# datvo06/MSAU

Measured on AMD Instinct MI355X. Metric: chargrid tiles/sec (train fwd+bwd), 336x256x64 3-stage MSAU, higher is better.
Workload: dtype bf16; 1 GPU; configs[1]: one-hot chargrid 336x256x64, 3-stage MSAU (featRoot 8, 4 scales, res_depth 2), batch 16/GPU, fwd+masked-CE+bwd+clip+Adam; global_batch=16, parallelism=dp1, graph=False

## Files before the change

### include/msau_hip.h

```cpp
#ifndef MSAU_HIP_H
#define MSAU_HIP_H

#include <stdint.h>

#ifdef __cplusplus
extern "C" {
#endif

typedef enum { MSAU_F32 = 0, MSAU_BF16 = 1 } msau_dtype;

typedef enum {
    MSAU_OK = 0,
    MSAU_ERR_ARG = -1,
    MSAU_ERR_LDS = -2,
    MSAU_ERR_HIP = -3
} msau_status;

const char* msau_last_error(void);
int msau_version(void);
const char* msau_source_hash(void);
int msau_sizeof(int which);
int msau_lds_pixel_stride(int raw_bytes, int esz, int c8_per_chunk, int read_stride);
int msau_lds_wrow_stride(int nks, int esz);

enum {
    MSAU_CONV_RELU_IN  = 1,
    MSAU_CONV_RELU_OUT = 2,
    MSAU_CONV_ADD      = 4,
    MSAU_CONV_ACCUM    = 8,
    MSAU_CONV_MASK_A   = 16,
    MSAU_CONV_MASK_B   = 32,
    MSAU_CONV_DOUT     = 128,
    MSAU_CONV_LRN      = 256,
    MSAU_CONV_POOL     = 512,
    MSAU_CONV_IDS      = 1024,
    MSAU_CONV_OWNER    = 2048,
    MSAU_CONV_NCHW     = 4096,
    MSAU_CONV_WGRAD    = 8192,
    MSAU_CONV_ELU      = 32768,
    MSAU_CONV_EXTENT   = 65536,
    MSAU_CONV_HEAD     = 64
};

typedef struct {
    int32_t B, Hin, Win, Hout, Wout;
    int32_t C1, C2;
    int32_t Cout;
    int32_t KH, KW, dil;
    int32_t pad_t, pad_l;
    int32_t stride;
    int32_t ups;
    int32_t flags;
    const void* x1;
    const void* x2;
    const void* wpack;
    const float* bias;
    const void* add;
    const void* mask_a;
    const void* mask_b;
    void* y;
    float* head_probs;
    uint8_t* head_argmax;
    int32_t head_classes;
    int32_t flags2;
    void* y2;
    const void* mask_b2;
    float lrn_alpha_over_n, lrn_beta, lrn_k;
    int32_t reserved0;
    void* pool_y;
    uint8_t* pool_idx;
    const void* wg_x1;
    float* wg_slabs;
    int32_t wg_nslabs;
    int32_t reserved1;
    const int32_t* extent;
} msau_conv_desc;
int msau_conv2d_rider_slabs(int dtype, const msau_conv_desc* d);

typedef struct {
    int32_t cch;
    int32_t nchunks;
    int32_t kchunk;
    int32_t rows;
    int64_t bytes;
} msau_conv_pack_geom;

int msau_conv_pack_geometry(int dtype, int C1_stored, int C2_stored, int Cout_stored, int KH, int KW, int dil,
                            int stride, int ups, msau_conv_pack_geom* out);
int msau_conv2d(void* stream, int dtype, const msau_conv_desc* d);
int msau_conv2d_launch_info(int dtype, const msau_conv_desc* d, int32_t* info8);

enum { MSAU_PAIR_RELU_IN = 1, MSAU_PAIR_RELU_MID = 2, MSAU_PAIR_MASK_MID = 4,
       MSAU_PAIR_LRN_BWD = 16,
       MSAU_PAIR_WGRAD1 = 32,
       MSAU_PAIR_COUPLE = 64,
       MSAU_PAIR_DCOUPLE = 128,
       MSAU_PAIR_TILES = 8 };
typedef struct {
    int32_t B, H, W, C;
    int32_t flags1, flags2;
    const void* x;
    const void* w1;
    const float* b1;
    const void* mask_mid;
    void* mid;
    const void* w2;
    const float* b2;
    const void* add;
    const void* mask_a;
    const void* mask_b;
    void* y;
    void* pool_y;
    uint8_t* pool_idx;
    uint8_t* bits_mid;
    uint8_t* bits_a;
    const void* lrn_a;
    void* lrn_da;
    float lrn_alpha_over_n, lrn_beta, lrn_k;
    int32_t reserved0;
    const void* wg1_x;
    float* wg1_slabs;
    int32_t wg1_nslabs;
    int32_t reserved1;
    const void* cpl_prev;
    const void* cpl_w;
    const float* cpl_b;
    void* cpl_y;
    void* cpl_pool_y;
    uint8_t* cpl_pool_idx;
    const void* dcp_dz;
    const void* dcp_w;
    const void* dcp_mask;
    void* dcp_dprev;
} msau_conv_pair_desc;
int msau_conv_pair_applicable(int dtype, const msau_conv_pair_desc* d);
int msau_conv_pair(void* stream, int dtype, const msau_conv_pair_desc* d);
int64_t msau_conv_pair_bits_bytes(int dtype, const msau_conv_pair_desc* d);
int msau_conv_pair_wgrad_slabs(int dtype, const msau_conv_pair_desc* d);
int msau_conv_pair_instance(int dtype, const msau_conv_pair_desc* d);
void msau_reload_env(void);

typedef struct {
    int32_t B, Hin, Win, Hout, Wout;
    int32_t C1, C2, Cout;
    int32_t KH, KW, dil, pad_t, pad_l, stride;
    int32_t flags;
    const void* x1;
    const void* x2;
    const void* g;
    float* slabs;
    int32_t nslabs;
} msau_wgrad_desc;

typedef struct {
    int32_t cch, nchunks;
    int32_t kext;
    int32_t max_slabs;
// ... 239 lines not shown
```

### msau_amd/_lib.py

```python
from __future__ import annotations

import ctypes as C
import os

HERE = os.path.dirname(os.path.abspath(__file__))
LIB_PATH = os.environ.get("MSAU_HIP_LIB", os.path.join(HERE, "libmsau_hip.so"))

F32, BF16 = 0, 1

CONV_RELU_IN, CONV_RELU_OUT, CONV_ADD, CONV_ACCUM, CONV_MASK_A, CONV_MASK_B, CONV_HEAD, CONV_DOUT = 1, 2, 4, 8, 16, 32, 64, 128
CONV_LRN, CONV_POOL, CONV_IDS, CONV_OWNER, CONV_NCHW, CONV_WGRAD, CONV_ELU = 256, 512, 1024, 2048, 4096, 8192, 32768
CONV_EXTENT = 65536

i32, i64, vp, f32 = C.c_int32, C.c_int64, C.c_void_p, C.c_float


class ConvDesc(C.Structure):
    _fields_ = [(n, i32) for n in ("B", "Hin", "Win", "Hout", "Wout", "C1", "C2", "Cout", "KH", "KW", "dil",
                                   "pad_t", "pad_l", "stride", "ups", "flags")] + \
               [(n, vp) for n in ("x1", "x2", "wpack", "bias", "add", "mask_a", "mask_b", "y", "head_probs", "head_argmax")] + \
               [("head_classes", i32), ("flags2", i32), ("y2", vp), ("mask_b2", vp)] + \
               [("lrn_alpha_over_n", f32), ("lrn_beta", f32), ("lrn_k", f32), ("reserved0", i32), ("pool_y", vp), ("pool_idx", vp)] + \
               [("wg_x1", vp), ("wg_slabs", vp), ("wg_nslabs", i32), ("reserved1", i32), ("extent", vp)]


class ConvPairDesc(C.Structure):
    _fields_ = [(n, i32) for n in ("B", "H", "W", "C", "flags1", "flags2")] + \
               [(n, vp) for n in ("x", "w1", "b1", "mask_mid", "mid", "w2", "b2", "add", "mask_a", "mask_b", "y", "pool_y", "pool_idx", "bits_mid", "bits_a",
                                  "lrn_a", "lrn_da")] + \
               [("lrn_alpha_over_n", f32), ("lrn_beta", f32), ("lrn_k", f32), ("reserved0", i32), ("wg1_x", vp), ("wg1_slabs", vp), ("wg1_nslabs", i32), ("reserved1", i32)] + \
               [(n, vp) for n in ("cpl_prev", "cpl_w", "cpl_b", "cpl_y", "cpl_pool_y", "cpl_pool_idx", "dcp_dz", "dcp_w", "dcp_mask", "dcp_dprev")]


PAIR_RELU_IN, PAIR_RELU_MID, PAIR_MASK_MID, PAIR_TILES, PAIR_LRN_BWD, PAIR_WGRAD1, PAIR_COUPLE, PAIR_DCOUPLE = 1, 2, 4, 8, 16, 32, 64, 128


class BoxArgs(C.Structure):
    _fields_ = [(n, vp) for n in ("in_", "ii", "params_fwd", "params_refl", "out", "gout", "gin", "ii_g", "ws", "flat_grads", "ws_ii",
                                  "mask_a", "add", "mask_b")] + \
               [(n, i64) for n in ("off_hmin", "off_hmax", "off_wmin", "off_wmax")] + \
               [(n, i32) for n in ("B", "H", "W", "C", "F", "Cs_in", "Cs_out", "relu_in", "accumulate")] + \
               [("max_h", f32), ("max_w", f32)]


class ConvPackGeom(C.Structure):
    _fields_ = [("cch", i32), ("nchunks", i32), ("kchunk", i32), ("rows", i32), ("bytes", i64)]


class WgradDesc(C.Structure):
    _fields_ = [(n, i32) for n in ("B", "Hin", "Win", "Hout", "Wout", "C1", "C2", "Cout", "KH", "KW", "dil",
                                   "pad_t", "pad_l", "stride", "flags")] + \
               [(n, vp) for n in ("x1", "x2", "g", "slabs")] + [("nslabs", i32)]


class WgradGeom(C.Structure):
    _fields_ = [("cch", i32), ("nchunks", i32), ("kext", i32), ("max_slabs", i32), ("slab_bytes", i64),
                ("lean", i32), ("reserved", i32)]


class PackEntry(C.Structure):
    _fields_ = [("src_off", i64), ("dst_off", i64)] + \
               [(n, i32) for n in ("kind", "dim0", "dim1", "KH", "KW", "row_is_dim0", "flip", "row_off", "rows_real",
                                   "rows_pad", "k1_real", "k1_store", "k2_real", "k2_store", "cch", "nchunks",
                                   "kchunk", "dtype")]


class UnpackEntry(C.Structure):
    _fields_ = [("slab_off", i64), ("w_off", i64), ("b_off", i64), ("b_src_off", i64), ("b_slab_stride", i64)] + \
               [(n, i32) for n in ("b_elem_stride", "b_nslabs", "b_count", "nslabs", "slab_elems", "kext", "dim0", "dim1", "KH",
                                   "KW", "row_is_dim0", "rows_real", "k1_real", "k1_store", "k2_real", "k2_store",
                                   "cch", "nchunks", "accumulate")]


class Op(C.Structure):
    _fields_ = [("kind", i32), ("dtype", i32), ("args", vp)]


class LrnArgs(C.Structure):
    _fields_ = [("a", vp), ("dy", vp), ("out", vp), ("npix", i64), ("C", i32), ("Cs", i32), ("n", i32),
                ("alpha", f32), ("beta", f32), ("k", f32)]


class PoolArgs(C.Structure):
    _fields_ = [("x_or_dy", vp), ("y_or_dx", vp), ("idx", vp), ("mask", vp)] + \
               [(n, i32) for n in ("B", "H", "W", "Cs", "accumulate")] + [("extent", vp)]


class AttnArgs(C.Structure):
    _fields_ = [(n, vp) for n in ("f", "g", "h", "x_or_dy", "y", "stats", "df", "dg", "dh", "ws")] + \
               [(n, i32) for n in ("B", "N", "Ds", "Cs")] + [("extent", vp), ("W", i32), ("reserved0", i32)]


class CsumArgs(C.Structure):
    _fields_ = [("g", vp), ("npix", i64), ("Cs", i32), ("partials", vp), ("nblk", i32)]


class ReduceArgs(C.Structure):
    _fields_ = [("slab_arena", vp), ("flat_grads", vp), ("table_dev", vp), ("n_entries", i32), ("max_elems", i32)]


class AllreduceArgs(C.Structure):
    _fields_ = [("comm", vp), ("buf", vp), ("count", i64)]


class OwnerCtx(C.Structure):
    _fields_ = [(n, vp) for n in ("owner", "boxes", "feats", "w", "wt", "table", "sums", "csum")] + \
# ... 230 lines not shown
```

### msau_amd/csrc/conv.hip

```cpp
#include "msau_common.h"

namespace {

struct ConvGeom {
    int esz, taps, cch, nchunks, kchunk, rows, CT, ngroups;
    int nslices;
};

__host__ __device__ inline int pix_stride_bytes(int cch, int esz) {
    int ps = cch * esz;
    if (((ps >> 4) & 1) == 0) ps += 16;
    return ps;
}

struct TileGeom { int TH, TIH, TIW, PS, WS, in_bytes, w_bytes, tab_bytes, total; };

inline bool conv_compact(int KH, int KW, int dil, int stride, int ups) { return stride == 1 && ups == 1 && dil >= 16 && KH * KW > 1; }

inline TileGeom tile_geom(const ConvGeom& g, int PT, int KH, int KW, int dil, int stride, int ups = 1) {
    TileGeom t;
    t.TH = 4 * PT;
    t.TIH = (t.TH - 1) * stride + (KH - 1) * dil + 1;
    t.TIW = 15 * stride + (KW - 1) * dil + 1;
    if (conv_compact(KH, KW, dil, stride, ups)) { t.TIH = KH * KW * t.TH; t.TIW = 16; }
// ... 228 lines not shown
#pragma unroll
                    for (int j = 0; j < 4; ++j) v[j] = fmaxf(v[j], 0.f);
                }
            }
            if (flags & MSAU_CONV_MASK_B) {
                V4 m = load4<T>(mask_b + pbase + co);
                if (flags & MSAU_CONV_ELU) {
#pragma unroll
                    for (int j = 0; j < 4; ++j) v[j] = ((float)m[j] > 0.f) ? v[j] : v[j] * ((float)m[j] + 1.f);
                } else {
#pragma unroll
                    for (int j = 0; j < 4; ++j) v[j] = ((float)m[j] > 0.f) ? v[j] : 0.f;
                }
            }
            if (outside) v = f32x4{0.f, 0.f, 0.f, 0.f};
            V4 o;
#pragma unroll
            for (int j = 0; j < 4; ++j) o[j] = (T)v[j];
            store4<T>(y + pbase + co, o);
        }
    }
}

template <typename T, int CT, int PT>
int launch_conv(hipStream_t s, const ConvArgs& a, int nblocks, int nsplit, int lds) {
    static bool attr_set = false;
    if (!attr_set) {
        hipError_t e = hipFuncSetAttribute(reinterpret_cast<const void*>(&conv_kernel<T, CT, PT>),
                                           hipFuncAttributeMaxDynamicSharedMemorySize, MSAU_LDS_LIMIT);
        if (e != hipSuccess) return msau_set_error(MSAU_ERR_HIP, "conv: hipFuncSetAttribute: %s", hipGetErrorString(e));
        attr_set = true;
    }
    hipLaunchKernelGGL((conv_kernel<T, CT, PT>), dim3(nblocks, nsplit), dim3(256), lds, s, a);
    MSAU_CHECK_LAUNCH("conv_kernel");
    return 0;
}

template <typename T, int CT>
int launch_conv_pt(hipStream_t s, const ConvArgs& a, int PT, int nblocks, int nsplit, int lds) {
    switch (PT) {
        case 4: return launch_conv<T, CT, 4>(s, a, nblocks, nsplit, lds);
        case 2: return launch_conv<T, CT, 2>(s, a, nblocks, nsplit, lds);
        default: return launch_conv<T, CT, 1>(s, a, nblocks, nsplit, lds);
    }
}

template <typename T>
int launch_conv_ct(hipStream_t s, const ConvArgs& a, int CT, int PT, int nblocks, int nsplit, int lds) {
    switch (CT) {
        case 1: return launch_conv_pt<T, 1>(s, a, PT, nblocks, nsplit, lds);
        case 2: return launch_conv_pt<T, 2>(s, a, PT, nblocks, nsplit, lds);
        case 4: return launch_conv_pt<T, 4>(s, a, PT, nblocks, nsplit, lds);
        default: return launch_conv_pt<T, 8>(s, a, PT, nblocks, nsplit, lds);
    }
}

}

extern "C" int msau_conv_pack_geometry(int dtype, int C1, int C2, int Cout, int KH, int KW, int dil, int stride, int ups,
                                       msau_conv_pack_geom* out) {
    ConvGeom g;
    int rc = conv_geom(dtype, C1, C2, Cout, KH, KW, dil, stride, ups, &g);
    if (rc) return rc;
    out->cch = g.cch; out->nchunks = g.nchunks; out->kchunk = g.kchunk; out->rows = g.rows * g.nslices;
    out->bytes = (int64_t)g.nslices * g.nchunks * g.rows * g.kchunk * g.esz;
    return 0;
}

static int conv_plan(int dtype, const msau_conv_desc* d, ConvGeom* gout, TileGeom* tout, int* PTout, int64_t* nbout);
int msau_conv_lean_applicable(int dtype, const msau_conv_desc* d, int nchunks, int CT);
int msau_conv_lean_try(hipStream_t s, int dtype, const msau_conv_desc* d, int kchunk, int nchunks, int CT);
int msau_conv_lean_head_capable(int dtype, const msau_conv_desc* d, int nchunks, int CT);
int msau_conv_lean_dout_capable(int dtype, const msau_conv_desc* d, int nchunks, int CT);
int msau_conv_lean_lrn_capable(int dtype, const msau_conv_desc* d, int nchunks, int CT);
int msau_conv_lean_pool_capable(int dtype, const msau_conv_desc* d, int nchunks, int CT);
int msau_conv_lean_ids_capable(int dtype, const msau_conv_desc* d, int nchunks, int CT);
int msau_conv_chunked_try(hipStream_t s, int dtype, const msau_conv_desc* d, int cch, int kchunk, int nchunks, int CT);
int msau_conv_chunked_capable(int dtype, const msau_conv_desc* d, int cch, int nchunks, int CT);
int msau_firstconv_takes(int dtype, const msau_conv_desc* d);
int msau_firstconv_launch(hipStream_t s, int dtype, const msau_conv_desc* d, int real_channels);

static int conv_takes_extent(int dtype, const msau_conv_desc* d, const ConvGeom& g) {
    const int only_others = MSAU_CONV_HEAD | MSAU_CONV_DOUT | MSAU_CONV_LRN | MSAU_CONV_POOL | MSAU_CONV_IDS | MSAU_CONV_OWNER |
                            MSAU_CONV_NCHW | MSAU_CONV_WGRAD;
    if (d->flags & only_others) return 0;
    if (g.nslices == 1 && (msau_rowconv_takes(dtype, d) || msau_conv_chunked_capable(dtype, d, g.cch, g.nchunks, g.CT) ||
                           msau_conv_lean_applicable(dtype, d, g.nchunks, g.CT)))
        return 0;
    return 1;
}

extern "C" int msau_conv2d_launch_info(int dtype, const msau_conv_desc* d, int32_t* info) {
    MSAU_CHECK_ARG(d && info, "conv2d_launch_info: null pointer");
    ConvGeom g; TileGeom t; int PT; int64_t nb;
    int rc = conv_plan(dtype, d, &g, &t, &PT, &nb);
    if (rc) return rc;
    info[0] = g.CT; info[1] = PT; info[2] = t.total; info[3] = (int32_t)nb; info[4] = g.cch; info[5] = g.nchunks;
    info[6] = msau_conv_lean_applicable(dtype, d, g.nchunks, g.CT);
    if (g.nslices == 1 && msau_rowconv_takes(dtype, d)) info[6] = 3;
    if (g.nslices == 1 && !(d->flags & (MSAU_CONV_HEAD | MSAU_CONV_DOUT | MSAU_CONV_LRN | MSAU_CONV_POOL | MSAU_CONV_IDS)) &&
        msau_conv_chunked_capable(dtype, d, g.cch, g.nchunks, g.CT)) info[6] = 2;
    info[7] = msau_conv_lean_head_capable(dtype, d, g.nchunks, g.CT) | (msau_conv_lean_dout_capable(dtype, d, g.nchunks, g.CT) << 1) |
              (((d->flags & MSAU_CONV_DOUT) && g.nslices == 1 && msau_rowconv_takes(dtype, d)) << 1) |
              (msau_conv_lean_lrn_capable(dtype, d, g.nchunks, g.CT) << 2) | (msau_conv_lean_pool_capable(dtype, d, g.nchunks, g.CT) << 3) |
              (msau_conv_lean_ids_capable(dtype, d, g.nchunks, g.CT) << 4);
    {
        msau_conv_desc p = *d;
        p.flags |= MSAU_CONV_OWNER;
        if (msau_ownerconv_takes(dtype, &p)) info[7] |= 32;
    }
    {
        msau_conv_desc p = *d;
        p.flags |= MSAU_CONV_NCHW;
        if (msau_firstconv_takes(dtype, &p)) info[7] |= 64;
    }
    {
        msau_conv_desc p = *d;
        p.flags |= MSAU_CONV_EXTENT;
        if (conv_takes_extent(dtype, &p, g)) info[7] |= 128;
    }
    if (g.nslices == 1 && !(info[7] & 4)) {
        msau_conv_desc p = *d;
        p.flags |= MSAU_CONV_LRN;
        if (!p.y2) p.y2 = p.y;
        if (!(p.lrn_k > 0.f)) p.lrn_k = 1.f;
        if (msau_rowconv_takes(dtype, &p)) info[7] |= 4;
    }
    return 0;
}

static int conv_plan(int dtype, const msau_conv_desc* d, ConvGeom* gout, TileGeom* tout, int* PTout, int64_t* nbout) {
    ConvGeom g;
    int rc = conv_geom(dtype, d->C1, d->C2, d->Cout, d->KH, d->KW, d->dil, d->stride, d->ups, &g);
    if (rc) return rc;
    int PT = 4;
    auto ntiles = [&](int pt) { return (int64_t)d->B * cdiv(d->Hout, 4 * pt) * cdiv(d->Wout, 16); };
    if (ntiles(4) < 512) PT = ntiles(2) >= 384 ? 2 : 1;
    TileGeom t = tile_geom(g, PT, d->KH, d->KW, d->dil, d->stride, d->ups);
    while (t.total > 150 * 1024 && PT > 1) { PT >>= 1; t = tile_geom(g, PT, d->KH, d->KW, d->dil, d->stride, d->ups); }
    if (t.total > 150 * 1024) return msau_set_error(MSAU_ERR_LDS, "conv2d: tile needs %d B of LDS", t.total);
    int64_t nb = ntiles(PT);
    MSAU_CHECK_ARG(nb < (1ll << 31), "conv2d: grid too large");
    *gout = g; *tout = t; *PTout = PT; *nbout = nb;
    return 0;
}

extern "C" int msau_conv2d(void* stream, int dtype, const msau_conv_desc* d) {
    MSAU_CHECK_ARG(d && d->x1 && d->wpack && d->y, "conv2d: null pointer");
    MSAU_CHECK_ARG(d->B > 0 && d->Hin > 0 && d->Win > 0 && d->Hout > 0 && d->Wout > 0, "conv2d: bad dims");
    MSAU_CHECK_ARG(d->C1 % 8 == 0 && d->C2 % 8 == 0 && (d->C2 == 0 || d->x2), "conv2d: bad sources");
    MSAU_CHECK_ARG(!(d->flags & MSAU_CONV_ADD) || d->add, "conv2d: ADD without pointer");
    MSAU_CHECK_ARG(!(d->flags & MSAU_CONV_MASK_A) || d->mask_a, "conv2d: MASK_A without pointer");
    MSAU_CHECK_ARG(!(d->flags & MSAU_CONV_MASK_B) || d->mask_b, "conv2d: MASK_B without pointer");
    if (d->flags & MSAU_CONV_EXTENT) {
        MSAU_CHECK_ARG(d->extent, "conv2d: MSAU_CONV_EXTENT without extent pointer");
        ConvGeom g;
        int rc = conv_geom(dtype, d->C1, d->C2, d->Cout, d->KH, d->KW, d->dil, d->stride, d->ups, &g);
        if (rc) return rc;
        if (!conv_takes_extent(dtype, d, g))
            return msau_set_error(MSAU_ERR_ARG, "conv2d: MSAU_CONV_EXTENT is not implemented for this launch (flags 0x%x; see "
                                  "msau_conv2d_launch_info info[7] & 128): only the generic tile kernel has it", d->flags);
    }
    if (d->flags & MSAU_CONV_WGRAD)
        MSAU_CHECK_ARG(msau_conv2d_rider_slabs(dtype, d) > 0, "conv2d: MSAU_CONV_WGRAD is not implemented for this launch (msau_conv2d_rider_slabs says 0)");
    if (d->flags & MSAU_CONV_OWNER) {
        MSAU_CHECK_ARG(msau_ownerconv_takes(dtype, d), "conv2d: MSAU_CONV_OWNER is the 3x3 stride-1 C -> 8 conv, no other flag but RELU_OUT");
        return msau_ownerconv_fwd(static_cast<hipStream_t>(stream), dtype, d);
    }
    if (d->flags & MSAU_CONV_NCHW) {
        MSAU_CHECK_ARG(msau_firstconv_takes(dtype, d) && d->head_classes > 0 && d->head_classes <= d->C1,
                       "conv2d: MSAU_CONV_NCHW is the bf16 3x3 64 -> 8 conv (W %% 4 == 0, W <= 288), head_classes = real input channels");
        return msau_firstconv_launch(static_cast<hipStream_t>(stream), dtype, d, d->head_classes);
    }
    ConvGeom g; TileGeom t; int PT; int64_t nb;
    int rc = conv_plan(dtype, d, &g, &t, &PT, &nb);
    if (rc) return rc;
    if (d->flags & MSAU_CONV_HEAD) {
        MSAU_CHECK_ARG(d->head_probs && d->head_argmax && d->head_classes > 0 && d->head_classes <= 16 &&
                       d->head_classes <= d->Cout && d->flags == MSAU_CONV_HEAD, "conv2d: bad HEAD arguments");
        if (!msau_conv_lean_head_capable(dtype, d, g.nchunks, g.CT))
            return msau_set_error(MSAU_ERR_ARG, "conv2d: MSAU_CONV_HEAD is not implemented for this launch (see "
                                  "msau_conv2d_launch_info info[7]); run msau_softmax_argmax_nhwc on y instead");
    }
    if (d->flags & MSAU_CONV_DOUT) {
        const int okf = MSAU_CONV_DOUT | MSAU_CONV_ADD | MSAU_CONV_ACCUM | MSAU_CONV_MASK_B | MSAU_CONV_WGRAD;
        MSAU_CHECK_ARG(d->y2 && !(d->flags & ~okf) && !(d->flags2 & ~(MSAU_CONV_ACCUM | MSAU_CONV_MASK_B)) &&
                       (!(d->flags2 & MSAU_CONV_MASK_B) || d->mask_b2), "conv2d: bad DOUT arguments");
        if (!msau_conv_lean_dout_capable(dtype, d, g.nchunks, g.CT) && !(g.nslices == 1 && msau_rowconv_takes(dtype, d)))
            return msau_set_error(MSAU_ERR_ARG, "conv2d: MSAU_CONV_DOUT is not implemented for this launch (see "
                                  "msau_conv2d_launch_info info[7]); issue one launch per output instead");
    }
    if (d->flags & MSAU_CONV_LRN) {
        MSAU_CHECK_ARG(d->y2 && !(d->flags & ~(MSAU_CONV_LRN | MSAU_CONV_RELU_IN)) && d->lrn_k > 0.f, "conv2d: bad LRN arguments");
        if (!msau_conv_lean_lrn_capable(dtype, d, g.nchunks, g.CT) && !(g.nslices == 1 && msau_rowconv_takes(dtype, d)))
            return msau_set_error(MSAU_ERR_ARG, "conv2d: MSAU_CONV_LRN is not implemented for this launch (see "
                                  "msau_conv2d_launch_info info[7]); run msau_lrn_fwd on y instead");
    }
    if (d->flags & MSAU_CONV_IDS) {
        if (!msau_conv_lean_ids_capable(dtype, d, g.nchunks, g.CT))
            return msau_set_error(MSAU_ERR_ARG, "conv2d: MSAU_CONV_IDS is not implemented for this launch (see msau_conv2d_launch_info "
                                  "info[7] & 16); paint the one-hot input with msau_onehot_ids instead");
    }
    if (d->flags & MSAU_CONV_POOL) {
        MSAU_CHECK_ARG(d->pool_y && !(d->flags & (MSAU_CONV_DOUT | MSAU_CONV_HEAD | MSAU_CONV_LRN)), "conv2d: bad POOL arguments");
        if (!msau_conv_lean_pool_capable(dtype, d, g.nchunks, g.CT))
            return msau_set_error(MSAU_ERR_ARG, "conv2d: MSAU_CONV_POOL is not implemented for this launch (see "
                                  "msau_conv2d_launch_info info[7]); run msau_maxpool2x2_fwd on y instead");
    }
    if (g.nslices == 1 && msau_rowconv_takes(dtype, d))
        return msau_rowconv_launch(static_cast<hipStream_t>(stream), dtype, d, g.kchunk, g.rows);
    if (g.nslices == 1 && !(d->flags & (MSAU_CONV_HEAD | MSAU_CONV_DOUT | MSAU_CONV_LRN | MSAU_CONV_POOL | MSAU_CONV_IDS))) {
        rc = msau_conv_chunked_try(static_cast<hipStream_t>(stream), dtype, d, g.cch, g.kchunk, g.nchunks, g.CT);
        if (rc != 0) return rc < 0 ? rc : 0;
    }
    if (g.nslices == 1) {
        rc = msau_conv_lean_try(static_cast<hipStream_t>(stream), dtype, d, g.kchunk, g.nchunks, g.CT);
        if (rc != 0) return rc < 0 ? rc : 0;
    }
    if (d->flags & MSAU_CONV_DOUT) return msau_set_error(MSAU_ERR_ARG, "conv2d: DOUT launch was not taken by a lean instance");
    MSAU_CHECK_ARG(g.nslices == 1 || !(d->flags & MSAU_CONV_HEAD), "conv2d: HEAD with more than 128 output channels");
    hipStream_t s = static_cast<hipStream_t>(stream);
    static const int split_wgs = getenv("MSAU_CONV_ROWSPLIT") ? atoi(getenv("MSAU_CONV_ROWSPLIT")) : 768;
    int cts = g.CT;
    while (cts > 1 && nb * g.nslices * (g.CT / cts) < split_wgs) cts >>= 1;
    const int w_bytes = roundup(cts * 16 * t.WS, 16), lds_total = t.in_bytes + w_bytes + t.tab_bytes;
    for (int sl = 0; sl < g.nslices; ++sl) {
        ConvArgs a;
        a.d = *d;
        a.ystride = d->Cout;
        a.compact = conv_compact(d->KH, d->KW, d->dil, d->stride, d->ups);
        if (g.nslices > 1) {
            const size_t co0 = (size_t)sl * 128, esz = g.esz;
            a.d.Cout = d->Cout - (int)co0 < 128 ? d->Cout - (int)co0 : 128;
            a.d.wpack = static_cast<const char*>(d->wpack) + (size_t)sl * g.nchunks * g.rows * g.kchunk * esz;
            if (d->bias) a.d.bias = d->bias + co0;
            a.d.y = static_cast<char*>(d->y) + co0 * esz;
            if (d->add) a.d.add = static_cast<const char*>(d->add) + co0 * esz;
            if (d->mask_a) a.d.mask_a = static_cast<const char*>(d->mask_a) + co0 * esz;
            if (d->mask_b) a.d.mask_b = static_cast<const char*>(d->mask_b) + co0 * esz;
        }
        a.cch = g.cch; a.nchunks = g.nchunks; a.kchunk = g.kchunk; a.ngroups = g.ngroups;
        a.TIH = t.TIH; a.TIW = t.TIW; a.PS = t.PS; a.WS = t.WS; a.in_bytes = t.in_bytes; a.w_bytes = w_bytes;
        a.tiles_x = cdiv(d->Wout, 16); a.tiles_y = cdiv(d->Hout, 4 * PT);
        a.ct_total = g.CT; a.rows_total = g.rows;
        rc = dtype == MSAU_F32 ? launch_conv_ct<float>(s, a, cts, PT, (int)nb, g.CT / cts, lds_total)
                               : launch_conv_ct<bf16_t>(s, a, cts, PT, (int)nb, g.CT / cts, lds_total);
        if (rc) return rc;
    }
    return 0;
}
```

### msau_amd/csrc/conv_lean.hip

```cpp
#include "msau_common.h"
#include <cstdlib>

namespace {

struct LeanArgs {
    msau_conv_desc d;
    int kchunk;
    int in_px1, in_px2, in_row1, in_row2;
    int out_px, out_row;
    int tiles_x, tiles_y, ntiles;
    unsigned mag_tx, mag_ty;
    int per_xcd;
    int ct_total;
#ifdef MSAU_STAMPS
    unsigned long long* stamps;
#endif
};
#ifdef MSAU_STAMPS
#define STAMP(i) do { if (a.stamps && threadIdx.x == 0) a.stamps[((size_t)blockIdx.y * gridDim.x + blockIdx.x) * 8 + (i)] = __builtin_amdgcn_s_memrealtime(); } while (0)
#else
#define STAMP(i) do {} while (0)
#endif

template <typename T, int CIN8, int CT, int KS, bool DUAL, int DIL = 1, int WGW = 1, int STRIDE = 1>
struct LeanCfg {
    static constexpr int ESZ = (int)sizeof(T);
    static constexpr int TI = 15 * STRIDE + 1 + (KS - 1) * DIL;
    static constexpr int TIW = (16 * WGW - 1) * STRIDE + 1 + (KS - 1) * DIL;
    static constexpr int NT = 256 * WGW;
    static constexpr int PSRAW = CIN8 * 8 * ESZ;
    static constexpr int NPIX = TI * TIW;
    static constexpr int NCH = DUAL ? 2 : 1;
    static constexpr int C8H = CIN8 / NCH;
    static constexpr int PS = lds_pixel_stride(PSRAW, ESZ, C8H, STRIDE);
    static constexpr int NG = KS * KS * C8H;
    static constexpr int NKSH = (NG + 3) / 4;
    static constexpr int NKS = NCH * NKSH;
    static constexpr bool WREG = CT * NKS <= 8;
    static constexpr int WS = lds_wrow_stride(NKSH, ESZ);
    static constexpr int IN_BYTES = ((NPIX * PS + 15) / 16) * 16;
    static constexpr int LDS = IN_BYTES + (WREG ? 0 : NCH * CT * 16 * WS);
};

constexpr int kOperandBits = MSAU_CONV_RELU_IN | MSAU_CONV_RELU_OUT | MSAU_CONV_ADD | MSAU_CONV_ACCUM | MSAU_CONV_MASK_A | MSAU_CONV_MASK_B;
enum { EPI_NONE = 0, EPI_LRN = 1, EPI_POOL = 2, EPI_HEAD = 3 };
template <typename T, int CIN8, int CT, int KS, bool DUAL, int DIL = 1, int WGW = 1, bool DOUT = false, bool SPLIT = false,
          int STRIDE = 1, int UPS = 1, int EPI = EPI_NONE, int EOP = -1, bool IDS = false>
__global__ __launch_bounds__(256 * WGW) void conv_lean_kernel(const LeanArgs a) {
    static_assert(!IDS || (!DUAL && STRIDE == 1 && UPS == 1 && !DOUT && !SPLIT), "id-mask input: plain single-source instances");
    static_assert(!SPLIT || (CT == 1 && !DUAL && !DOUT && WGW == 1), "SPLIT instances are single-source, one tile per workgroup");
    static_assert((STRIDE == 1 && UPS == 1) || (!DUAL && !DOUT && WGW == 1 && DIL == 1 && STRIDE * UPS == 2), "strided / upsampling instances");
    STAMP(0);
    const int cty = SPLIT ? (int)blockIdx.y : 0;
    const int CTT = SPLIT ? a.ct_total : CT;
    using Cfg = LeanCfg<T, CIN8, CT, KS, DUAL, DIL, WGW, STRIDE>;
    constexpr int NT = Cfg::NT;
    typedef typename Vec8<T>::type V8;
    typedef typename Vec4<T>::type V4;
    constexpr int ESZ = Cfg::ESZ, TI = Cfg::TIW, PS = Cfg::PS, NKS = Cfg::NKS, NG = Cfg::NG, NKSH = Cfg::NKSH, C8H = Cfg::C8H;
    extern __shared__ __align__(16) unsigned char smem[];
    const msau_conv_desc& d = a.d;
    const int tid = threadIdx.x, lane = tid & 63;
    const int wave_all = __builtin_amdgcn_readfirstlane(tid >> 6);
    const int wave = wave_all & 3, cwt = wave_all >> 2;
    const int lr = lane & 15, lg = lane >> 4;
    const bool relu_in = (EOP >= 0 ? EOP : d.flags) & MSAU_CONV_RELU_IN;

    const T* wp = static_cast<const T*>(d.wpack) + (SPLIT ? (size_t)cty * 16 * a.kchunk : 0);
    V8 afr[Cfg::WREG ? CT : 1][Cfg::WREG ? NKS : 1];
    if constexpr (Cfg::WREG) {
#pragma unroll
        for (int ct = 0; ct < CT; ++ct)
#pragma unroll
            for (int ks = 0; ks < NKS; ++ks)
                afr[ct][ks] = load8<T>(wp + ((size_t)(ks / NKSH) * (CT * 16) + ct * 16 + lr) * a.kchunk + (ks % NKSH) * 32 + lg * 8);
    }

    int koff[NKS];
#pragma unroll
    for (int ks = 0; ks < NKS; ++ks) {
        const int G = (ks % NKSH) * 4 + lg;
        const int tap = G / C8H, cg = G - tap * C8H;
        const int ky = tap / KS, kx = tap - ky * KS;
        koff[ks] = G < NG ? (ky * DIL * TI + kx * DIL) * PS + ((ks / NKSH) * C8H + cg) * 8 * ESZ : 0;
    }
    const unsigned char* pixp = smem + ((wave * 4) * STRIDE * TI + (cwt * 16 + lr) * STRIDE) * PS;

    const int flags = EOP >= 0 ? ((d.flags & ~kOperandBits) | EOP) : d.flags;
    const int Cout = d.Cout;
    f32x4 bv[CT];
#pragma unroll
    for (int ct = 0; ct < CT; ++ct) {
        bv[ct] = f32x4{0.f, 0.f, 0.f, 0.f};
        if (d.bias && lg * (CTT * 4) + (cty + ct) * 4 < Cout) bv[ct] = *reinterpret_cast<const f32x4*>(d.bias + lg * (CTT * 4) + (cty + ct) * 4);
    }
    const long long delta_add = static_cast<const char*>(d.add) - static_cast<const char*>(d.y);
    const long long delta_ma = static_cast<const char*>(d.mask_a) - static_cast<const char*>(d.y);
    const long long delta_mb = static_cast<const char*>(d.mask_b) - static_cast<const char*>(d.y);
    const int lane_out = (cwt * 16 + lr) * a.out_px + (lg * (CTT * 4) + cty * 4) * ESZ;

    constexpr int C8S = DUAL ? CIN8 / 2 : CIN8;
    constexpr int NITEMS = Cfg::NPIX * C8S;
    constexpr int NIT = (NITEMS + NT - 1) / NT;
    constexpr int NSRC = DUAL ? 2 : 1;
    constexpr bool PIPE = IDS || NIT * NSRC <= 6;
    V8 pre[IDS ? 1 : NSRC][IDS ? 1 : NIT];
    constexpr int NIDS = (Cfg::NPIX + NT - 1) / NT;
    int pre_id[IDS ? NIDS : 1];
    auto decode = [&](int tile, int& b, int& oy0, int& ox0) {
        const int t1 = a.tiles_x > 1 ? __umulhi((unsigned)tile, a.mag_tx) : tile;
        ox0 = (tile - t1 * a.tiles_x) * (16 * WGW);
        b = a.tiles_y > 1 ? __umulhi((unsigned)t1, a.mag_ty) : t1;
        oy0 = (t1 - b * a.tiles_y) * 16;
    };
    auto issue_loads = [&](int tile) {
        int b, oy0, ox0;
        decode(tile, b, oy0, ox0);
        const int vy0 = oy0 * STRIDE - d.pad_t, vx0 = ox0 * STRIDE - d.pad_l;
        if constexpr (IDS) {
            const int* ids = static_cast<const int*>(d.x1) + (long long)b * d.Hin * d.Win;
#pragma unroll
            for (int it = 0; it < NIDS; ++it) {
                const int pix = tid + it * NT;
                const int iy = pix / TI, ix = pix - iy * TI;
                const int vy = vy0 + iy, vx = vx0 + ix;
                pre_id[it] = -1;
                if (pix < Cfg::NPIX && (unsigned)vy < (unsigned)d.Hin && (unsigned)vx < (unsigned)d.Win) pre_id[it] = ids[vy * d.Win + vx];
            }
        } else
#pragma unroll
        for (int sidx = 0; sidx < NSRC; ++sidx) {
            const char* base = static_cast<const char*>(sidx ? d.x2 : d.x1) + (long long)b * d.Hin * (sidx ? a.in_row2 : a.in_row1);
            const int in_row = sidx ? a.in_row2 : a.in_row1, in_px = sidx ? a.in_px2 : a.in_px1;
#pragma unroll
            for (int it = 0; it < NIT; ++it) {
                const int idx = tid + it * NT;
                pre[sidx][it] = zero8<T>();
                if ((it + 1) * NT <= NITEMS || idx < NITEMS) {
                    const int pix = idx / C8S, cg = idx - pix * C8S;
                    const int iy = pix / TI, ix = pix - iy * TI;
                    int vy = vy0 + iy, vx = vx0 + ix;
                    bool ok;
                    if constexpr (UPS == 2) {
                        ok = vy >= 0 && vx >= 0 && !((vy | vx) & 1) && (vy >> 1) < d.Hin && (vx >> 1) < d.Win;
                        vy >>= 1; vx >>= 1;
                    } else {
                        ok = (unsigned)vy < (unsigned)d.Hin && (unsigned)vx < (unsigned)d.Win;
                    }
                    if (ok)
                        pre[sidx][it] = *reinterpret_cast<const V8*>(base + (unsigned)(vy * in_row + vx * in_px + cg * 8 * ESZ));
                }
            }
        }
    };
    auto write_lds = [&]() {
        if constexpr (IDS) {
#pragma unroll
            for (int it = 0; it < NIDS; ++it) {
                const int pix = tid + it * NT;
                if (pix < Cfg::NPIX) {
                    const int id = pre_id[it];
#pragma unroll
                    for (int cg = 0; cg < C8S; ++cg) {
                        V8 v;
#pragma unroll
                        for (int j = 0; j < 8; ++j) v[j] = (T)(cg * 8 + j == id ? 1.0f : 0.0f);
                        *reinterpret_cast<V8*>(smem + pix * PS + cg * 8 * ESZ) = v;
                    }
                }
            }
        } else
#pragma unroll
        for (int sidx = 0; sidx < NSRC; ++sidx)
#pragma unroll
            for (int it = 0; it < NIT; ++it) {
                const int idx = tid + it * NT;
                if ((it + 1) * NT <= NITEMS || idx < NITEMS) {
                    const int pix = idx / C8S, cg = idx - pix * C8S;
                    V8 v = pre[sidx][it];
                    if (relu_in) v = relu8<T>(v);
                    *reinterpret_cast<V8*>(smem + pix * PS + (sidx * C8S + cg) * 8 * ESZ) = v;
                }
            }
    };
    int tile0 = blockIdx.x, tend = a.ntiles, tstep = gridDim.x;
    if (a.per_xcd) {
        const int xcd = blockIdx.x & 7;
        tile0 = xcd * a.per_xcd + (blockIdx.x >> 3);
        tend = min(a.ntiles, (xcd + 1) * a.per_xcd);
        tstep = gridDim.x >> 3;
    }
    if (PIPE && tile0 < tend) issue_loads(tile0);
    if constexpr (!Cfg::WREG) {
        unsigned char* lds_w = smem + Cfg::IN_BYTES;
        constexpr int WG8 = NKSH * 4;
        constexpr int WTOT = Cfg::NCH * CT * 16 * WG8, NWIT = (WTOT + NT - 1) / NT, WB = NWIT < 8 ? NWIT : 8;
#pragma unroll
        for (int it0 = 0; it0 < NWIT; it0 += WB) {
            V8 wr[WB];
#pragma unroll
            for (int j = 0; j < WB; ++j) {
                const int idx = tid + (it0 + j) * NT;
                if (it0 + j < NWIT && idx < WTOT) {
                    const int r = idx / WG8, g8 = idx - r * WG8;
                    wr[j] = load8<T>(wp + (size_t)r * a.kchunk + g8 * 8);
                }
            }
#pragma unroll
            for (int j = 0; j < WB; ++j) {
                const int idx = tid + (it0 + j) * NT;
                if (it0 + j < NWIT && idx < WTOT) {
                    const int r = idx / WG8, g8 = idx - r * WG8;
                    *reinterpret_cast<V8*>(lds_w + r * Cfg::WS + g8 * 8 * ESZ) = wr[j];
                }
            }
        }
    }

    STAMP(1);
    for (int tile = tile0; tile < tend; tile += tstep) {
        int b, oy0, ox0;
        decode(tile, b, oy0, ox0);
        __syncthreads();
        if (!PIPE) issue_loads(tile);
        write_lds();
        __syncthreads();
        if (tile == tile0) STAMP(2);
        if (PIPE && tile + tstep < tend) issue_loads(tile + tstep);
        const int oyw = oy0 + wave * 4;
        f32x4 acc[CT][4];
#pragma unroll
        for (int ct = 0; ct < CT; ++ct)
#pragma unroll
            for (int pt = 0; pt < 4; ++pt) acc[ct][pt] = f32x4{0.f, 0.f, 0.f, 0.f};
#pragma unroll
        for (int ks = 0; ks < NKS; ++ks) {
            const unsigned char* p = pixp + koff[ks];
            V8 bfrag[4];
#pragma unroll
            for (int pt = 0; pt < 4; ++pt) bfrag[pt] = *reinterpret_cast<const V8*>(p + pt * STRIDE * TI * PS);
#pragma unroll
            for (int ct = 0; ct < CT; ++ct) {
                V8 af;
                if constexpr (Cfg::WREG) af = afr[ct][ks];
                else af = *reinterpret_cast<const V8*>(smem + Cfg::IN_BYTES + ((ks / NKSH) * (CT * 16) + ct * 16 + lr) * Cfg::WS +
                                                       ((ks % NKSH) * 32 + lg * 8) * ESZ);
#pragma unroll
                for (int pt = 0; pt < 4; ++pt) acc[ct][pt] = mma8(af, bfrag[pt], acc[ct][pt]);
            }
        }

        if (tile == tile0) { asm volatile("" :: "v"(acc[0][0][0])); STAMP(3); }
        if constexpr (DOUT) {
            const bool t2 = lg >= 2;
            const int lfl = t2 ? d.flags2 : flags;
            char* yb = static_cast<char*>(t2 ? d.y2 : d.y);
            const char* mb = static_cast<const char*>(t2 ? d.mask_b2 : d.mask_b);
            const char* ad = static_cast<const char*>(d.add);
            if (ox0 + lr < d.Wout) {
                const long long off0 = ((long long)(b * d.Hout + oyw)) * a.out_row + (long long)ox0 * a.out_px +
                                       lr * a.out_px + (lg & 1) * (CT * 4) * ESZ;
#pragma unroll
                for (int ct = 0; ct < CT; ++ct) {
                    V4 r_add[4], r_acc[4], r_mb[4];
#pragma unroll
                    for (int pt = 0; pt < 4; ++pt) {
                        if (oyw + pt < d.Hout) {
                            const long long o = off0 + ct * 4 * ESZ + (long long)pt * a.out_row;
                            if (lfl & MSAU_CONV_ADD) r_add[pt] = *reinterpret_cast<const V4*>(ad + o);
                            if (lfl & MSAU_CONV_ACCUM) r_acc[pt] = *reinterpret_cast<const V4*>(yb + o);
                            if (lfl & MSAU_CONV_MASK_B) r_mb[pt] = *reinterpret_cast<const V4*>(mb + o);
                        }
                    }
#pragma unroll
                    for (int pt = 0; pt < 4; ++pt) {
                        if (oyw + pt < d.Hout) {
                            const long long o = off0 + ct * 4 * ESZ + (long long)pt * a.out_row;
                            f32x4 v = acc[ct][pt] + bv[ct];
                            if (lfl & MSAU_CONV_ADD) {
#pragma unroll
                                for (int j = 0; j < 4; ++j) v[j] += (float)r_add[pt][j];
                            }
                            if (lfl & MSAU_CONV_ACCUM) {
#pragma unroll
                                for (int j = 0; j < 4; ++j) v[j] += (float)r_acc[pt][j];
                            }
                            if (lfl & MSAU_CONV_MASK_B) {
#pragma unroll
                                for (int j = 0; j < 4; ++j) v[j] = ((float)r_mb[pt][j] > 0.f) ? v[j] : 0.f;
                            }
                            V4 ov;
#pragma unroll
                            for (int j = 0; j < 4; ++j) ov[j] = (T)v[j];
                            *reinterpret_cast<V4*>(yb + o) = ov;
                        }
                    }
                }
            }
        } else {
        constexpr bool POOL_OK = EPI == EPI_POOL;
        static_assert(EPI == EPI_NONE || (CT <= 2 && !DOUT && STRIDE == 1 && UPS == 1), "fused epilogues: <= 2 channel tiles, one output");
        V4 keep[POOL_OK ? CT : 1][4];
        if constexpr (POOL_OK) {
#pragma unroll
            for (int ct = 0; ct < CT; ++ct)
#pragma unroll
                for (int pt = 0; pt < 4; ++pt)
#pragma unroll
// ... 213 lines not shown
        const int oy0 = (t1 - b * a.tiles_y) * 16;
        const int vy0 = oy0 - d.pad_t, vx0 = ox0 - d.pad_l;
        const char* xb = static_cast<const char*>(d.x1) + (long long)b * d.Hin * a.in_row1;
        auto issue = [&](int ch) {
#pragma unroll
            for (int it = 0; it < NITX; ++it) {
                const int idx = tid + it * 256;
                const int pix = idx / C8CH, cg = idx - pix * C8CH;
                const int iy = pix / TI, ix = pix - iy * TI;
                const int vy = vy0 + iy, vx = vx0 + ix;
                xr[it] = zero8<T>();
                if (idx < NPIX * C8CH && (unsigned)vy < (unsigned)d.Hin && (unsigned)vx < (unsigned)d.Win)
                    xr[it] = *reinterpret_cast<const V8*>(xb + (unsigned)(vy * a.in_row1 + vx * a.in_px1 + (ch * C8CH * 8 + cg * 8) * ESZ));
            }
#pragma unroll
            for (int it = 0; it < NITW; ++it) {
                const int idx = tid + it * 256;
                const int r = idx / WG8, g8 = idx - r * WG8;
                wr[it] = zero8<T>();
                if (idx < CT * 16 * WG8) wr[it] = load8<T>(wp + ((size_t)ch * CT * 16 + r) * a.kchunk + g8 * 8);
            }
        };
        f32x4 acc[CT][4];
#pragma unroll
        for (int ct = 0; ct < CT; ++ct)
#pragma unroll
            for (int pt = 0; pt < 4; ++pt) acc[ct][pt] = f32x4{0.f, 0.f, 0.f, 0.f};
        issue(0);
        for (int ch = 0; ch < nchunks; ++ch) {
            __syncthreads();
#pragma unroll
            for (int it = 0; it < NITX; ++it) {
                const int idx = tid + it * 256;
                if (idx < NPIX * C8CH) *reinterpret_cast<V8*>(smem + (idx / C8CH) * PS + (idx % C8CH) * 8 * ESZ) = xr[it];
            }
#pragma unroll
            for (int it = 0; it < NITW; ++it) {
                const int idx = tid + it * 256;
                const int r = idx / WG8, g8 = idx - r * WG8;
                if (idx < CT * 16 * WG8) *reinterpret_cast<V8*>(lds_w + r * WS + g8 * 8 * ESZ) = wr[it];
            }
            __syncthreads();
            if (ch + 1 < nchunks) issue(ch + 1);
#pragma unroll
            for (int ks = 0; ks < NKS; ++ks) {
                const unsigned char* p = pixp + koff[ks];
                V8 bfrag[4];
#pragma unroll
                for (int pt = 0; pt < 4; ++pt) bfrag[pt] = *reinterpret_cast<const V8*>(p + pt * TI * PS);
#pragma unroll
                for (int ct = 0; ct < CT; ++ct) {
                    const V8 af = *reinterpret_cast<const V8*>(lds_w + (ct * 16 + lr) * WS + (ks * 32 + lg * 8) * ESZ);
#pragma unroll
                    for (int pt = 0; pt < 4; ++pt) acc[ct][pt] = mma8(af, bfrag[pt], acc[ct][pt]);
                }
            }
        }
        const int oyw = oy0 + wave * 4;
        if (ox0 + lr < d.Wout) {
            char* y = static_cast<char*>(d.y) + ((long long)(b * d.Hout + oyw) * d.Wout + ox0 + lr) * a.out_px;
#pragma unroll
            for (int ct = 0; ct < CT; ++ct) {
                if (lg * (CT * 4) + ct * 4 >= d.Cout) continue;
#pragma unroll
                for (int pt = 0; pt < 4; ++pt) {
                    if (oyw + pt < d.Hout) {
                        f32x4 v = acc[ct][pt] + bv[ct];
                        if (d.flags & MSAU_CONV_RELU_OUT) {
#pragma unroll
                            for (int j = 0; j < 4; ++j) v[j] = fmaxf(v[j], 0.f);
                        }
                        V4 o;
#pragma unroll
                        for (int j = 0; j < 4; ++j) o[j] = (T)v[j];
                        *reinterpret_cast<V4*>(y + (long long)pt * a.out_row + (lg * (CT * 4) + ct * 4) * ESZ) = o;
                    }
                }
            }
        }
    }
}

template <typename T, int CIN8, int CT, int KS, bool DUAL, int DIL = 1, int WGW = 1, bool DOUT = false, bool SPLIT = false,
          int STRIDE = 1, int UPS = 1, int EPI = EPI_NONE, int EOP = -1, bool IDS = false>
int launch_lean_e(hipStream_t s, const LeanArgs& a0) {
    using Cfg = LeanCfg<T, CIN8, CT, KS, DUAL, DIL, WGW, STRIDE>;
    if (Cfg::LDS + 256 > MSAU_LDS_LIMIT) return 0;
    LeanArgs a = a0;
    a.tiles_x = cdiv(a.d.Wout, 16 * WGW);
    a.ntiles = a.d.B * a.tiles_x * a.tiles_y;
    a.mag_tx = (unsigned)((0x100000000ull + a.tiles_x - 1) / a.tiles_x);
    static bool attr_set = false;
    if (!attr_set && Cfg::LDS > 60 * 1024) {
        hipError_t e = hipFuncSetAttribute(reinterpret_cast<const void*>(&conv_lean_kernel<T, CIN8, CT, KS, DUAL, DIL, WGW, DOUT, SPLIT, STRIDE, UPS, EPI, EOP, IDS>),
                                           hipFuncAttributeMaxDynamicSharedMemorySize, MSAU_LDS_LIMIT);
        if (e != hipSuccess) return msau_set_error(MSAU_ERR_HIP, "conv_lean: hipFuncSetAttribute: %s", hipGetErrorString(e));
        attr_set = true;
    }
    int per_cu = MSAU_LDS_LIMIT / (Cfg::LDS + 256);
    static const int percu_max = std::getenv("MSAU_LEAN_PERCU") ? atoi(std::getenv("MSAU_LEAN_PERCU")) : 4;
    per_cu = per_cu < 1 ? 1 : (per_cu > percu_max / WGW ? (percu_max / WGW < 1 ? 1 : percu_max / WGW) : per_cu);
    int grid = 256 * per_cu;
    if (grid > a.ntiles) grid = a.ntiles;
    static const bool xcd_off = std::getenv("MSAU_XCD") && std::getenv("MSAU_XCD")[0] == '0';
    a.per_xcd = 0;
    if (!xcd_off && grid >= 64) {
        grid &= ~7;
        a.per_xcd = cdiv(a.ntiles, 8);
    }
    hipLaunchKernelGGL((conv_lean_kernel<T, CIN8, CT, KS, DUAL, DIL, WGW, DOUT, SPLIT, STRIDE, UPS, EPI, EOP, IDS>), dim3(grid, SPLIT ? a.ct_total : 1), dim3(256 * WGW), Cfg::LDS, s, a);
    MSAU_CHECK_LAUNCH("conv_lean_kernel");
    return 1;
}

template <typename T, int CIN8, int CT, int KS, bool DUAL, int DIL = 1, int WGW = 1, bool DOUT = false, bool SPLIT = false,
          int STRIDE = 1, int UPS = 1, int EPI = EPI_NONE>
int launch_lean(hipStream_t s, const LeanArgs& a) {
    if constexpr (CIN8 <= 2 && !DOUT && EPI != EPI_HEAD) {
        switch (a.d.flags & kOperandBits) {
#define EOP_CASE(V) case V: return launch_lean_e<T, CIN8, CT, KS, DUAL, DIL, WGW, DOUT, SPLIT, STRIDE, UPS, EPI, V>(s, a);
            EOP_CASE(0) EOP_CASE(2) EOP_CASE(3) EOP_CASE(6) EOP_CASE(8) EOP_CASE(12) EOP_CASE(20) EOP_CASE(32) EOP_CASE(40)
#undef EOP_CASE
            default: break;
        }
    }
    return launch_lean_e<T, CIN8, CT, KS, DUAL, DIL, WGW, DOUT, SPLIT, STRIDE, UPS, EPI, -1>(s, a);
}

template <typename T, int CIN8, int KS, bool DUAL>
int lean_ct(hipStream_t s, const LeanArgs& a, int CT) {
    if constexpr (sizeof(T) == 2 && (CIN8 == 1 || (DUAL && CIN8 == 2)) && KS == 3) {
        if (CT == 1 && a.d.Wout >= 64 && (int64_t)a.d.B * a.tiles_y * cdiv(a.d.Wout, 32) >= 512)
            return launch_lean<T, CIN8, 1, KS, DUAL, 1, 2>(s, a);
    }
    if (CT == 1) return launch_lean<T, CIN8, 1, KS, DUAL>(s, a);
    if (CT == 2) return launch_lean<T, CIN8, 2, KS, DUAL>(s, a);
    if constexpr (CIN8 >= 4 && KS != 4) {
        if (CT == 4) return launch_lean<T, CIN8, 4, KS, DUAL>(s, a);
    }
    return 0;
}

template <typename T, int KS>
int lean_cin(hipStream_t s, const LeanArgs& a, int cin8, bool dual, int CT) {
    if (!dual) {
        switch (cin8) {
            case 1: return lean_ct<T, 1, KS, false>(s, a, CT);
            case 2: return lean_ct<T, 2, KS, false>(s, a, CT);
            case 4: return lean_ct<T, 4, KS, false>(s, a, CT);
            case 8: return lean_ct<T, 8, KS, false>(s, a, CT);
            default: return 0;
        }
    }
    switch (cin8) {
        case 2: return lean_ct<T, 2, KS, true>(s, a, CT);
        case 4: return lean_ct<T, 4, KS, true>(s, a, CT);
        case 8: return lean_ct<T, 8, KS, true>(s, a, CT);
        case 16: if constexpr (KS == 1) return lean_ct<T, 16, KS, true>(s, a, CT); else return 0;
        default: return 0;
    }
}

template <typename T, int DIL>
int lean_dil(hipStream_t s, const LeanArgs& a, int cin8, int CT) {
#define LD_CASE(C8, CTV) if (cin8 == C8 && CT == CTV) return launch_lean<T, C8, CTV, 3, false, DIL>(s, a);
    LD_CASE(1, 1) LD_CASE(2, 1) LD_CASE(2, 2) LD_CASE(4, 1) LD_CASE(4, 2) LD_CASE(4, 4) LD_CASE(8, 2)
#undef LD_CASE
    return 0;
}

}

static bool lean_split_wanted(const msau_conv_desc* d, int CT);

static int lean_lds_bytes(int esz, int cin8, int CT, int KS, int dil, int wgw, int stride, bool dual) {
    const int ti = 15 * stride + 1 + (KS - 1) * dil, tiw = (16 * wgw - 1) * stride + 1 + (KS - 1) * dil;
    const int psraw = cin8 * 8 * esz, ps = ((psraw / 16) % 2 == 0) ? psraw + 16 : psraw;
    const int nch = dual ? 2 : 1, c8h = cin8 / nch, ng = KS * KS * c8h, nksh = (ng + 3) / 4, nks = nch * nksh;
    const bool wreg = CT * nks <= 8;
    const int ws = nksh * 32 * esz + 16;
    const int in_bytes = ((ti * tiw * ps + 15) / 16) * 16;
    return in_bytes + (wreg ? 0 : nch * CT * 16 * ws);
}

static bool lean_strided_shape(const msau_conv_desc* d, int nchunks, int CT) {
    if (d->KH != 3 || d->KW != 3 || d->dil != 1 || d->C2 || nchunks != 1 || d->stride * d->ups != 2) return false;
    if (d->flags & (MSAU_CONV_DOUT | MSAU_CONV_HEAD | MSAU_CONV_RELU_IN)) return false;
    if (d->pad_t < 0 || d->pad_l < 0 || d->pad_t > 2 || d->pad_l > 2) return false;
    if ((int64_t)d->B * cdiv(d->Hout, 16) * cdiv(d->Wout, 16) < 64) return false;
    const int c8 = d->C1 / 8;
    if (d->ups == 2) return (c8 == 8 && CT == 2) || (c8 == 4 && CT == 1) || (c8 == 2 && CT == 1);
    return (c8 == 4 && CT == 4) || (c8 == 2 && CT == 2) || (c8 == 1 && CT == 1);
}
template <typename T>
int lean_strided(hipStream_t s, const LeanArgs& a, int c8, int CT, bool ups) {
#define ST_CASE(C8, CTV, ST, UP) if (c8 == C8 && CT == CTV) return launch_lean<T, C8, CTV, 3, false, 1, 1, false, false, ST, UP>(s, a);
    if (ups) { ST_CASE(8, 2, 1, 2) ST_CASE(4, 1, 1, 2) ST_CASE(2, 1, 1, 2) }
    else { ST_CASE(4, 4, 2, 1) ST_CASE(2, 2, 2, 1) ST_CASE(1, 1, 2, 1) }
#undef ST_CASE
    return 0;
}

int msau_conv_lean_applicable(int dtype, const msau_conv_desc* d, int nchunks, int CT) {
    if (d->flags & (MSAU_CONV_ELU | MSAU_CONV_EXTENT)) return 0;
    if (d->stride * d->ups == 2) {
        const int esz = dtype == MSAU_F32 ? 4 : 2;
        if ((int64_t)d->Hin * d->Win * d->C1 * esz >= (1ll << 31) || (int64_t)d->Wout * d->Cout * esz * 20 >= (1ll << 31)) return 0;
        if (!lean_strided_shape(d, nchunks, CT)) return 0;
        return lean_lds_bytes(esz, d->C1 / 8, CT, 3, 1, 1, d->stride, false) + 256 <= MSAU_LDS_LIMIT;
    }
    if (d->stride != 1 || d->ups != 1 || d->KH != d->KW || (d->KH != 1 && d->KH != 3 && d->KH != 4)) return 0;
    if (d->dil != 1) {
        if (d->KH != 3 || d->C2 || (d->dil != 2 && d->dil != 4 && d->dil != 8)) return 0;
        const int c8 = d->C1 / 8;
        const bool ok = (c8 == 1 && CT == 1) || (c8 == 2 && CT <= 2) || (c8 == 4 && (CT == 1 || CT == 2 || CT == 4)) || (c8 == 8 && CT == 2);
        if (!ok) return 0;
    }
    if (nchunks != (d->C2 ? 2 : 1)) return 0;
    if (d->Hin != d->Hout || d->Win != d->Wout) return 0;
    if (d->pad_t < 0 || d->pad_l < 0 || d->pad_t > (d->KH - 1) * d->dil || d->pad_l > (d->KW - 1) * d->dil) return 0;
    if (CT > 4 || (CT == 4 && (d->C1 + d->C2) < 32)) return 0;
    if (d->KH == 4 && ((d->C1 + d->C2) != 8 || d->C2)) return 0;
    if ((int64_t)d->B * cdiv(d->Hout, 16) * cdiv(d->Wout, 16) < 64) return 0;
    const bool dual = d->C2 != 0;
    if (dual && d->C1 != d->C2) return 0;
    const int cin8 = (d->C1 + d->C2) / 8;
    const int esz = dtype == MSAU_F32 ? 4 : 2;
    if ((int64_t)d->Hin * d->Win * (d->C1 > d->C2 ? d->C1 : d->C2) * esz >= (1ll << 31)) return 0;
    if ((int64_t)d->Wout * d->Cout * esz * 20 >= (1ll << 31)) return 0;
    if (cin8 != 1 && cin8 != 2 && cin8 != 4 && cin8 != 8 && !(cin8 == 16 && dual && d->KH == 1)) return 0;
    if (dual && cin8 < 2) return 0;
    const bool split = lean_split_wanted(d, CT);
    if (lean_lds_bytes(esz, cin8, split ? 1 : CT, d->KH, d->dil, 1, 1, dual) + 256 > MSAU_LDS_LIMIT) return 0;
    return 1;
}

int msau_conv_lean_dout_capable(int dtype, const msau_conv_desc* d, int nchunks, int CT) {
    if (!msau_conv_lean_applicable(dtype, d, nchunks, CT)) return 0;
    return d->C2 == 0 && d->dil == 1 && d->stride == 1 && d->ups == 1 && (d->KH == 1 || d->KH == 3) && (CT == 1 || CT == 2 || CT == 4) &&
           d->Cout == CT * 16 && d->C1 == CT * 8;
}

static bool lean_wide_tile(const msau_conv_desc* d, int tiles_y) {
    return d->Wout >= 64 && (int64_t)d->B * tiles_y * cdiv(d->Wout, 32) >= 512;
}
static int lean_epi_case(int dtype, const msau_conv_desc* d, int CT, int epi) {
    const int c8 = (d->C1 + d->C2) / 8, k = d->KH;
    const bool dual = d->C2 != 0, split = lean_split_wanted(d, CT);
    if (epi == EPI_LRN && !dual && !split && k == 3) {
        if (c8 == 1 && CT == 1 && d->dil == 1 && d->Cout == 8) return dtype == MSAU_BF16 && lean_wide_tile(d, cdiv(d->Hout, 16)) ? 1 : 2;
        if (c8 == 1 && CT == 1 && d->dil == 2 && d->Cout == 16) return 3;
        if (c8 == 2 && CT == 2 && d->dil == 4 && d->Cout == 32) return 4;
        if (c8 == 2 && CT == 1 && d->dil == 1 && d->Cout == 16) return 5;
        if (c8 == 2 && CT == 2 && d->dil == 2 && d->Cout == 32) return 6;
    }
    if (epi == EPI_POOL && d->dil == 1) {
        if (dual && k == 1 && !split) {
            if (c8 == 2 && CT == 1) return 10;
            if (c8 == 4 && CT == 1) return 11;
            if (c8 == 8 && CT == 2) return 12;
        }
        if (!dual && k == 3 && split && c8 == 4) return 13;
    }
    return 0;
}
template <typename T>
int lean_epi(hipStream_t s, const LeanArgs& a, int which) {
    switch (which) {
        case 1: if constexpr (sizeof(T) == 2) return launch_lean<T, 1, 1, 3, false, 1, 2, false, false, 1, 1, EPI_LRN>(s, a); else return 0;
        case 2: return launch_lean<T, 1, 1, 3, false, 1, 1, false, false, 1, 1, EPI_LRN>(s, a);
        case 3: return launch_lean<T, 1, 1, 3, false, 2, 1, false, false, 1, 1, EPI_LRN>(s, a);
        case 4: return launch_lean<T, 2, 2, 3, false, 4, 1, false, false, 1, 1, EPI_LRN>(s, a);
        case 5: return launch_lean<T, 2, 1, 3, false, 1, 1, false, false, 1, 1, EPI_LRN>(s, a);
        case 6: return launch_lean<T, 2, 2, 3, false, 2, 1, false, false, 1, 1, EPI_LRN>(s, a);
        case 10: return launch_lean<T, 2, 1, 1, true, 1, 1, false, false, 1, 1, EPI_POOL>(s, a);
        case 11: return launch_lean<T, 4, 1, 1, true, 1, 1, false, false, 1, 1, EPI_POOL>(s, a);
        case 12: return launch_lean<T, 8, 2, 1, true, 1, 1, false, false, 1, 1, EPI_POOL>(s, a);
        case 13: return launch_lean<T, 4, 1, 3, false, 1, 1, false, true, 1, 1, EPI_POOL>(s, a);
        default: return 0;
    }
}

int msau_conv_lean_lrn_capable(int dtype, const msau_conv_desc* d, int nchunks, int CT) {
    if (!msau_conv_lean_applicable(dtype, d, nchunks, CT)) return 0;
    if (d->stride != 1 || d->ups != 1 || (d->flags & (MSAU_CONV_DOUT | MSAU_CONV_HEAD | MSAU_CONV_POOL))) return 0;
    return lean_epi_case(dtype, d, CT, EPI_LRN) != 0;
}

int msau_conv_lean_pool_capable(int dtype, const msau_conv_desc* d, int nchunks, int CT) {
    if (!msau_conv_lean_applicable(dtype, d, nchunks, CT)) return 0;
    if (d->stride != 1 || d->ups != 1 || (d->flags & (MSAU_CONV_DOUT | MSAU_CONV_HEAD | MSAU_CONV_LRN))) return 0;
    return lean_epi_case(dtype, d, CT, EPI_POOL) != 0;
}

template <typename T>
int lean_dout(hipStream_t s, const LeanArgs& a, int KS, int CT) {
#define DO_CASE(K, C) if (KS == K && CT == C) return launch_lean<T, C, C, K, false, 1, 1, true>(s, a);
    DO_CASE(1, 1) DO_CASE(1, 2) DO_CASE(1, 4) DO_CASE(3, 1) DO_CASE(3, 2) DO_CASE(3, 4)
#undef DO_CASE
    return 0;
}

static int lean_split_tiles() {
    static const int v = std::getenv("MSAU_SPLIT_TILES") ? atoi(std::getenv("MSAU_SPLIT_TILES")) : 512;
    return v;
}
static bool lean_split_wanted(const msau_conv_desc* d, int CT) {
    const int cin8 = d->C1 / 8;
    return d->C2 == 0 && d->dil == 1 && (d->KH == 1 || d->KH == 3) && (CT == 2 || CT == 4) && (cin8 == 4 || cin8 == 8) &&
           !(d->flags & (MSAU_CONV_DOUT | MSAU_CONV_HEAD)) &&
           (int64_t)d->B * cdiv(d->Hout, 16) * cdiv(d->Wout, 16) < lean_split_tiles();
}
template <typename T>
int lean_split(hipStream_t s, const LeanArgs& a, int cin8, int KS) {
#define SP_CASE(C8, K) if (cin8 == C8 && KS == K) return launch_lean<T, C8, 1, K, false, 1, 1, false, true>(s, a);
    SP_CASE(4, 1) SP_CASE(4, 3) SP_CASE(8, 1) SP_CASE(8, 3)
#undef SP_CASE
    return 0;
}

int msau_conv_lean_ids_capable(int dtype, const msau_conv_desc* d, int nchunks, int CT) {
    msau_conv_desc e = *d;
    e.flags &= ~MSAU_CONV_IDS;
    return msau_conv_lean_applicable(dtype, &e, nchunks, CT) && d->C1 == 64 && d->C2 == 0 && CT == 1 && d->KH == 3 && d->dil == 1 &&
           d->stride == 1 && d->ups == 1 && !(d->flags & ~(MSAU_CONV_IDS | MSAU_CONV_RELU_OUT));
}

int msau_conv_lean_head_capable(int dtype, const msau_conv_desc* d, int nchunks, int CT) {
    return msau_conv_lean_applicable(dtype, d, nchunks, CT) && d->KH == 4 && CT == 1 && d->dil == 1;
}

static int chunked_variant(int dtype, const msau_conv_desc* d, int cch, int nchunks, int CT) {
    static const bool off = std::getenv("MSAU_CONV_CHUNKED") && std::getenv("MSAU_CONV_CHUNKED")[0] == '0';
    if (off || nchunks < 2 || d->C2 || d->KH != 3 || d->KW != 3 || d->stride != 1 || d->ups != 1) return 0;
    if (d->Hin != d->Hout || d->Win != d->Wout || d->pad_t < 0 || d->pad_l < 0 || d->pad_t > 2 * d->dil || d->pad_l > 2 * d->dil) return 0;
    if (d->flags & ~MSAU_CONV_RELU_OUT) return 0;
    const int esz = dtype == MSAU_F32 ? 4 : 2;
    if ((int64_t)d->Hin * d->Win * d->C1 * esz >= (1ll << 31)) return 0;
    const int64_t ntiles = (int64_t)d->B * cdiv(d->Wout, 16) * cdiv(d->Hout, 16);
    if (!(ntiles >= 64 && ntiles < (1 << 20) && cdiv(d->Wout, 16) < 4096 && cdiv(d->Hout, 16) < 4096)) return 0;
    if (cch == 64 && CT == 1 && d->dil == 1) return 1;
    if (cch == 32 && CT == 2 && d->dil == 8 && nchunks == 2 && dtype == MSAU_BF16) return 2;
    return 0;
}
int msau_conv_chunked_capable(int dtype, const msau_conv_desc* d, int cch, int nchunks, int CT) {
    if (d->flags & (MSAU_CONV_ELU | MSAU_CONV_EXTENT)) return 0;
    return chunked_variant(dtype, d, cch, nchunks, CT) != 0;
}

template <typename T, int C8CH, int CT, int DIL>
static int launch_chunked(hipStream_t s, const LeanArgs& a, int nchunks) {
    using Cfg = LeanCfg<T, C8CH, CT, 3, false, DIL>;
    constexpr int lds = Cfg::IN_BYTES + CT * 16 * lds_wrow_stride(Cfg::NKS, Cfg::ESZ);
    static_assert(lds + 256 <= MSAU_LDS_LIMIT, "chunked conv: tile + weight chunk must fit the LDS");
    static bool attr_set = false;
    if (!attr_set && lds > 60 * 1024) {
        hipError_t e = hipFuncSetAttribute(reinterpret_cast<const void*>(&conv_chunked_kernel<T, C8CH, CT, DIL>), hipFuncAttributeMaxDynamicSharedMemorySize, MSAU_LDS_LIMIT);
        if (e != hipSuccess) return msau_set_error(MSAU_ERR_HIP, "conv_chunked: hipFuncSetAttribute: %s", hipGetErrorString(e));
        attr_set = true;
    }
    int per_cu = MSAU_LDS_LIMIT / (lds + 256);
    per_cu = per_cu < 1 ? 1 : (per_cu > 3 ? 3 : per_cu);
    int grid = 256 * per_cu;
    if (grid > a.ntiles) grid = a.ntiles;
    hipLaunchKernelGGL((conv_chunked_kernel<T, C8CH, CT, DIL>), dim3(grid), dim3(256), lds, s, a, nchunks);
    MSAU_CHECK_LAUNCH("conv_chunked_kernel");
    return 1;
}

int msau_conv_chunked_try(hipStream_t s, int dtype, const msau_conv_desc* d, int cch, int kchunk, int nchunks, int CT) {
    const int variant = chunked_variant(dtype, d, cch, nchunks, CT);
    if (!variant) return 0;
    const int esz = dtype == MSAU_F32 ? 4 : 2;
    LeanArgs a;
    a.d = *d;
    a.kchunk = kchunk;
    a.in_px1 = d->C1 * esz; a.in_row1 = d->Win * a.in_px1; a.in_px2 = a.in_row2 = 0;
    a.out_px = d->Cout * esz; a.out_row = d->Wout * a.out_px;
    a.tiles_x = cdiv(d->Wout, 16); a.tiles_y = cdiv(d->Hout, 16);
// ... 63 lines not shown
```

### msau_amd/csrc/conv_rows.hip

```cpp
#include "msau_common.h"
#include <cstdlib>
#include <utility>

namespace {

typedef unsigned int u32x4 __attribute__((ext_vector_type(4)));
typedef unsigned int u32x2 __attribute__((ext_vector_type(2)));
typedef unsigned long long u64;
constexpr unsigned kOOB = 0x80000000u;

constexpr int OW = 30, XW = 34;
constexpr int MP = XW * 16;
constexpr int WAVE_LDS = 2 * MP;
constexpr int UNR = 6;
typedef __attribute__((address_space(3))) bf16x4* lds_v4;
constexpr int WG_ROW = 36 * 16;

struct RowArgs {
    msau_conv_pair_desc d;
    int nstrips, nseg, SH, ntasks, tasks_per_xcd;
    int row_bytes;
    unsigned img_bytes, plane_img;
};

// ... 694 lines not shown
                for (int jj = 0; jj < 4; ++jj) bal[jj] = __builtin_amdgcn_ballot_w64((float)r[jj] > 0.f);
                __builtin_amdgcn_raw_buffer_store_b32(lane_word(bal), rba, ownrow ? (unsigned)(t * plane_pitch) + bal_off : kOOB, 0, 0);
            }
            bf16x4 po = o;
            if constexpr (CPL != 0) {
                *reinterpret_cast<bf16x4*>(ywr) = o;
                __builtin_amdgcn_wave_barrier();
                const u32x4 yb = *reinterpret_cast<const u32x4*>(yrd);
                __builtin_amdgcn_wave_barrier();
                u32x4 bf;
#pragma unroll
                for (int w = 0; w < 4; ++w) bf[w] = lg < 2 ? PV[I % 3][w] : yb[w];
                PV[I % 3] = load_prev(t + 3);
                const f32x4 zacc = mma8(AC, __builtin_bit_cast(bf16x8, bf), cbias);
#pragma unroll
                for (int jj = 0; jj < 4; ++jj) po[jj] = (bf16_t)fmaxf(zacc[jj], 0.f);
                __builtin_amdgcn_raw_buffer_store_b64(__builtin_bit_cast(u32x2, po), rcz, ownrow ? (unsigned)(t * a.row_bytes) + out_col : kOOB, 0, 0);
            }
            if constexpr (PL) {
                bf16x4 cur;
#pragma unroll
                for (int jj = 0; jj < 4; ++jj) cur[jj] = ownrow && out_ok ? po[jj] : (bf16_t)0.f;
                const bool odd = (t & 1) != 0;
                const bool last_even = !odd && t == H - 1;
                if (odd || last_even) {
                    const bf16x4 top = odd ? prev_out : cur, bot = odd ? cur : bf16x4{};
                    typedef int dw2 __attribute__((ext_vector_type(2)));
                    dw2 st = __builtin_bit_cast(dw2, top), sb = __builtin_bit_cast(dw2, bot), nt, nb;
#pragma unroll
                    for (int w = 0; w < 2; ++w) {
                        nt[w] = __builtin_amdgcn_mov_dpp(st[w], 0xB1, 0xf, 0xf, true);
                        nb[w] = __builtin_amdgcn_mov_dpp(sb[w], 0xB1, 0xf, 0xf, true);
                    }
                    const bf16x4 ntop = __builtin_bit_cast(bf16x4, nt), nbot = __builtin_bit_cast(bf16x4, nb);
                    bf16x4 best;
                    unsigned idx = 0;
#pragma unroll
                    for (int jj = 0; jj < 4; ++jj) {
                        float bv = (float)top[jj];
                        unsigned bi = 0;
                        const float c1 = (float)ntop[jj], c2 = (float)bot[jj], c3 = (float)nbot[jj];
                        if (c1 > bv) { bv = c1; bi = 1; }
                        if (c2 > bv) { bv = c2; bi = 2; }
                        if (c3 > bv) { bv = c3; bi = 3; }
                        best[jj] = (bf16_t)bv;
                        idx |= bi << (8 * jj);
                    }
                    const int ty = odd ? t - 1 : t;
                    const bool pok = out_ok && !(lr & 1) && ty >= y0 && ty < y1;
                    const unsigned e = (unsigned)(((ty >> 1) * Wo + ((x0 + lr) >> 1)) * 16 + c0);
                    __builtin_amdgcn_raw_buffer_store_b64(__builtin_bit_cast(u32x2, best), rp, pok ? e * 2 : kOOB, 0, 0);
                    __builtin_amdgcn_raw_buffer_store_b32(idx, ri, pok ? e : kOOB, 0, 0);
                }
                prev_out = cur;
            }
        }
        if constexpr (BWD) {
            cu64p pm = plane_row(pm0, m + 2), pa = plane_row(pa0, t + 2);
#pragma unroll
            for (int jj = 0; jj < 4; ++jj) { mm[P][jj] = pm[jj]; ma[P][jj] = pa[jj]; }
        }
        __builtin_amdgcn_sched_barrier(0);
    };

    for (int tg = y0 - 2; tg < y1; tg += UNR) {
        step(IC<0>{}, tg);
        step(IC<1>{}, tg);
        step(IC<2>{}, tg);
        step(IC<3>{}, tg);
        step(IC<4>{}, tg);
        step(IC<5>{}, tg);
    }
}

struct RowConvArgs {
    msau_conv_desc d;
    int nstrips, nseg, SH, ntasks, tasks_per_xcd;
    int row_bytes, wrow, wchunk;
    unsigned img_bytes;
};

constexpr int WGC_ROW = 32 * 16;

template <int NS, int KH, int KW, int EPI, int EPI2 = 0, bool WG = false>
__global__ __launch_bounds__(256) void rowconv8_kernel(const RowConvArgs a) {
    constexpr bool DOUT = (EPI & MSAU_CONV_DOUT) != 0;
    static_assert(!WG || (DOUT && KW == 1 && NS == 1 && EPI == MSAU_CONV_DOUT && EPI2 == MSAU_CONV_MASK_B), "the rider belongs to the coupling conv's data gradient");
    __shared__ __align__(16) unsigned char wsm[WG ? 4 * 3 * WGC_ROW + 64 + 2 * 8 * 16 * 4 : 16];
    constexpr bool K1D = KW == 1 && NS == 2;
    static_assert((KW == 3 && (NS == 1 || NS == 2)) || (K1D && KH == 1) || (KW == 1 && NS == 1 && KH == 1 && DOUT) || (KW == 4 && NS == 1),
                  "instances: 3x3, 1x1 dual, 1x1 two-output, 4x4");
    static_assert(!DOUT || (!(EPI & ~(MSAU_CONV_DOUT | MSAU_CONV_ADD | MSAU_CONV_ACCUM | MSAU_CONV_MASK_B)) && !(EPI2 & ~(MSAU_CONV_ACCUM | MSAU_CONV_MASK_B)) &&
                            NS == 1 && KW != 4), "two outputs: EPI = flags of y, EPI2 = flags2 of y2");
    static_assert(DOUT || EPI2 == 0, "EPI2 belongs to the second output");
    constexpr int XL = KW == 4 ? 2 : 1;
    constexpr int NSL = K1D ? 1 : NS;
#ifndef MSAU_ROWCONV_PF
#define MSAU_ROWCONV_PF 3
#endif
    constexpr int NXR = KH == 4 ? 8 : KH + MSAU_ROWCONV_PF;
    constexpr bool HAS_MA = (EPI & MSAU_CONV_MASK_A) != 0, HAS_ADD = (EPI & MSAU_CONV_ADD) != 0, HAS_ACC = (EPI & MSAU_CONV_ACCUM) != 0,
                   HAS_MB = (EPI & MSAU_CONV_MASK_B) != 0, RELU_OUT = (EPI & MSAU_CONV_RELU_OUT) != 0, LRN = (EPI & MSAU_CONV_LRN) != 0;
    const msau_conv_desc& d = a.d;
    const int lane = threadIdx.x & 63;
    const int wave = __builtin_amdgcn_readfirstlane(threadIdx.x >> 6);
    const int tloc = (blockIdx.x >> 3) * 4 + wave;
    const int task = (blockIdx.x & 7) * a.tasks_per_xcd + tloc;
    const bool live = tloc < a.tasks_per_xcd && task < a.ntasks;
    if constexpr (!WG) { if (!live) return; }
    f32x4 wacc = {0.f, 0.f, 0.f, 0.f}, waccb = {0.f, 0.f, 0.f, 0.f};
    if (live) {
    const int t1 = task / a.nstrips, strip = task - t1 * a.nstrips;
    const int b = t1 / a.nseg, seg = t1 - b * a.nseg;
    const int H = d.Hout, W = d.Wout;
    const int x0 = strip * 32;
    const int y0 = seg * a.SH, y1 = min(H, y0 + a.SH);
    const int lr = lane & 15, lg = lane >> 4;
    const int c0 = (lg & 1) * 4;
    const int j = 2 * lr + (lg >> 1);

    bf16x8 A[NSL][KH][XL];
    bf16x8 A2[DOUT ? KH : 1];
    {
        const int co = lr & 7, pp = lr >> 3;
        const bf16_t* w = static_cast<const bf16_t*>(d.wpack) + co * a.wrow;
#pragma unroll
        for (int s = 0; s < NSL; ++s)
#pragma unroll
            for (int ky = 0; ky < KH; ++ky) {
                if constexpr (K1D) {
                    const bool ok = (lg & 1) == pp;
                    A[s][ky][0] = ok ? load8<bf16_t>(w + (lg >> 1) * a.wchunk) : zero8<bf16_t>();
                } else {
                    const int kx = lg - pp;
                    const bool ok = kx >= 0 && kx < KW;
                    A[s][ky][0] = ok ? load8<bf16_t>(w + s * a.wchunk + (ky * KW + (ok ? kx : 0)) * 8) : zero8<bf16_t>();
                    if constexpr (KW == 4) {
                        const bool ok4 = lg == 0 && pp == 1;
                        A[s][ky][1] = ok4 ? load8<bf16_t>(w + s * a.wchunk + (ky * KW + 3) * 8) : zero8<bf16_t>();
                    }
                    if constexpr (DOUT) A2[ky] = ok ? load8<bf16_t>(w + 8 * a.wrow + (ky * KW + (ok ? kx : 0)) * 8) : zero8<bf16_t>();
                }
            }
    }
    f32x4 bias = {0.f, 0.f, 0.f, 0.f}, bias2 = {0.f, 0.f, 0.f, 0.f};
    if (d.bias) bias = *reinterpret_cast<const f32x4*>(d.bias + c0);
    if (DOUT && d.bias) bias2 = *reinterpret_cast<const f32x4*>(d.bias + 8 + c0);
    constexpr bool ACC2 = (EPI2 & MSAU_CONV_ACCUM) != 0, MB2 = (EPI2 & MSAU_CONV_MASK_B) != 0;

    const long long img = (long long)b * a.img_bytes;
    const __amdgpu_buffer_rsrc_t rx1 = rsrc_of(static_cast<const char*>(d.x1) + img, a.img_bytes);
    const __amdgpu_buffer_rsrc_t rx2 = rsrc_of(NS == 2 && !K1D ? static_cast<const char*>(d.x2) + img : nullptr, NS == 2 && !K1D ? a.img_bytes : 0u);
    const __amdgpu_buffer_rsrc_t ry = rsrc_of(static_cast<char*>(d.y) + img, a.img_bytes);
    const __amdgpu_buffer_rsrc_t ry2 = rsrc_of(LRN || DOUT ? static_cast<char*>(d.y2) + img : nullptr, LRN || DOUT ? a.img_bytes : 0u);
    const __amdgpu_buffer_rsrc_t rma = rsrc_of(HAS_MA ? static_cast<const char*>(d.mask_a) + img : nullptr, HAS_MA ? a.img_bytes : 0u);
    const __amdgpu_buffer_rsrc_t radd = rsrc_of(HAS_ADD ? static_cast<const char*>(d.add) + img : nullptr, HAS_ADD ? a.img_bytes : 0u);
    const __amdgpu_buffer_rsrc_t rmb = rsrc_of(HAS_MB ? static_cast<const char*>(d.mask_b) + img : nullptr, HAS_MB ? a.img_bytes : 0u);
    const __amdgpu_buffer_rsrc_t rmb2 = rsrc_of(MB2 ? static_cast<const char*>(d.mask_b2) + img : nullptr, MB2 ? a.img_bytes : 0u);

    const int lxm = K1D ? x0 + 2 * lr + (lg & 1) : x0 - d.pad_l + 2 * lr + lg;
    const int lxe = x0 - d.pad_l + 2 * lr + 4;
    const unsigned lcol_m = (unsigned)lxm < (unsigned)W && !(KW == 1 && !K1D && lg >= 2) ? (unsigned)(lxm * 16) : kOOB;
    const unsigned lcol_e = (unsigned)lxe < (unsigned)W ? (unsigned)(lxe * 16) : kOOB;
    const int rlast = min(H - 1, y1 - 1 - d.pad_t + KH - 1);
    const bool b075 = d.lrn_beta == 0.75f;
    u32x4 X[NSL][NXR][XL];
    const char* src1x1 = nullptr;
    if constexpr (K1D) src1x1 = static_cast<const char*>(lg < 2 ? d.x1 : d.x2) + img + (lxm < W ? lxm : W - 1) * 16;
    auto load_row = [&](int r, auto slot) {
        constexpr int S = decltype(slot)::value;
        const bool ok = r >= 0 && r <= rlast;
        const unsigned ro = (unsigned)(r * a.row_bytes);
        if constexpr (K1D) {
            X[0][S][0] = *reinterpret_cast<const u32x4*>(src1x1 + (long long)(ok ? r : y0) * a.row_bytes);
        } else {
            X[0][S][0] = __builtin_amdgcn_raw_buffer_load_b128(rx1, ok ? ro + lcol_m : kOOB, 0, 0);
            if constexpr (KW == 4) X[0][S][1] = __builtin_amdgcn_raw_buffer_load_b128(rx1, ok ? ro + lcol_e : kOOB, 0, 0);
            if constexpr (NS == 2) X[1][S][0] = __builtin_amdgcn_raw_buffer_load_b128(rx2, ok ? ro + lcol_m : kOOB, 0, 0);
        }
    };
    const bool out_ok = x0 + j < W;
    const unsigned out_col = out_ok ? (unsigned)((x0 + j) * 16 + c0 * 2) : kOOB;
    u32x2 OPA[2], OPD[2], OPB[2], OPY[2], OPB2[2], OPY2[2];
    auto load_ops = [&](int t, auto slot) {
        constexpr int P = decltype(slot)::value;
        const unsigned o = (t >= y0 && t < y1) ? (unsigned)(t * a.row_bytes) + out_col : kOOB;
        if constexpr (ACC2) OPY2[P] = __builtin_amdgcn_raw_buffer_load_b64(ry2, o, 0, 0);
        if constexpr (MB2) OPB2[P] = __builtin_amdgcn_raw_buffer_load_b64(rmb2, o, 0, 0);
        if constexpr (HAS_MA) OPA[P] = __builtin_amdgcn_raw_buffer_load_b64(rma, o, 0, 0);
        if constexpr (HAS_ADD) OPD[P] = __builtin_amdgcn_raw_buffer_load_b64(radd, o, 0, 0);
        if constexpr (HAS_ACC) OPY[P] = __builtin_amdgcn_raw_buffer_load_b64(ry, o, 0, 0);
        if constexpr (HAS_MB) OPB[P] = __builtin_amdgcn_raw_buffer_load_b64(rmb, o, 0, 0);
    };

    u32x4 PVX[WG ? NXR : 1];
    const __amdgpu_buffer_rsrc_t rwp = rsrc_of(WG ? static_cast<const char*>(d.wg_x1) + img : nullptr, WG ? a.img_bytes : 0u);
    auto load_prev = [&](int r, auto slot) {
        constexpr int S = decltype(slot)::value;
        if constexpr (WG) PVX[S] = __builtin_amdgcn_raw_buffer_load_b128(rwp, r >= y0 && r < y1 ? (unsigned)(r * a.row_bytes) + lcol_m : kOOB, 0, 0);
    };
    unsigned char* const wbase = wsm + wave * 3 * WGC_ROW;
    unsigned char* const wzero = wsm + 4 * 3 * WGC_ROW;
    const int wpx = (2 * lr + lg) * 16;
    const int wry = j * 16 + c0 * 2;
    const int trp = 8 * (lane >> 4) + ((lane & 15) >> 2), trc = lane & 3;
    const unsigned char* const tr_x = wbase + (trc < 2 ? WGC_ROW : 2 * WGC_ROW) + trp * 16 + (trc & 1) * 8;
    const unsigned char* const tr_g = trc < 2 ? wbase + trp * 16 + (trc & 1) * 8 : wzero + (trc & 1) * 8;
    const int tr_g_hi = trc < 2 ? 4 * 16 : 0;
    auto trfrag = [&](const unsigned char* p, int hi) -> bf16x8 {
        const bf16x4 lo4 = __builtin_amdgcn_ds_read_tr16_b64_v4bf16((lds_v4)p);
        const bf16x4 hi4 = __builtin_amdgcn_ds_read_tr16_b64_v4bf16((lds_v4)(p + hi));
        return __builtin_shufflevector(lo4, hi4, 0, 1, 2, 3, 4, 5, 6, 7);
    };
    const u32x4 wones_bits = {0x3F803F80u, 0x3F803F80u, 0x3F803F80u, 0x3F803F80u};
    if constexpr (WG) {
        if (lane < 4) reinterpret_cast<unsigned*>(wzero)[lane] = 0u;
        __builtin_amdgcn_wave_barrier();
    }

    {
        const int r0 = y0 - d.pad_t;
        [&]<int... K>(std::integer_sequence<int, K...>) { (load_row(r0 + K, IC<K>{}), ...); }(std::make_integer_sequence<int, NXR - 1>{});
        [&]<int... K>(std::integer_sequence<int, K...>) { (load_prev(r0 + K, IC<K>{}), ...); }(std::make_integer_sequence<int, NXR - 1>{});
    }
    load_ops(y0, IC<0>{});
    load_ops(y0 + 1, IC<1>{});

    auto step = [&](auto ic, const int tg) {
        constexpr int I = decltype(ic)::value, P = I & 1;
        const int t = tg + I;
        load_row(t - d.pad_t + NXR - 1, IC<(I + NXR - 1) % NXR>{});
        load_prev(t - d.pad_t + NXR - 1, IC<(I + NXR - 1) % NXR>{});
        f32x4 acc = bias;
#pragma unroll
        for (int ky = 0; ky < KH; ++ky)
#pragma unroll
            for (int s = 0; s < NSL; ++s)
#pragma unroll
                for (int e = 0; e < XL; ++e) acc = mma8(A[s][ky][e], __builtin_bit_cast(bf16x8, X[s][(I + ky) % NXR][e]), acc);
        const unsigned oo = (t >= y0 && t < y1) ? (unsigned)(t * a.row_bytes) + out_col : kOOB;
        if constexpr (DOUT) {
            f32x4 acc_b = bias2;
#pragma unroll
            for (int ky = 0; ky < KH; ++ky) acc_b = mma8(A2[ky], __builtin_bit_cast(bf16x8, X[0][(I + ky) % NXR][0]), acc_b);
            bf16x4 o1, o2;
#pragma unroll
            for (int jj = 0; jj < 4; ++jj) {
                float v1 = acc[jj];
                if constexpr (HAS_ADD) v1 += (float)__builtin_bit_cast(bf16x4, OPD[P])[jj];
                if constexpr (HAS_ACC) v1 += (float)__builtin_bit_cast(bf16x4, OPY[P])[jj];
                if constexpr (HAS_MB) v1 = (float)__builtin_bit_cast(bf16x4, OPB[P])[jj] > 0.f ? v1 : 0.f;
                float v2 = acc_b[jj];
                if constexpr (ACC2) v2 += (float)__builtin_bit_cast(bf16x4, OPY2[P])[jj];
                if constexpr (MB2) v2 = (float)__builtin_bit_cast(bf16x4, OPB2[P])[jj] > 0.f ? v2 : 0.f;
                o1[jj] = (bf16_t)v1;
                o2[jj] = (bf16_t)v2;
            }
            __builtin_amdgcn_raw_buffer_store_b64(__builtin_bit_cast(u32x2, o1), ry, oo, 0, 0);
            __builtin_amdgcn_raw_buffer_store_b64(__builtin_bit_cast(u32x2, o2), ry2, oo, 0, 0);
            if constexpr (WG) {
                if (lg < 2) {
                    *reinterpret_cast<u32x4*>(wbase + wpx) = X[0][I % NXR][0];
                    *reinterpret_cast<u32x4*>(wbase + WGC_ROW + wpx) = PVX[I % NXR];
                }
                *reinterpret_cast<u32x2*>(wbase + 2 * WGC_ROW + wry) = OPB2[P];
                __builtin_amdgcn_wave_barrier();
                const bf16x8 xf = trfrag(tr_x, 4 * 16);
                const bf16x8 gf = trfrag(tr_g, tr_g_hi);
                __builtin_amdgcn_wave_barrier();
                wacc = mma8(xf, gf, wacc);
                waccb = mma8(__builtin_bit_cast(bf16x8, wones_bits), gf, waccb);
            }
            load_ops(t + 2, IC<P>{});
            __builtin_amdgcn_sched_barrier(0);
            return;
        }
        f32x4 v = acc;
        if constexpr (HAS_MA) {
            const bf16x4 mk = __builtin_bit_cast(bf16x4, OPA[P]);
#pragma unroll
            for (int jj = 0; jj < 4; ++jj) v[jj] = (float)mk[jj] > 0.f ? v[jj] : 0.f;
        }
        if constexpr (HAS_ADD) {
            const bf16x4 ad = __builtin_bit_cast(bf16x4, OPD[P]);
#pragma unroll
            for (int jj = 0; jj < 4; ++jj) v[jj] += (float)ad[jj];
        }
        if constexpr (HAS_ACC) {
            const bf16x4 yo = __builtin_bit_cast(bf16x4, OPY[P]);
#pragma unroll
            for (int jj = 0; jj < 4; ++jj) v[jj] += (float)yo[jj];
        }
        if constexpr (RELU_OUT) {
#pragma unroll
            for (int jj = 0; jj < 4; ++jj) v[jj] = fmaxf(v[jj], 0.f);
        }
        if constexpr (HAS_MB) {
            const bf16x4 mk = __builtin_bit_cast(bf16x4, OPB[P]);
#pragma unroll
            for (int jj = 0; jj < 4; ++jj) v[jj] = (float)mk[jj] > 0.f ? v[jj] : 0.f;
        }
        bf16x4 o;
#pragma unroll
        for (int jj = 0; jj < 4; ++jj) o[jj] = (bf16_t)v[jj];
        __builtin_amdgcn_raw_buffer_store_b64(__builtin_bit_cast(u32x2, o), ry, oo, 0, 0);
        if constexpr (LRN) {
            float x[4], Pf[4], run = 0.f;
#pragma unroll
            for (int jj = 0; jj < 4; ++jj) { x[jj] = (float)o[jj]; run += x[jj] * x[jj]; Pf[jj] = run; }
            const int h = lg & 1;
            const float other = __builtin_bit_cast(float, __builtin_amdgcn_ds_swizzle(__builtin_bit_cast(int, run), 0x401F));
            const float inc = h ? run + other : run;
            const float E = inc - run;
            const float tot = h ? inc : other + run;
            bf16x4 o2;
// ... 402 lines not shown
    const int SH = segment_rows(d->B, d->H, nstrips, c8 ? 2 + SKEW : 2, !c8);
    const int ntasks = d->B * nstrips * cdiv(d->H, SH);
    return 8 * (roundup(cdiv(ntasks, 8), 4) / 4);
}

int msau_rowpair_launch(hipStream_t s, const msau_conv_pair_desc* d) {
    RowArgs a;
    a.d = *d;
    const bool c8 = d->C == 8;
    const bool bwd = (d->flags1 & ~(MSAU_PAIR_LRN_BWD | MSAU_PAIR_WGRAD1)) == kBwd1, bits = d->bits_mid && d->bits_a, pool = !bwd && (d->flags2 & MSAU_CONV_POOL);
    const int cpl = !bwd && (d->flags1 & MSAU_PAIR_COUPLE) ? (d->cpl_pool_y ? 2 : 1) : 0;
    a.nstrips = cdiv(d->W, c8 ? OW : OW16);
    a.SH = segment_rows(d->B, d->H, a.nstrips, c8 ? 2 + SKEW : 2, !c8);
    if ((pool || cpl == 2) && (a.SH & 1) && a.SH < d->H) ++a.SH;
    a.nseg = cdiv(d->H, a.SH);
    a.ntasks = d->B * a.nstrips * a.nseg;
    a.tasks_per_xcd = roundup(cdiv(a.ntasks, 8), 4);
    a.row_bytes = d->W * d->C * 2;
    a.img_bytes = (unsigned)d->H * (unsigned)a.row_bytes;
    a.plane_img = (unsigned)d->H * (unsigned)a.nstrips * 32u;
    const dim3 grid(8 * (a.tasks_per_xcd / 4)), block(256);
    if (d->flags1 & MSAU_PAIR_WGRAD1)
        MSAU_CHECK_ARG((int)grid.x == d->wg1_nslabs, "conv_pair: MSAU_PAIR_WGRAD1 launch has %d workgroups, the caller allocated %d slabs "
                       "(msau_conv_pair_wgrad_slabs under other MSAU_ROWS_* settings?)", (int)grid.x, d->wg1_nslabs);
    if (c8) {
        const bool lrnb = d->flags1 & MSAU_PAIR_LRN_BWD, wg1 = d->flags1 & MSAU_PAIR_WGRAD1;
        if (bwd && lrnb && wg1) hipLaunchKernelGGL((rowpair_c8_kernel<true, true, true, true>), grid, block, 0, s, a);
        else if (bwd && wg1) hipLaunchKernelGGL((rowpair_c8_kernel<true, true, false, true>), grid, block, 0, s, a);
        else if (bwd && lrnb) hipLaunchKernelGGL((rowpair_c8_kernel<true, true, true>), grid, block, 0, s, a);
        else if (bwd) hipLaunchKernelGGL((rowpair_c8_kernel<true, true>), grid, block, 0, s, a);
        else if (cpl == 2 && bits) hipLaunchKernelGGL((rowpair_c8_kernel<false, true, false, false, 2>), grid, block, 0, s, a);
        else if (cpl == 2) hipLaunchKernelGGL((rowpair_c8_kernel<false, false, false, false, 2>), grid, block, 0, s, a);
        else if (cpl && bits) hipLaunchKernelGGL((rowpair_c8_kernel<false, true, false, false, 1>), grid, block, 0, s, a);
        else if (cpl) hipLaunchKernelGGL((rowpair_c8_kernel<false, false, false, false, 1>), grid, block, 0, s, a);
        else if (bits) hipLaunchKernelGGL((rowpair_c8_kernel<false, true>), grid, block, 0, s, a);
        else hipLaunchKernelGGL((rowpair_c8_kernel<false, false>), grid, block, 0, s, a);
    } else {
        if (bwd && (d->flags1 & MSAU_PAIR_LRN_BWD)) hipLaunchKernelGGL((rowpair_c16_kernel<true, true, false, 0, true>), grid, block, 0, s, a);
        else if (bwd) hipLaunchKernelGGL((rowpair_c16_kernel<true, true, false>), grid, block, 0, s, a);
        else if (cpl == 2 && bits) hipLaunchKernelGGL((rowpair_c16_kernel<false, true, false, 2>), grid, block, 0, s, a);
        else if (cpl == 2) hipLaunchKernelGGL((rowpair_c16_kernel<false, false, false, 2>), grid, block, 0, s, a);
        else if (cpl && bits) hipLaunchKernelGGL((rowpair_c16_kernel<false, true, false, 1>), grid, block, 0, s, a);
        else if (cpl) hipLaunchKernelGGL((rowpair_c16_kernel<false, false, false, 1>), grid, block, 0, s, a);
        else if (bits && pool) hipLaunchKernelGGL((rowpair_c16_kernel<false, true, true>), grid, block, 0, s, a);
        else if (bits) hipLaunchKernelGGL((rowpair_c16_kernel<false, true, false>), grid, block, 0, s, a);
        else if (pool) hipLaunchKernelGGL((rowpair_c16_kernel<false, false, true>), grid, block, 0, s, a);
        else hipLaunchKernelGGL((rowpair_c16_kernel<false, false, false>), grid, block, 0, s, a);
    }
    MSAU_CHECK_LAUNCH("rowpair_kernel");
    return 0;
}

namespace {
template <int NS, int KH, int KW, int EPI, int EPI2 = 0>
int launch_rowconv8(hipStream_t s, const RowConvArgs& a) {
    hipLaunchKernelGGL((rowconv8_kernel<NS, KH, KW, EPI, EPI2>), dim3(8 * (a.tasks_per_xcd / 4)), dim3(256), 0, s, a);
    MSAU_CHECK_LAUNCH("rowconv8_kernel");
    return 0;
}
int rowconv_case(int dtype, const msau_conv_desc* d) {
    const RowsEnv& e = rows_env();
    if (!e.on || !e.conv || dtype != MSAU_BF16 || (d->flags & (MSAU_CONV_ELU | MSAU_CONV_EXTENT))) return 0;
    if (d->ups == 2) {
        const bool c16 = d->C1 == 16 && d->Cout == 8, c32 = d->C1 == 32 && d->Cout == 16 && e.deconv >= 2;
        if (!e.deconv || !(c16 || c32) || d->C2 != 0 || d->KH != 3 || d->KW != 3 || d->stride != 1 || d->dil != 1 || d->flags) return 0;
        if (d->pad_t != 1 || d->pad_l != 1) return 0;
        if ((d->Hout != 2 * d->Hin && d->Hout != 2 * d->Hin - 1) || (d->Wout != 2 * d->Win && d->Wout != 2 * d->Win - 1)) return 0;
        if ((int64_t)d->Hout * d->Wout * d->Cout * 2 >= (1ll << 31)) return 0;
        if ((int64_t)d->B * cdiv(d->Win, 16) * cdiv(d->Hout, 8) < e.min_tasks) return 0;
        return c16 ? 12 : 16;
    }
    const bool dout = d->flags & MSAU_CONV_DOUT;
    if (d->Cout != (dout ? 16 : 8) || d->C1 != 8 || (d->C2 != 0 && d->C2 != 8) || d->stride != 1 || d->ups != 1 || d->dil != 1) return 0;
    if (d->Hin != d->Hout || d->Win != d->Wout || d->KH != d->KW) return 0;
    if ((int64_t)d->Hout * d->Wout * 16 >= (1ll << 31)) return 0;
    if ((int64_t)d->B * cdiv(d->Wout, 32) * cdiv(d->Hout, 8) < e.min_tasks) return 0;
    const int f = d->flags, k = d->KH, dual = d->C2 != 0;
    if (dout) {
        if (!e.dout || dual || !d->y2) return 0;
        const int f1 = f & ~MSAU_CONV_DOUT, f2 = d->flags2;
        if (k == 3 && d->pad_t == 1 && d->pad_l == 1 && f2 == 0) return f1 == 0 ? 9 : f1 == MSAU_CONV_ACCUM ? 10 : 0;
        if (k == 1 && d->pad_t == 0 && d->pad_l == 0 && f1 == 0 && f2 == MSAU_CONV_MASK_B && d->mask_b2) return 11;
        if (k == 1 && d->pad_t == 0 && d->pad_l == 0 && f1 == MSAU_CONV_WGRAD && f2 == MSAU_CONV_MASK_B && d->mask_b2 && d->wg_x1 && d->wg_slabs && e.cplwg) return 13;
        return 0;
    }
    if (k == 3 && !dual && d->pad_t == 1 && d->pad_l == 1) {
        if (f == MSAU_CONV_LRN) return d->y2 && d->lrn_k > 0.f ? 1 : 0;
        if (f == 0) return 2;
        if (f == MSAU_CONV_ACCUM) return 3;
    }
    if (k == 3 && dual && d->pad_t == 1 && d->pad_l == 1 && f == 0) return 4;
    if (k == 1 && dual && d->pad_t == 0 && d->pad_l == 0 && f == MSAU_CONV_RELU_OUT) return 5;
    if (k == 4 && !dual && d->pad_t == d->pad_l && (d->pad_t == 1 || d->pad_t == 2)) {
        if (f == 0) return 6;
        if (f == MSAU_CONV_MASK_B) return 7;
        if (f == (MSAU_CONV_ACCUM | MSAU_CONV_MASK_B)) return 8;
    }
    return 0;
}
}

int msau_rowconv_takes(int dtype, const msau_conv_desc* d) { return rowconv_case(dtype, d) != 0; }

namespace {
void rowconv_split(const msau_conv_desc* d, RowConvArgs& a) {
    a.nstrips = cdiv(d->Wout, 32);
    const int unr = d->KH == 4 ? 8 : d->KH + MSAU_ROWCONV_PF;
    const RowsEnv& e = rows_env();
    int nseg = e.waves / (d->B * a.nstrips);
    if (nseg < 1) nseg = 1;
    int sh = e.sh > 0 ? e.sh : cdiv(d->Hout, nseg);
    if (sh < 8) sh = 8;
    sh = roundup(sh, unr);
    a.SH = sh < d->Hout ? sh : d->Hout;
    a.nseg = cdiv(d->Hout, a.SH);
    a.ntasks = d->B * a.nstrips * a.nseg;
    a.tasks_per_xcd = roundup(cdiv(a.ntasks, 8), 4);
}
}

extern "C" int msau_conv2d_rider_slabs(int dtype, const msau_conv_desc* d) {
    if (!d || !(d->flags & MSAU_CONV_WGRAD) || rowconv_case(dtype, d) != 13) return 0;
    RowConvArgs a;
    rowconv_split(d, a);
    return 8 * (a.tasks_per_xcd / 4);
}

int msau_rowconv_launch(hipStream_t s, int dtype, const msau_conv_desc* d, int kchunk, int rows) {
    const int which = rowconv_case(dtype, d);
    if (which == 12 || which == 16) {
        MSAU_CHECK_ARG(kchunk == (which == 12 ? 160 : 288) && rows == 16, "rowdeconv: packed image of another geometry (kchunk %d, rows %d)", kchunk, rows);
        RowDeconvArgs a;
        a.d = *d;
        a.nstrips = cdiv(d->Win, 16);
        const RowsEnv& e = rows_env();
        int nseg = e.waves / (d->B * a.nstrips);
        if (nseg < 1) nseg = 1;
        int sh = e.sh > 0 ? e.sh : cdiv(d->Hout, nseg);
        if (sh < 8) sh = 8;
        a.SH = roundup(sh, 8);
        a.nseg = cdiv(d->Hout, a.SH);
        a.ntasks = d->B * a.nstrips * a.nseg;
        a.tasks_per_xcd = roundup(cdiv(a.ntasks, 8), 4);
        a.in_row_bytes = d->Win * d->C1 * 2;
        a.out_row_bytes = d->Wout * d->Cout * 2;
        a.in_img_bytes = (unsigned)d->Hin * (unsigned)a.in_row_bytes;
        a.out_img_bytes = (unsigned)d->Hout * (unsigned)a.out_row_bytes;
        if (which == 12) hipLaunchKernelGGL(rowdeconv8_kernel, dim3(8 * (a.tasks_per_xcd / 4)), dim3(256), 0, s, a);
        else hipLaunchKernelGGL(rowdeconv16_kernel, dim3(8 * (a.tasks_per_xcd / 4)), dim3(256), 0, s, a);
        MSAU_CHECK_LAUNCH("rowdeconv_kernel");
        return 0;
    }
    RowConvArgs a;
    a.d = *d;
    rowconv_split(d, a);
    a.row_bytes = d->Wout * 16;
    a.img_bytes = (unsigned)d->Hout * (unsigned)a.row_bytes;
    a.wrow = kchunk;
    a.wchunk = rows * kchunk;
    switch (which) {
        case 1: return launch_rowconv8<1, 3, 3, MSAU_CONV_LRN>(s, a);
        case 2: return launch_rowconv8<1, 3, 3, 0>(s, a);
        case 3: return launch_rowconv8<1, 3, 3, MSAU_CONV_ACCUM>(s, a);
        case 4: return launch_rowconv8<2, 3, 3, 0>(s, a);
        case 5: return launch_rowconv8<2, 1, 1, MSAU_CONV_RELU_OUT>(s, a);
        case 6: return launch_rowconv8<1, 4, 4, 0>(s, a);
        case 7: return launch_rowconv8<1, 4, 4, MSAU_CONV_MASK_B>(s, a);
        case 8: return launch_rowconv8<1, 4, 4, MSAU_CONV_ACCUM | MSAU_CONV_MASK_B>(s, a);
        case 9: return launch_rowconv8<1, 3, 3, MSAU_CONV_DOUT>(s, a);
        case 10: return launch_rowconv8<1, 3, 3, MSAU_CONV_DOUT | MSAU_CONV_ACCUM>(s, a);
        case 11: return launch_rowconv8<1, 1, 1, MSAU_CONV_DOUT, MSAU_CONV_MASK_B>(s, a);
        case 13:
            MSAU_CHECK_ARG(8 * (a.tasks_per_xcd / 4) == d->wg_nslabs, "conv2d: MSAU_CONV_WGRAD launch has %d workgroups, the caller allocated %d slabs "
                           "(msau_conv2d_rider_slabs under other MSAU_ROWS_* settings?)", 8 * (a.tasks_per_xcd / 4), d->wg_nslabs);
            hipLaunchKernelGGL((rowconv8_kernel<1, 1, 1, MSAU_CONV_DOUT, MSAU_CONV_MASK_B, true>), dim3(8 * (a.tasks_per_xcd / 4)), dim3(256), 0, s, a);
            MSAU_CHECK_LAUNCH("rowconv8_kernel");
            return 0;
    }
    return msau_set_error(MSAU_ERR_ARG, "rowconv: no instance");
}

int msau_rowwgrad_takes(int dtype, const msau_wgrad_desc* d, int cch, int nchunks, int kextc) {
    const RowsEnv& e = rows_env();
    if (!e.on || !e.wgrad || dtype != MSAU_BF16) return 0;
    if (d->C1 != 8 || d->C2 != 0 || d->Cout != 8 || (d->KH != 3 && d->KH != 4) || d->KW != d->KH || d->dil != 1 || d->stride != 1) return 0;
    if (d->pad_t != 1 || d->pad_l != 1 || d->Hin != d->Hout || d->Win != d->Wout) return 0;
    if (d->flags & ~MSAU_CONV_RELU_IN) return 0;
    if (cch != 8 || nchunks != 1 || kextc != (d->KH == 4 ? 144 : 80) || d->nslabs < 1) return 0;
    if (d->KH == 4 && !e.wgrad4) return 0;
    if ((int64_t)d->Hout * d->Wout * 16 >= (1ll << 31)) return 0;
    if ((int64_t)d->B * cdiv(d->Wout, 30) * cdiv(d->Hout, 8) < e.min_tasks) return 0;
    return 1;
}

int msau_rowwgrad_launch(hipStream_t s, const msau_wgrad_desc* d) {
    RowWgradArgs a;
    a.d = *d;
    a.nstrips = cdiv(d->Wout, 30);
    const RowsEnv& e = rows_env();
    int target = WG_WAVES * d->nslabs;
    if (target > e.waves) target = e.waves;
    int nseg = target / (d->B * a.nstrips);
    if (nseg < 1) nseg = 1;
    int sh = e.sh > 0 ? e.sh : cdiv(d->Hout, nseg);
    if (sh < 9) sh = 9;
    sh = roundup(sh, d->KH);
    a.SH = sh < d->Hout ? sh : d->Hout;
    a.nseg = cdiv(d->Hout, a.SH);
    a.ntasks = d->B * a.nstrips * a.nseg;
    a.row_bytes = d->Wout * 16;
    a.img_bytes = (unsigned)d->Hout * (unsigned)a.row_bytes;
    a.kext = d->KH == 4 ? 144 : 80;
    const bool relu = d->flags & MSAU_CONV_RELU_IN;
    if (d->KH == 4) {
        if (relu) hipLaunchKernelGGL((rowwgrad8_kernel<true, 4>), dim3(d->nslabs), dim3(64 * WG_WAVES), 0, s, a);
        else hipLaunchKernelGGL((rowwgrad8_kernel<false, 4>), dim3(d->nslabs), dim3(64 * WG_WAVES), 0, s, a);
    } else if (relu) hipLaunchKernelGGL((rowwgrad8_kernel<true>), dim3(d->nslabs), dim3(64 * WG_WAVES), 0, s, a);
    else hipLaunchKernelGGL((rowwgrad8_kernel<false>), dim3(d->nslabs), dim3(64 * WG_WAVES), 0, s, a);
    MSAU_CHECK_LAUNCH("rowwgrad8_kernel");
    return 0;
}
```

### msau_amd/csrc/msau_common.h

```cpp
#pragma once
#include <hip/hip_runtime.h>
#include <stdint.h>
#include <stdio.h>
#include <stdarg.h>
#include "../../include/msau_hip.h"

typedef __bf16 bf16_t;
typedef __bf16 bf16x8 __attribute__((ext_vector_type(8)));
typedef __bf16 bf16x4 __attribute__((ext_vector_type(4)));
typedef float f32x4 __attribute__((ext_vector_type(4)));
typedef float f32x8 __attribute__((ext_vector_type(8)));

#define MSAU_LDS_LIMIT (160 * 1024)

int msau_set_error(int code, const char* fmt, ...);

int msau_rowpair_takes(int dtype, const msau_conv_pair_desc* d);
int64_t msau_rowpair_plane_bytes(const msau_conv_pair_desc* d);
int msau_ownerconv_takes(int dtype, const msau_conv_desc* d);
int msau_ownerconv_fwd(hipStream_t s, int dtype, const msau_conv_desc* d);
int msau_ownerconv_wgrad(hipStream_t s, int dtype, const msau_wgrad_desc* d, int cch, int nchunks, int kext);
int msau_ownerconv_slabs(const msau_wgrad_desc* d);
int msau_rowpair_workgroups(const msau_conv_pair_desc* d);
int msau_rowpair_launch(hipStream_t s, const msau_conv_pair_desc* d);
int msau_rowconv_takes(int dtype, const msau_conv_desc* d);
int msau_rowconv_launch(hipStream_t s, int dtype, const msau_conv_desc* d, int kchunk, int rows);
int msau_rowwgrad_takes(int dtype, const msau_wgrad_desc* d, int cch, int nchunks, int kextc);
int msau_rowwgrad_launch(hipStream_t s, const msau_wgrad_desc* d);

#define MSAU_CHECK_ARG(cond, ...)                                   \
    do {                                                            \
        if (!(cond)) return msau_set_error(MSAU_ERR_ARG, __VA_ARGS__); \
    } while (0)

#define MSAU_CHECK_LAUNCH(name)                                                         \
    do {                                                                                \
        hipError_t e__ = hipGetLastError();                                             \
        if (e__ != hipSuccess)                                                          \
            return msau_set_error(MSAU_ERR_HIP, "%s: %s", name, hipGetErrorString(e__)); \
    } while (0)

static inline int64_t cdiv64(int64_t a, int64_t b) { return (a + b - 1) / b; }
static inline int cdiv(int a, int b) { return (a + b - 1) / b; }
static inline int roundup(int a, int b) { return cdiv(a, b) * b; }

constexpr int lds_pixel_stride(int raw_bytes, int esz, int c8_per_chunk, int read_stride) {
    if (esz == 2 && c8_per_chunk >= 2 && read_stride == 1) {
        int p = raw_bytes / 16;
        while (p % 4 != 2) ++p;
        return p * 16;
    }
    return ((raw_bytes / 16) % 2 == 0) ? raw_bytes + 16 : raw_bytes;
}
constexpr int lds_wrow_stride(int nks, int esz) { return nks * 32 * esz + (esz == 2 ? 32 : 16); }

template <typename T> struct Vec8;
template <> struct Vec8<float>  { typedef f32x8 type; };
template <> struct Vec8<bf16_t> { typedef bf16x8 type; };
template <typename T> struct Vec4;
template <> struct Vec4<float>  { typedef f32x4 type; };
template <> struct Vec4<bf16_t> { typedef bf16x4 type; };

__device__ __forceinline__ bool pos_in_extent(int j, int W, int eh, int ew) { const int y = j / W; return y < eh && j - y * W < ew; }

template <typename T> __device__ __forceinline__ float to_f32(T v) { return (float)v; }
template <typename T> __device__ __forceinline__ T from_f32(float v) { return (T)v; }

template <typename T> __device__ __forceinline__ typename Vec8<T>::type zero8() {
    typename Vec8<T>::type z;
#pragma unroll
    for (int i = 0; i < 8; ++i) z[i] = (T)0.0f;
    return z;
}
template <typename T> __device__ __forceinline__ typename Vec8<T>::type relu8(typename Vec8<T>::type v) {
#pragma unroll
    for (int i = 0; i < 8; ++i) v[i] = ((float)v[i] > 0.0f) ? v[i] : (T)0.0f;
    return v;
}
typedef short s16x8 __attribute__((ext_vector_type(8)));
template <> __device__ __forceinline__ bf16x8 relu8<bf16_t>(bf16x8 v) {
    s16x8 i = __builtin_bit_cast(s16x8, v);
    s16x8 z = {0, 0, 0, 0, 0, 0, 0, 0};
    i = __builtin_elementwise_max(i, z);
    return __builtin_bit_cast(bf16x8, i);
}
template <typename T> __device__ __forceinline__ typename Vec8<T>::type load8(const T* p) {
    return *reinterpret_cast<const typename Vec8<T>::type*>(p);
}
template <typename T> __device__ __forceinline__ void store8(T* p, typename Vec8<T>::type v) {
    *reinterpret_cast<typename Vec8<T>::type*>(p) = v;
}
template <typename T> __device__ __forceinline__ typename Vec4<T>::type load4(const T* p) {
    return *reinterpret_cast<const typename Vec4<T>::type*>(p);
}
template <typename T> __device__ __forceinline__ void store4(T* p, typename Vec4<T>::type v) {
    *reinterpret_cast<typename Vec4<T>::type*>(p) = v;
}

__device__ __forceinline__ int msau_head_softmax(float (&v)[16], int C) {
    float mx = -INFINITY;
#pragma unroll
    for (int c = 0; c < 16; ++c) if (c < C) mx = fmaxf(mx, v[c]);
    float se = 0.f;
#pragma unroll
    for (int c = 0; c < 16; ++c) if (c < C) se += __expf(v[c] - mx);
    const float inv = 1.f / se;
    int best = 0;
    float bp = -1.f;
// ... 17 lines not shown
```

### msau_amd/plan.py

```python
from __future__ import annotations

import ctypes as C
import math
import os
from typing import Dict, List, NamedTuple, Optional, Tuple

import torch

from . import _lib as L


def same_pads(in_size: int, k: int, stride: int = 1, dilation: int = 1) -> Tuple[int, int]:
    k_eff = k + (k - 1) * (dilation - 1)
    out = -(-in_size // stride)
    pad = max((out - 1) * stride + k_eff - in_size, 0)
    return pad // 2, pad - pad // 2


def _ru(a: int, b: int) -> int:
    return -(-a // b) * b


def _ptr(t: Optional[torch.Tensor]) -> Optional[int]:
    return None if t is None else t.data_ptr()


class Launch(NamedTuple):
    kind: int
    args: Optional[C.Structure]
    key: str
    nbytes: float
    flops: float = 0.0


class Act:

    def __init__(self, plan: "Plan", name: str, H: int, W: int, C: int, relu_out: bool = False,
                 needs_grad: bool = True):
        self.plan, self.name, self.H, self.W, self.C = plan, name, H, W, C
        self.Cs = _ru(C, 8)
        self.relu_out = relu_out
        self.needs_grad = needs_grad and plan.training
        self.data = None if plan.reuse else torch.zeros((plan.B, H, W, self.Cs), dtype=plan.tdtype, device=plan.device)
        self.grad: Optional[torch.Tensor] = None
        self.n_contrib = 0
        plan.acts.append(self)

    @property
    def npix(self) -> int:
        return self.plan.B * self.H * self.W

    def register(self) -> int:
        k = self.n_contrib
        self.n_contrib += 1
        return k

    def slot_flags(self, k: int) -> Tuple[bool, bool]:
        return k != self.n_contrib - 1, (k == 0 and self.relu_out)

    def alloc_grad(self):
        if self.needs_grad and self.n_contrib > 0 and self.grad is None:
            self.grad = torch.zeros_like(self.data)


class Op:
    name = "op"

    def reads(self) -> List["Act"]:
        return []

    def writes(self) -> List["Act"]:
        return []

    def finalize(self):
        pass

    def fwd_recs(self) -> List[Launch]:
        raise NotImplementedError

    def bwd_recs(self) -> List[Launch]:
        return []


class ConvOp(Op):

    def __init__(self, plan: "Plan", name: str, x1: Act, x2: Optional[Act], wname: str, bname: str, out: Act,
                 k: int, dil: int = 1, relu_in: bool = False, relu_out: bool = False,
                 fwd_add: Optional[Act] = None, kind: str = "conv", head: bool = False):
        self.plan, self.name, self.x1, self.x2, self.out = plan, name, x1, x2, out
        self.head = head
        self.wname, self.bname, self.k, self.dil, self.kind = wname, bname, k, dil, kind
        self.relu_in, self.relu_out, self.fwd_add = relu_in, relu_out, fwd_add
        self.bwd_add: Optional[Act] = None
        self.pair: Optional["PairOp"] = None
        self.cpl: Optional["ConvOp"] = None
        self.cpl_fused_into: Optional["PairOp"] = None
        self.proj: Optional["ProjBwd"] = None
        self.dgrad2 = None
        self.dgrad_in_pair: Optional["PairOp"] = None
        if kind == "conv" and k == 1 and x2 is not None and relu_out and not relu_in and fwd_add is None and plan.ops:
            prod = plan.ops[-1]
            if isinstance(prod, ConvOp) and prod.out is x2 and prod.pair is not None and prod is prod.pair.c2 \
                    and x1.Cs == x2.Cs == out.Cs == x2.C == out.C:
                prod.cpl = self
        assert out.relu_out == relu_out
        if kind == "conv":
            assert out.H == x1.H and out.W == x1.W
            self.pad_t = same_pads(x1.H, k, 1, dil)[0]
            self.pad_l = same_pads(x1.W, k, 1, dil)[0]
        else:
            assert x2 is None and dil == 1 and not relu_in
            p = k // 2
            for o, i in ((out.H, x1.H), (out.W, x1.W)):
                op = o - ((i - 1) * 2 - 2 * p + k)
                assert 0 <= op < 2, f"{name}: output size {o} unreachable from {i}"
            self.pad_t = self.pad_l = k - 1 - p
        self.slots = []
        for x in (x1, x2):
            self.slots.append(x.register() if (x is not None and x.needs_grad) else None)
        self.stage = plan._cur_stage
        plan.ops.append(self)

    def reduce_group(self):
        return -1 if (self.stage == 0 and self.name.startswith("s0.d0.")) else self.stage

    def reads(self):
        return [t for t in (self.x1, self.x2, self.fwd_add) if t is not None]

    def writes(self):
        lrn, pool = getattr(self, "lrn", None), getattr(self, "pool", None)
        w = [self.out] + ([lrn.y] if lrn is not None else []) + ([pool.y] if pool is not None else [])
        if self.cpl is not None:
            w += [t for t in self.cpl.writes() if t not in w]
        return w

    def _geom(self, C1, C2, Cout, dil, stride, ups):
        g = L.ConvPackGeom()
        L.call("msau_conv_pack_geometry", self.plan.dtype, C1, C2, Cout, self.k, self.k, dil, stride, ups, C.byref(g))
        return g

    def _pack_entry(self, g, off, row_is_dim0, flip, row_off, rows_real, k1, k2):
# ... 57 lines not shown
        if P.training and self.dd_off is None:
            for si, x in enumerate((x1, x2)):
                if x is None or self.slots[si] is None:
                    continue
                if conv:
                    gd = self._geom(out.Cs, 0, x.Cs, self.dil, 1, 1)
                    self.d_off[si] = P.alloc_pack(gd.bytes)
                    e, n = self._pack_entry(gd, self.d_off[si], row_is_dim0=False, flip=True,
                                            row_off=(0 if si == 0 else x1.C), rows_real=x.C,
                                            k1=(out.C, out.Cs), k2=(0, 0))
                else:
                    gd = self._geom(out.Cs, 0, x.Cs, 1, 2, 1)
                    self.d_off[si] = P.alloc_pack(gd.bytes)
                    e, n = self._pack_entry(gd, self.d_off[si], row_is_dim0=True, flip=False, row_off=0,
                                            rows_real=x.C, k1=(out.C, out.Cs), k2=(0, 0))
                P.add_pack_entry(e, n)

    def bind(self):
        P = self.plan
        x1, x2, out = self.x1, self.x2, self.out
        conv = self.kind == "conv"
        d = L.ConvDesc()
        d.B, d.Hin, d.Win, d.Hout, d.Wout = P.B, x1.H, x1.W, out.H, out.W
        d.C1, d.C2, d.Cout = x1.Cs, (x2.Cs if x2 is not None else 0), out.Cs
        d.KH = d.KW = self.k
        d.dil, d.pad_t, d.pad_l, d.stride, d.ups = self.dil, self.pad_t, self.pad_l, 1, (1 if conv else 2)
        d.flags = (L.CONV_RELU_IN if self.relu_in else 0) | ((L.CONV_RELU_OUT | P.act_flag) if self.relu_out else 0) | \
                  (L.CONV_ADD if self.fwd_add is not None else 0) | P.extent_flag
        d.extent = P.extent_ptr(out)
        d.x1, d.x2 = _ptr(x1.data), _ptr(x2.data if x2 is not None else None)
        d.wpack, d.bias = P.pack_ptr(self.w_off), P.pack_ptr(self.b_off)
        d.add = _ptr(self.fwd_add.data) if self.fwd_add is not None else None
        d.y = _ptr(out.data)
        if self.head:
            d.head_probs, d.head_argmax, d.head_classes = _ptr(P.head_probs), _ptr(P.head_argmax), out.C
            info = (L.i32 * 8)()
            L.call("msau_conv2d_launch_info", P.dtype, C.byref(d), info)
            P.head_fused = bool(info[7] & 1) and d.flags == 0 and out.C <= 16
            if P.head_fused:
                d.flags = L.CONV_HEAD
        lrn = getattr(self, "lrn", None)
        if lrn is not None and conv and d.flags & ~L.CONV_RELU_IN == 0 and lrn.a.C == lrn.a.Cs:
            info = (L.i32 * 8)()
            L.call("msau_conv2d_launch_info", P.dtype, C.byref(d), info)
            if info[7] & 4:
                d.flags |= L.CONV_LRN
                d.y2 = _ptr(lrn.y.data)
                d.lrn_alpha_over_n, d.lrn_beta, d.lrn_k = 1e-4 / lrn.a.C, 0.75, 1.0
                lrn.fused_into = self
        pool = getattr(self, "pool", None)
        if pool is not None and conv and not (d.flags & (L.CONV_LRN | L.CONV_HEAD)):
            info = (L.i32 * 8)()
            L.call("msau_conv2d_launch_info", P.dtype, C.byref(d), info)
            if info[7] & 8:
                d.flags |= L.CONV_POOL
                d.pool_y, d.pool_idx = _ptr(pool.y.data), _ptr(pool.idx)
                pool.fused_into = self
        self.fdesc = d
        self.ddesc = [None, None]
        self.wdesc = None
        if not P.training or out.grad is None:
            return
        if self.dd_off is not None:
            dd = L.ConvDesc()
            dd.B = P.B
            dd.Hin, dd.Win, dd.Hout, dd.Wout = out.H, out.W, x1.H, x1.W
            dd.C1, dd.C2, dd.Cout = out.Cs, 0, x1.Cs + x2.Cs
            dd.KH = dd.KW = self.k
            dd.dil, dd.stride, dd.ups = self.dil, 1, 1
            dd.pad_t = (self.k - 1) * self.dil - self.pad_t
            dd.pad_l = (self.k - 1) * self.dil - self.pad_l
            assert not self.relu_in
            fl = [0, 0]
            for si, x in enumerate((x1, x2)):
                accum, maskb = x.slot_flags(self.slots[si])
                fl[si] = (L.CONV_ACCUM if accum else 0) | (L.CONV_MASK_B if maskb else 0)
                if maskb:
                    setattr(dd, "mask_b" if si == 0 else "mask_b2", _ptr(x.data))
            if self.bwd_add is not None:
                fl[0] |= L.CONV_ADD
                dd.add = _ptr(self.bwd_add.grad)
            dd.flags, dd.flags2 = fl[0] | L.CONV_DOUT, fl[1]
            dd.x1, dd.wpack, dd.bias = _ptr(out.grad), P.pack_ptr(self.dd_off), None
            dd.y, dd.y2 = _ptr(x1.grad), _ptr(x2.grad)
            self.ddesc[0] = dd
        for si, x in enumerate((x1, x2)):
            if x is None or self.slots[si] is None or self.dd_off is not None:
                continue
            accum, maskb = x.slot_flags(self.slots[si])
            dd = L.ConvDesc()
            dd.B = P.B
            dd.Hin, dd.Win, dd.Hout, dd.Wout = out.H, out.W, x.H, x.W
            dd.C1, dd.C2, dd.Cout = out.Cs, 0, x.Cs
            dd.KH = dd.KW = self.k
            if conv:
                dd.dil, dd.stride, dd.ups = self.dil, 1, 1
                dd.pad_t = (self.k - 1) * self.dil - self.pad_t
                dd.pad_l = (self.k - 1) * self.dil - self.pad_l
            else:
                dd.dil, dd.stride, dd.ups = 1, 2, 1
                dd.pad_t = dd.pad_l = self.k // 2
            fl = 0
            if self.relu_in:
                fl |= L.CONV_MASK_A
                dd.mask_a = _ptr(x.data)
            if si == 0 and self.bwd_add is not None:
                fl |= L.CONV_ADD
                dd.add = _ptr(self.bwd_add.grad)
            if accum:
                fl |= L.CONV_ACCUM
            if maskb:
                fl |= L.CONV_MASK_B | P.act_flag
                dd.mask_b = _ptr(x.data)
            dd.flags = fl | P.extent_flag
            dd.extent = P.extent_ptr(x)
            dd.x1, dd.wpack, dd.bias, dd.y = _ptr(out.grad), P.pack_ptr(self.d_off[si]), None, _ptr(x.grad)
            self.ddesc[si] = dd
        self.dgrad2 = None
        d1, d2 = self.ddesc
        if conv and self.k == 1 and x2 is not None and self.dd_off is None and d1 is not None and d2 is not None \
                and P.dtype == L.BF16 and not P.generic_only and x1.C == x1.Cs == x2.C == x2.Cs == out.Cs == 64 \
                and not ((d1.flags | d2.flags) & ~(L.CONV_ACCUM | L.CONV_MASK_B)) and os.environ.get("MSAU_DGRAD2", "1") != "0":
            geo = [self._geom(out.Cs, 0, x.Cs, 1, 1, 1) for x in (x1, x2)]
            if all((gq.nchunks, gq.rows, gq.kchunk) == (1, 64, 64) for gq in geo):
                a = L.Dgrad2Args()
                a.g, a.w1_pack, a.w2_pack = _ptr(out.grad), P.pack_ptr(self.d_off[0]), P.pack_ptr(self.d_off[1])
                a.dx1, a.dx2 = _ptr(x1.grad), _ptr(x2.grad)
                a.mask1 = d1.mask_b if d1.flags & L.CONV_MASK_B else None
                a.mask2 = d2.mask_b if d2.flags & L.CONV_MASK_B else None
                a.npix, a.C = out.npix, 64
                a.accumulate1, a.accumulate2 = int(bool(d1.flags & L.CONV_ACCUM)), int(bool(d2.flags & L.CONV_ACCUM))
                self.dgrad2 = a
        w = L.WgradDesc()
        w.B = P.B
        w.KH = w.KW = self.k
        if conv:
            w.Hin, w.Win, w.Hout, w.Wout = x1.H, x1.W, out.H, out.W
            w.C1, w.C2, w.Cout = x1.Cs, (x2.Cs if x2 is not None else 0), out.Cs
            w.dil, w.pad_t, w.pad_l, w.stride = self.dil, self.pad_t, self.pad_l, 1
            w.flags = L.CONV_RELU_IN if self.relu_in else 0
            w.x1, w.x2, w.g = _ptr(x1.data), _ptr(x2.data if x2 is not None else None), _ptr(out.grad)
            rows_real, k1, k2 = out.C, (x1.C, x1.Cs), ((x2.C, x2.Cs) if x2 is not None else (0, 0))
        else:
            w.Hin, w.Win, w.Hout, w.Wout = out.H, out.W, x1.H, x1.W
            w.C1, w.C2, w.Cout = out.Cs, 0, x1.Cs
            w.dil, w.pad_t, w.pad_l, w.stride = 1, self.k // 2, self.k // 2, 2
            w.flags = 0
            w.x1, w.x2, w.g = _ptr(out.grad), None, _ptr(x1.data)
            rows_real, k1, k2 = x1.C, (out.C, out.Cs), (0, 0)
        wg = L.WgradGeom()
        w.nslabs = 1
        L.call("msau_wgrad_geometry", P.dtype, C.byref(w), C.byref(wg))
        nslabs = max(1, min(wg.max_slabs, int(os.environ.get('MSAU_SLAB_CAP', '384')), max(int(os.environ.get('MSAU_SLAB_MIN', '64')), (int(os.environ.get('MSAU_SLAB_MB', '3')) << 20) // max(wg.slab_bytes, 1))))
        w.nslabs = nslabs
        slab_elems = wg.slab_bytes // 4
        self.slab_off = P.alloc_slab(nslabs * slab_elems)
        self.wdesc, self.wgeom = w, wg
        shp = P.pshape[self.wname]
        taps = self.k * self.k
        u = L.UnpackEntry()
        u.slab_off, u.w_off, u.b_off = self.slab_off, P.poff[self.wname], P.poff[self.bname]
        u.nslabs, u.slab_elems, u.kext = nslabs, slab_elems, wg.kext
        u.dim0, u.dim1, u.KH, u.KW, u.row_is_dim0, u.rows_real = shp[0], shp[1], self.k, self.k, 1, rows_real
        u.k1_real, u.k1_store = k1
        u.k2_real, u.k2_store = k2
        u.cch, u.nchunks, u.accumulate = wg.cch, wg.nchunks, 0
        if conv:
            u.b_src_off, u.b_slab_stride, u.b_elem_stride, u.b_nslabs = self.slab_off + taps * wg.cch, slab_elems, wg.kext, nslabs
            u.b_count = out.C
        else:
            self.csum_blocks = max(1, min(256, out.npix // 1024))
            self.csum_off = P.alloc_slab(self.csum_blocks * out.Cs)
            u.b_src_off, u.b_slab_stride, u.b_elem_stride, u.b_nslabs = self.csum_off, out.Cs, 1, self.csum_blocks
            u.b_count = out.C
        P.add_unpack_entry(u, slab_elems, self.reduce_group())
        self.uentry = u
        dd = self.ddesc[0]
        if conv and self.k == 1 and x2 is not None and self.dd_off is not None and dd is not None and not self.relu_in \
                and dd.flags == L.CONV_DOUT and dd.flags2 == L.CONV_MASK_B and u.kext == 16 and u.slab_elems == 256 and u.cch == 8 \
                and u.nchunks == 2 and os.environ.get("MSAU_COUPLE_WGRAD", "1") != "0" and P.cfg.get("couple_wgrad", True):
            dd.flags |= L.CONV_WGRAD
            dd.wg_x1, dd.wg_slabs = _ptr(x1.data), 1
            ns = int(L.load().msau_conv2d_rider_slabs(P.dtype, C.byref(dd)))
            if ns > 0:
                dd.wg_nslabs = ns
                self.wg_slab_off = P.alloc_slab(ns * 256)
                u.slab_off, u.nslabs = self.wg_slab_off, ns
                u.b_src_off, u.b_nslabs = self.wg_slab_off + 8, ns
                self.wg_fused = True
            else:
                dd.flags &= ~L.CONV_WGRAD
                dd.wg_x1 = dd.wg_slabs = None

    def late_bind(self):
        P = self.plan
        if self.wdesc is not None:
            self.wdesc.slabs = P.slab_ptr(self.slab_off)
        if self.wg_fused and self.pair is None and self.ddesc[0] is not None and self.ddesc[0].flags & L.CONV_WGRAD:
            self.ddesc[0].wg_slabs = P.slab_ptr(self.wg_slab_off)
        T = "f32" if P.dtype == L.F32 else "bf16"
        esz = 4 if P.dtype == L.F32 else 2
        taps = self.k * self.k
        cin_real = self.x1.C + (self.x2.C if self.x2 is not None else 0)
        self.flops = 2.0 * P.B * (self.out.H * self.out.W if self.kind == "conv" else self.x1.H * self.x1.W) * \
            taps * cin_real * self.out.C

        def conv_meta(d):
            info = (L.i32 * 8)()
            L.call("msau_conv2d_launch_info", P.dtype, C.byref(d), info)
            nin = d.B * d.Hin * d.Win * (d.C1 + d.C2)
            nout = d.B * d.Hout * d.Wout * d.Cout
            extra = sum(1 for f in (L.CONV_ADD, L.CONV_ACCUM, L.CONV_MASK_A, L.CONV_MASK_B, L.CONV_LRN) if d.flags & f)
            if d.flags & L.CONV_DOUT:
                half = nout // 2
                ex1 = sum(1 for f in (L.CONV_ADD, L.CONV_ACCUM, L.CONV_MASK_B) if d.flags & f)
                ex2 = sum(1 for f in (L.CONV_ACCUM, L.CONV_MASK_B) if d.flags2 & f)
                rider = (half * esz + d.wg_nslabs * 256 * 4) if d.flags & L.CONV_WGRAD else 0
                return f"conv_lean_kernel<{T},CIN{d.C1},CT{info[0]},K{d.KH},dout{',wgrad' if rider else ''}>", (nin + half * (2 + ex1 + ex2)) * esz + rider
            if info[6] == 3:
                name = f"rowconv_kernel<{T},CIN{d.C1 + d.C2},CO{d.Cout},K{d.KH}{',lrn' if d.flags & L.CONV_LRN else ''}{',ups2' if d.ups == 2 else ''}>"
            elif info[6] == 2:
                name = f"conv_chunked_kernel<{T},CIN{d.C1},K{d.KH}>"
            elif info[6]:
                var = ",dual" if d.C2 else ",ups2" if d.ups == 2 else ",s2" if d.stride == 2 else ""
                var += ",lrn" if d.flags & L.CONV_LRN else ""
                name = f"conv_lean_kernel<{T},CIN{d.C1 + d.C2},CT{info[0]},K{d.KH}{var}>"
            else:
                name = f"conv_kernel<{T},CT{info[0]},PT{info[1]}>"
            pooled = (nout // 4) * (esz + 1) if d.flags & L.CONV_POOL else 0
            return name, (nin + nout * (1 + extra)) * esz + pooled

        self.fkey, self.fbytes = conv_meta(self.fdesc)
        self.dmeta = [None, None]
        for si, dd in enumerate(self.ddesc):
            if dd is not None:
                src_c = (self.x1.C + self.x2.C) if self.dd_off is not None else (self.x1, self.x2)[si].C
                fl = 2.0 * P.B * (self.out.H * self.out.W if self.kind == "conv" else self.x1.H * self.x1.W) * taps * src_c * self.out.C
                self.dmeta[si] = conv_meta(dd) + (fl,)
        if self.dgrad2 is not None:
            a = self.dgrad2
            nops = 3 + a.accumulate1 + a.accumulate2 + (1 if a.mask1 else 0) + (1 if a.mask2 else 0)
            self.d2meta = ("dgrad2_1x1<bf16,C64>", self.out.npix * 64 * nops * esz, 2.0 * self.out.npix * 128 * self.out.C)
        if self.wdesc is not None:
            w, wg = self.wdesc, self.wgeom
            ctn = -(-w.Cout // 16)
            ctn = 4 if ctn == 3 else (8 if ctn > 4 else ctn)
            nkw = -(-(wg.kext // 16) // 4)
            nkw = 1 if nkw <= 1 else 2 if nkw <= 2 else 3 if nkw <= 3 else 5 if nkw <= 5 else 10
            if wg.lean == 2:
                self.wkey = f"rowwgrad_kernel<{T},C{wg.cch},CO{w.Cout},K{w.KH}>"
            elif wg.lean:
                self.wkey = f"wgrad_lean_kernel<{T},C{wg.cch},CO{w.Cout},K{w.KH}>"
            else:
                self.wkey = f"wgrad_kernel<{T},CT{ctn},NK{nkw}>"
            self.wbytes = (w.B * w.Hin * w.Win * (w.C1 + w.C2) * wg.nchunks // wg.nchunks + w.B * w.Hout * w.Wout * w.Cout) * esz \
                + w.nslabs * wg.slab_bytes

    def fwd_recs(self):
        if self.cpl_fused_into is not None:
            return []
        if self.pair is not None and self.pair.active:
            return [self.pair.fwd_rec()] if self is self.pair.c2 else []
        return [Launch(L.OP_CONV2D, self.fdesc, self.fkey, self.fbytes, self.flops)]

    def bwd_recs(self):
        if self.wdesc is None:
            return []
        side = L.OP_SIDE if self.plan.overlap_wgrad else 0
        if self.x1 is self.plan.x_in:
            side = 0
        recs = [] if self.wg_fused else [Launch(L.OP_WGRAD | side, self.wdesc, self.wkey, self.wbytes, self.flops)]
        if self.kind != "conv":
            P, g = self.plan, self.out.grad
            self._csum = L.CsumArgs(_ptr(g), self.out.npix, self.out.Cs, P.slab_ptr(self.csum_off), self.csum_blocks)
            recs.append(Launch(L.OP_CHANNEL_SUM | side, self._csum, "msau_channel_sum", g.numel() * g.element_size()))
        if self.pair is not None and self.pair.active and self.pair.bdesc is not None:
            if self is self.pair.c2:
                if self.pair.dcp is not None:
                    return [self.pair.bwd_rec()] + recs
                recs.append(self.pair.bwd_rec())
            return recs
        if self.dgrad_in_pair is not None:
            return recs
        if self.proj is not None and self.proj.active:
            return recs + (self.proj.recs() if self is self.proj.f else [])
        if self.dgrad2 is not None:
            return recs + [Launch(L.OP_DGRAD2_1X1, self.dgrad2, *self.d2meta)]
        return recs + [Launch(L.OP_CONV2D, dd, *self.dmeta[si]) for si, dd in enumerate(self.ddesc) if dd is not None]


class PairOp:

    def __init__(self, plan: "Plan", c1: ConvOp, c2: ConvOp):
        self.plan, self.c1, self.c2 = plan, c1, c2
        self.active = False
        self.fdesc = self.bdesc = None
        self.dcp: Optional[ConvOp] = None
        c1.pair = c2.pair = self
        plan.pairs.append(self)

    def bind(self):
        P, c1, c2 = self.plan, self.c1, self.c2
        x0, r1, out = c1.x1, c1.out, c2.out
        if os.environ.get("MSAU_FUSE_PAIR", "1") == "0" or not P.cfg.get("fuse_pair", True) or P.generic_only:
            return
        ok = (c1.kind == c2.kind == "conv" and c1.k == c2.k == 3 and c1.dil == c2.dil == 1 and c1.x2 is None and c2.x2 is None
              and c1.relu_in and c1.relu_out and c1.fwd_add is None and not c2.relu_in and c2.relu_out and c2.fwd_add is x0
              and c2.x1 is r1 and x0.C == x0.Cs == r1.C == out.C and x0.Cs in (8, 16, 32) and not c1.head and not c2.head
              and r1.n_contrib == (1 if P.training else 0))
        if not ok:
            return
        f = L.ConvPairDesc()
        f.B, f.H, f.W, f.C = P.B, x0.H, x0.W, x0.Cs
        f.flags1, f.flags2 = L.PAIR_RELU_IN | L.PAIR_RELU_MID, L.CONV_ADD | L.CONV_RELU_OUT
        f.x, f.w1, f.b1, f.mid = _ptr(x0.data), P.pack_ptr(c1.w_off), P.pack_ptr(c1.b_off), _ptr(r1.data)
        f.w2, f.b2, f.add, f.y = P.pack_ptr(c2.w_off), P.pack_ptr(c2.b_off), _ptr(x0.data), _ptr(out.data)
        if not L.load().msau_conv_pair_applicable(P.dtype, C.byref(f)):
            return
        pool = getattr(c2, "pool", None)
        if pool is not None and x0.Cs < int(os.environ.get("MSAU_PAIR_POOL_MINC", "16")):
            pool.fused_into = None
            pool = None
        if pool is not None:
            f.flags2 |= L.CONV_POOL
            f.pool_y, f.pool_idx = _ptr(pool.y.data), _ptr(pool.idx)
            if L.load().msau_conv_pair_applicable(P.dtype, C.byref(f)):
                pool.fused_into = self
            else:
                f.flags2 &= ~L.CONV_POOL
                pool.fused_into = None
        self.fdesc = f
        T = "f32" if P.dtype == L.F32 else "bf16"
        esz = 4 if P.dtype == L.F32 else 2
        self.key = f"conv_pair_kernel<{T},C{x0.Cs}>"
        n = P.B * x0.H * x0.W * x0.Cs
        self.fbytes = 3 * n * esz
        if f.flags2 & L.CONV_POOL:
            self.fbytes += (n // 4) * (esz + 1)
        if P.training and c1.ddesc[0] is not None and c2.ddesc[0] is not None and c1.ddesc[1] is None and c2.ddesc[1] is None \
                and c1.d_off[0] is not None and c2.d_off[0] is not None:
            d1, d2 = c1.ddesc[0], c2.ddesc[0]
            if d2.flags == L.CONV_MASK_B and not (d1.flags & ~(L.CONV_MASK_A | L.CONV_ADD | L.CONV_ACCUM | L.CONV_MASK_B)):
                b = L.ConvPairDesc()
                b.B, b.H, b.W, b.C = P.B, x0.H, x0.W, x0.Cs
                b.flags1, b.flags2 = L.PAIR_MASK_MID, d1.flags
                b.x, b.w1, b.b1, b.mask_mid, b.mid = _ptr(out.grad), P.pack_ptr(c2.d_off[0]), None, d2.mask_b, _ptr(r1.grad)
                b.w2, b.b2, b.add, b.mask_a, b.mask_b, b.y = P.pack_ptr(c1.d_off[0]), None, d1.add, d1.mask_a, d1.mask_b, d1.y
                use_bits = os.environ.get("MSAU_PAIR_BITS", "1") != "0"
                if use_bits:
                    b.bits_mid = b.bits_a = 1
                if L.load().msau_conv_pair_applicable(P.dtype, C.byref(b)):
                    self.bdesc = b
                else:
                    b.bits_mid = b.bits_a = None
                self.bbytes = 5 * n * esz
                if self.bdesc is not None and use_bits:
                    nbits = int(L.load().msau_conv_pair_bits_bytes(P.dtype, C.byref(b)))
                    if nbits != int(L.load().msau_conv_pair_bits_bytes(P.dtype, C.byref(f))):
                        f.flags1 |= L.PAIR_TILES
                        b.flags1 |= L.PAIR_TILES
                        nbits = int(L.load().msau_conv_pair_bits_bytes(P.dtype, C.byref(b)))
                    self.bits_mid = torch.zeros((nbits,), dtype=torch.uint8, device=P.device)
                    self.bits_a = torch.zeros_like(self.bits_mid)
                    for dsc in (f, b):
                        dsc.bits_mid, dsc.bits_a = _ptr(self.bits_mid), _ptr(self.bits_a)
                    self.fbytes += 2 * nbits
                    self.bbytes = 3 * n * esz + 2 * nbits
                lrn = getattr(x0, "lrn_producer", None)
                if self.bdesc is not None and lrn is not None and x0.n_contrib == 1 and not (d1.flags & L.CONV_ACCUM) \
                        and lrn.a.grad is not None and lrn.a.n_contrib == 1 and not lrn.a.relu_out and lrn.a.C == lrn.a.Cs == x0.Cs \
                        and os.environ.get("MSAU_FUSE_LRN_BWD", "1") != "0":
                    b.flags1 |= L.PAIR_LRN_BWD
                    b.lrn_a, b.lrn_da = _ptr(lrn.a.data), _ptr(lrn.a.grad)
                    b.lrn_alpha_over_n, b.lrn_beta, b.lrn_k = 1e-4 / lrn.a.C, 0.75, 1.0
                    if L.load().msau_conv_pair_instance(P.dtype, C.byref(b)) == 2:
                        lrn.bwd_fused_into = self
                        self.bbytes += n * esz
                    else:
                        b.flags1 &= ~L.PAIR_LRN_BWD
                        b.lrn_a = b.lrn_da = None
                u = c1.uentry
                if self.bdesc is not None and u is not None and c1.wdesc is not None and c1.relu_in and r1.n_contrib == 1 \
                        and u.kext == 80 and u.slab_elems == 640 and os.environ.get("MSAU_PAIR_WGRAD", "1") != "0":
                    b.flags1 |= L.PAIR_WGRAD1
                    b.wg1_x, b.wg1_slabs = _ptr(x0.data), 1
                    ns = int(L.load().msau_conv_pair_wgrad_slabs(P.dtype, C.byref(b)))
                    if ns > 0:
                        b.wg1_nslabs = ns
                        self.wg_slab_off = P.alloc_slab(ns * 640)
                        u.slab_off, u.nslabs = self.wg_slab_off, ns
                        u.b_src_off, u.b_nslabs = self.wg_slab_off + 72, ns
                        c1.wg_fused = True
                        self.bbytes += ns * 640 * 4
                    else:
                        b.flags1 &= ~L.PAIR_WGRAD1
                        b.wg1_x = b.wg1_slabs = None
        cp = c2.cpl
        self.cpl = None
        if cp is not None and not (f.flags2 & L.CONV_POOL) and cp.x2 is out and getattr(cp, "lrn", None) is None and not cp.head \
                and os.environ.get("MSAU_PAIR_COUPLE", "1") != "0" and P.cfg.get("fuse_couple", True):
            f.flags1 |= L.PAIR_COUPLE
            f.cpl_prev, f.cpl_w, f.cpl_b, f.cpl_y = _ptr(cp.x1.data), P.pack_ptr(cp.w_off), P.pack_ptr(cp.b_off), _ptr(cp.out.data)
            cpool = getattr(cp, "pool", None)
            if cpool is not None:
                f.cpl_pool_y, f.cpl_pool_idx = _ptr(cpool.y.data), _ptr(cpool.idx)
                if not L.load().msau_conv_pair_applicable(P.dtype, C.byref(f)):
                    f.cpl_pool_y = f.cpl_pool_idx = None
                    cpool = None
            if L.load().msau_conv_pair_applicable(P.dtype, C.byref(f)):
                self.cpl = cp
                cp.cpl_fused_into = self
                if cpool is not None:
                    cpool.fused_into = self
                elif getattr(cp, "pool", None) is not None and cp.pool.fused_into is cp:
                    cp.pool.fused_into = None
                self.fbytes += 2 * n * esz + ((n // 4) * (esz + 1) if f.cpl_pool_y else 0)
            else:
                f.flags1 &= ~L.PAIR_COUPLE
                f.cpl_prev = f.cpl_w = f.cpl_b = f.cpl_y = f.cpl_pool_y = f.cpl_pool_idx = None
        b = self.bdesc
        plain = False
        if b is not None and cp is not None and cp.x2 is out and getattr(cp, "dcp_off", None) is not None and out.n_contrib == 1:
            d1, d2 = cp.ddesc
            if cp.dd_off is not None:
                plain = d1 is not None and d1.flags == L.CONV_DOUT and d1.flags2 == L.CONV_MASK_B and d1.mask_b2 == _ptr(out.data)
            else:
                plain = d1 is not None and d2 is not None and d1.flags == 0 and d2.flags == L.CONV_MASK_B and d2.mask_b == _ptr(out.data)
        if plain and os.environ.get("MSAU_PAIR_DCOUPLE", "1") != "0" and P.cfg.get("fuse_couple", True):
            b.flags1 |= L.PAIR_DCOUPLE
            b.dcp_dz, b.dcp_w, b.dcp_mask, b.dcp_dprev = _ptr(cp.out.grad), P.pack_ptr(cp.dcp_off), _ptr(out.data), _ptr(cp.x1.grad)
            if L.load().msau_conv_pair_applicable(P.dtype, C.byref(b)) and L.load().msau_conv_pair_instance(P.dtype, C.byref(b)) == 1:
                self.dcp = cp
                cp.dgrad_in_pair = self
                self.bbytes += 3 * n * esz
            else:
                b.flags1 &= ~L.PAIR_DCOUPLE
                b.dcp_dz = b.dcp_w = b.dcp_mask = b.dcp_dprev = None
        probe = self.bdesc if self.bdesc is not None else f
        if L.load().msau_conv_pair_instance(P.dtype, C.byref(probe)) == 2:
            self.key = f"rowpair_kernel<{T},C{x0.Cs}>"
        self.active = True

    def late_bind(self):
        if self.bdesc is not None and self.c1.wg_fused:
            self.bdesc.wg1_slabs = self.plan.slab_ptr(self.wg_slab_off)

    def fwd_rec(self) -> Launch:
        flops = self.c1.flops + self.c2.flops + (self.cpl.flops if self.cpl is not None else 0.0)
        return Launch(L.OP_CONV_PAIR, self.fdesc, self.key, self.fbytes, flops)

    def bwd_rec(self) -> Launch:
        flops = self.c1.flops + self.c2.flops + (2.0 * self.dcp.flops if self.dcp is not None else 0.0)
        return Launch(L.OP_CONV_PAIR, self.bdesc, self.key, self.bbytes, flops)


class BoxOp(Op):

    def __init__(self, plan, name, x: Act, y: Act, pname: str, relu_in: bool):
        self.plan, self.name, self.x, self.y, self.pname, self.relu_in = plan, name, x, y, pname, relu_in
        self.F = plan.cfg["num_box_per_channels"]
        assert y.C == x.C * self.F and x.C == x.Cs
        self.slot = x.register() if x.needs_grad else None
        self.bwd_add: Optional[Act] = None
        self.stage = plan._cur_stage
        plan.ops.append(self)
        plan.box_ops.append(self)

    def reads(self):
        return [self.x]

    def writes(self):
        return [self.y]

    def finalize(self):
        P, x = self.plan, self.x
        n = P.B * x.C * (x.H + 1) * (x.W + 1)
        self.ii = torch.zeros((n,), dtype=torch.float32, device=P.device) if P.training else None
        P.box_scratch = max(P.box_scratch, n * (self.F if P.training else 1))
        P.box_ws_ii = max(P.box_ws_ii, int(L.load().msau_box_integral_ws_floats(P.B, x.H, x.W, x.C * (self.F if P.training else 1))))
        self.params = torch.zeros((2, 4, x.C * self.F), dtype=torch.float32, device=P.device)
        self.ws = None
        if P.training and self.y.grad is not None:
            self.ws = torch.zeros((int(L.load().msau_box_pgrad_ws_floats(P.B, x.H, x.W, x.C, self.F)),), dtype=torch.float32, device=P.device)

    def _meta(self, bwd: bool) -> Tuple[str, float]:
        P, x, y = self.plan, self.x, self.y
        esz = 4 if P.dtype == L.F32 else 2
        T = "f32" if P.dtype == L.F32 else "bf16"
        nii = P.B * x.C * (x.H + 1) * (x.W + 1) * 4
        if not bwd:
            return f"box_fwd<{T},C{x.C}>", x.npix * x.Cs * esz + 4 * nii + y.npix * y.Cs * esz
        return f"box_bwd<{T},C{x.C}>", 2 * y.npix * y.Cs * esz + nii + 4 * self.F * nii + x.npix * x.Cs * esz

    def _args(self):
        P, x, y = self.plan, self.x, self.y
        a = L.BoxArgs()
        a.in_, a.ii = _ptr(x.data), _ptr(self.ii) if self.ii is not None else _ptr(P.box_ii_g)
        a.params_fwd, a.params_refl = self.params[0].data_ptr(), self.params[1].data_ptr()
        a.out, a.ws_ii = _ptr(y.data), _ptr(P.box_ws)
        a.B, a.H, a.W, a.C, a.F, a.Cs_in, a.Cs_out = P.B, x.H, x.W, x.C, self.F, x.Cs, y.Cs
        a.relu_in = int(self.relu_in)
        mb = float(P.cfg["max_box_sizes"])
        a.max_h = a.max_w = mb
        offs = [P.poff[f"{self.pname}.{nm}"] for nm in ("x_min", "x_max", "y_min", "y_max")]
        a.off_hmin, a.off_hmax, a.off_wmin, a.off_wmax = offs
        return a

    def fwd_recs(self):
        self._fa = self._args()
        return [Launch(L.OP_BOX_FWD, self._fa, *self._meta(False))]

    def bwd_recs(self):
        P, x, y = self.plan, self.x, self.y
        if self.ws is None:
            return []
        a = self._args()
        a.gout, a.ii_g, a.ws = _ptr(y.grad), _ptr(P.box_ii_g), _ptr(self.ws)
        a.gin = None
        if x.grad is not None and self.slot is not None:
            accum, maskb = x.slot_flags(self.slot)
            a.gin, a.accumulate = _ptr(x.grad), int(accum)
            a.mask_a = _ptr(x.data) if self.relu_in else None
            a.add = _ptr(self.bwd_add.grad) if self.bwd_add is not None else None
            a.mask_b = _ptr(x.data) if maskb else None
        P._box_bwd_args.append(a)
        return [Launch(L.OP_BOX_BWD, a, *self._meta(True))]

    def load_params(self, s, flat_params: torch.Tensor):
        a = self._fa
        L.call("msau_box_params", s, flat_params.data_ptr(), a.off_hmin, a.off_hmax, a.off_wmin, a.off_wmax, a.C, a.F, a.max_h, a.max_w,
               self.params[0].data_ptr(), self.params[1].data_ptr())


class LrnOp(Op):

    def __init__(self, plan, name, a: Act, y: Act):
        self.plan, self.name, self.a, self.y = plan, name, a, y
        self.slot = a.register() if a.needs_grad else None
        self.stage = plan._cur_stage
        self.fused_into = None
        self.bwd_fused_into = None
        y.lrn_producer = self
        prod = plan.ops[-1] if plan.ops else None
        if isinstance(prod, ConvOp) and prod.out is a and os.environ.get("MSAU_FUSE_LRN", "1") != "0":
            prod.lrn = self
        plan.ops.append(self)

    def reads(self):
        return [self.a]

    def writes(self):
        return [self.y]

    def _meta(self, bwd: bool) -> Tuple[str, float]:
        P, a = self.plan, self.a
        n = a.npix * a.Cs * (4 if P.dtype == L.F32 else 2)
        return f"lrn_{'bwd' if bwd else 'fwd'}<{'f32' if P.dtype == L.F32 else 'bf16'},C{a.Cs}>", (3 if bwd else 2) * n

    def fwd_recs(self):
        a, y = self.a, self.y
        if self.fused_into is not None:
            return []
        self._fa = L.LrnArgs(_ptr(a.data), None, _ptr(y.data), a.npix, a.C, a.Cs, a.C, 1e-4, 0.75, 1.0)
        return [Launch(L.OP_LRN_FWD, self._fa, *self._meta(False))]

    def bwd_recs(self):
        a, y = self.a, self.y
        if y.grad is None or a.grad is None or self.bwd_fused_into is not None:
            return []
        self._ba = L.LrnArgs(_ptr(a.data), _ptr(y.grad), _ptr(a.grad), a.npix, a.C, a.Cs, a.C, 1e-4, 0.75, 1.0)
        return [Launch(L.OP_LRN_BWD, self._ba, *self._meta(True))]


class PoolOp(Op):

    def __init__(self, plan, name, x: Act, y: Act):
        self.plan, self.name, self.x, self.y = plan, name, x, y
        assert y.H == (x.H + 1) // 2 and y.W == (x.W + 1) // 2 and y.Cs == x.Cs
        self.idx = torch.zeros((plan.B, y.H, y.W, y.Cs), dtype=torch.uint8, device=plan.device) if plan.training else None
        self.slot = x.register() if x.needs_grad else None
        self.stage = plan._cur_stage
        self.fused_into = None
        prod = plan.ops[-1] if plan.ops else None
        if isinstance(prod, ConvOp) and prod.out is x and os.environ.get("MSAU_FUSE_POOL", "1") != "0":
            prod.pool = self
        plan.ops.append(self)

    def reads(self):
        return [self.x]

    def writes(self):
        return [self.y]

    def _meta(self, bwd: bool) -> Tuple[str, float]:
        P, x, y = self.plan, self.x, self.y
        esz = 4 if P.dtype == L.F32 else 2
        T = "f32" if P.dtype == L.F32 else "bf16"
        nx, ny = x.npix * x.Cs, y.npix * y.Cs
        if not bwd:
            return f"pool_fwd<{T},C{x.Cs}>", (nx + ny) * esz + (ny if P.training else 0)
        accum, maskb = x.slot_flags(self.slot)
        return f"pool_bwd<{T},C{x.Cs}>", (ny + nx * (1 + int(accum) + int(maskb))) * esz + ny

    def fwd_recs(self):
        x, y = self.x, self.y
        if self.fused_into is not None:
            return []
        self._fa = L.PoolArgs(_ptr(x.data), _ptr(y.data), _ptr(self.idx), None, self.plan.B, x.H, x.W, x.Cs, 0, None)
        return [Launch(L.OP_POOL_FWD, self._fa, *self._meta(False))]

    def bwd_recs(self):
        x, y = self.x, self.y
        if y.grad is None or x.grad is None:
            return []
        accum, maskb = x.slot_flags(self.slot)
        self._ba = L.PoolArgs(_ptr(y.grad), _ptr(x.grad), _ptr(self.idx), _ptr(x.data) if maskb else None,
                              self.plan.B, x.H, x.W, x.Cs, int(accum) | (2 if maskb and self.plan.act_flag else 0),
                              self.plan.extent_ptr(x))
        return [Launch(L.OP_POOL_BWD, self._ba, *self._meta(True))]


class AttnCoreOp(Op):

    def __init__(self, plan, name, f: Act, g: Act, h: Act, x: Act, y: Act):
        self.plan, self.name, self.f, self.g, self.h, self.x, self.y = plan, name, f, g, h, x, y
        self.N = x.H * x.W
        self.stats = torch.zeros((plan.B, self.N, 2), dtype=torch.float32, device=plan.device)
        self.ws = torch.zeros((plan.B, self.N), dtype=torch.float32, device=plan.device)
        for t in (f, g, h):
            t.register()
        self.stage = plan._cur_stage
        plan.ops.append(self)

    def reads(self):
        return [self.f, self.g, self.h, self.x]

    def writes(self):
        return [self.y]

    def _args(self, bwd):
        return L.AttnArgs(_ptr(self.f.data), _ptr(self.g.data), _ptr(self.h.data),
                          _ptr(self.y.grad) if bwd else _ptr(self.x.data), _ptr(self.y.data), _ptr(self.stats),
                          _ptr(self.f.grad), _ptr(self.g.grad), _ptr(self.h.grad), _ptr(self.ws),
                          self.plan.B, self.N, self.f.Cs, self.h.Cs, self.plan.extent_ptr(self.x), self.x.W)

    def _meta(self, bwd: bool) -> Tuple[str, float, float]:
        P = self.plan
        esz = 4 if P.dtype == L.F32 else 2
        T = "f32" if P.dtype == L.F32 else "bf16"
        npx = P.B * self.N
        small, big = npx * self.f.Cs * esz, npx * self.h.Cs * esz
        ffl = 2.0 * P.B * self.N * self.N * (self.f.C + self.h.C)
        if not bwd:
            return f"selfattn_fwd<{T}>", 2 * small + 3 * big, ffl
        return f"selfattn_bwd<{T}>", 4 * small + 4 * big, 2.0 * ffl

    def fwd_recs(self):
        self._fa = self._args(False)
        return [Launch(L.OP_ATTN_FWD, self._fa, *self._meta(False))]

    def bwd_recs(self):
        if self.y.grad is None:
            return []
        self._ba = self._args(True)
        return [Launch(L.OP_ATTN_BWD, self._ba, *self._meta(True))]


class ProjBwd:

    def __init__(self, plan: "Plan", f: ConvOp, g: ConvOp, h: ConvOp):
        self.plan, self.f, self.g, self.h = plan, f, g, h
        self.active = False
        self.args = None
        for c in (f, g, h):
            c.proj = self
        plan.projs.append(self)

    def bind(self):
        P, f, g, h = self.plan, self.f, self.g, self.h
        x = f.x1
        df, dg, dh = f.ddesc[0], g.ddesc[0], h.ddesc[0]
        if P.dtype != L.BF16 or P.generic_only or os.environ.get("MSAU_ATTN_PROJ_FUSE", "1") == "0" or None in (df, dg, dh):
            return
        if not (x.C == x.Cs == 64 and f.out.Cs == g.out.Cs == 8 and h.out.Cs == 64 and f.k == g.k == h.k == 1
                and g.x1 is x and h.x1 is x and f.x2 is None and g.x2 is None and h.x2 is None
                and f.dd_off is None and not (f.relu_in or g.relu_in or h.relu_in)):
            return
        A, M, D = L.CONV_ACCUM, L.CONV_MASK_B, L.CONV_ADD
        if (dh.flags & ~(A | D)) or dg.flags != A or (df.flags & ~M) != A:
            return
        for c, kch in ((f, 32), (g, 32), (h, 64)):
            gd = c._geom(c.out.Cs, 0, x.Cs, 1, 1, 1)
            if (gd.nchunks, gd.rows, gd.kchunk) != (1, 64, kch):
                return
        a = L.AttnProjBwdArgs()
        a.df, a.dg, a.dh = _ptr(f.out.grad), _ptr(g.out.grad), _ptr(h.out.grad)
# ... 730 lines not shown
                and os.environ.get("MSAU_CE_MULTI", "1") != "0":
            K = self.counts_k
            if K > 1:
                L.call("msau_label_counts_split", s, labels.data_ptr(), self.counts.data_ptr(), self.B, HW, K, key="msau_label_counts")
            else:
                L.call("msau_label_counts", s, labels.data_ptr(), self.counts.data_ptr(), self.B, HW)
            L.call("msau_masked_ce_multi", s, self.dtype, lg.data.data_ptr(), _ptr(ax.data) if ax is not None else None,
                   labels.data_ptr(), self.counts.data_ptr(), lg.grad.data_ptr(), _ptr(ax.grad) if ax is not None else None,
                   self.loss_buf.data_ptr(), self.ce_multi_ws.data_ptr(), self.B, HW, lg.C, lg.Cs, 1.0 / self.B, K)
            return self.loss_buf
        L.call("msau_label_counts", s, labels.data_ptr(), self.counts.data_ptr(), self.B, HW)
        self.loss_buf.zero_()
        for act in (self.logits, self.aux):
            if act is None:
                continue
            L.call("msau_masked_ce", s, self.dtype, act.data.data_ptr(), labels.data_ptr(), self.counts.data_ptr(),
                   act.grad.data_ptr(), self.loss_buf.data_ptr(), self.ce_ws.data_ptr(), self.B, HW, act.C, act.Cs,
                   1.0 / self.B)
        return self.loss_buf

    def set_native_dp(self, comm: int, comm_stream, buckets, flat_grads: torch.Tensor):
        assert self.training and self._bwd_seq is not None and self.overlap_wgrad
        nb = len(self._bwd_segs)
        assert len(buckets) == nb + 1, (len(buckets), nb)
        arr, n, keep = self._bwd_seq
        recs = [(arr[i].kind, arr[i].args) for i in range(n)]
        self._dp_args = []
        out = []
        for i, (b, start, cnt) in enumerate(self._bwd_segs):
            out += recs[start:start + cnt]
            lo, hi = buckets[i + 1]
            self._dp_args.append(L.AllreduceArgs(comm, flat_grads.data_ptr() + 4 * lo, hi - lo))
            out.append((L.OP_ALLREDUCE | L.OP_COMM, C.addressof(self._dp_args[-1])))
        lo, hi = buckets[0]
        self._dp_args.append(L.AllreduceArgs(comm, flat_grads.data_ptr() + 4 * lo, hi - lo))
        out.append((L.OP_ALLREDUCE | L.OP_COMM, C.addressof(self._dp_args[-1])))
        seq = (L.Op * len(out))()
        for i, (kind, args) in enumerate(out):
            seq[i].kind, seq[i].dtype, seq[i].args = kind, self.dtype, args
        self._bwd_seq_dp = (seq, len(out), (keep, self._dp_args))
        self._dp_stream = comm_stream
        self._dp_flat = flat_grads.data_ptr()

    def backward(self, flat_grads: torch.Tensor, on_stage_done=None, native_dp: bool = False, single_stream: bool = False):
        s = self._stream()
        for ra in self._reduce_args:
            ra.flat_grads = flat_grads.data_ptr()
        for ba in self._box_bwd_args:
            ba.flat_grads = flat_grads.data_ptr()
        arr, n, _ = self._bwd_seq
        if not self.overlap_wgrad or self._one_stream(single_stream):
            self._run_seq(self._bwd_seq, s)
            if on_stage_done is not None:
                for b, _, _ in self._bwd_segs:
                    on_stage_done(b, torch.cuda.current_stream())
            return
        if self._side is None:
            self._side = L.concurrent_stream(self.device)
        side = self._side.cuda_stream
        if native_dp:
            seq, m, _ = self._bwd_seq_dp
            assert flat_grads.data_ptr() == self._dp_flat, "set_native_dp was given another gradient buffer"
            L.call("msau_run_ops_dp", s, side, self._dp_stream.cuda_stream, seq, m, 1)
            return
        if on_stage_done is None:
            L.call("msau_run_ops_overlap", s, side, arr, n, 1)
            return
        for i, (b, start, cnt) in enumerate(self._bwd_segs):
            last = i == len(self._bwd_segs) - 1
            seg = C.cast(C.byref(arr, start * C.sizeof(L.Op)), C.POINTER(L.Op))
            L.call("msau_run_ops_overlap", s, side, seg, cnt, 1 if last else 0)
            on_stage_done(b, self._side)

    def input_grad_nchw(self) -> torch.Tensor:
        a = self.x_in
        out = torch.empty((self.B, a.C, a.H, a.W), dtype=torch.float32, device=self.device)
        L.call("msau_nhwc_to_nchw", self._stream(), self.dtype, a.grad.data_ptr(), out.data_ptr(), self.B, a.C, a.Cs, a.H, a.W)
        return out

    def activation_bytes(self) -> int:
        n = 0
        for a in self.acts:
            n += a.data.numel() * a.data.element_size()
            if a.grad is not None:
                n += a.grad.numel() * a.grad.element_size()
        return n
```

Measured before the change: 5767 tiles/s.

## Fuse maxpool backward into coupling conv data-gradient load path

Adds an UNPOOL_IN mode to the 1x1 two-output bf16 dgrad conv (lean and row kernels). The mode gathers the pooled gradient through the argmax indices, adds it to the partial gradient, applies the ReLU mask, and writes the combined gradient while staging inputs. The plan routes other contributions into a separate partial buffer and drops the standalone pool-backward launch. This removes a kernel launch and a full read/write pass over the activation gradient, at the cost of extra loads per tile, an extra gradient buffer, and reordered backward records.

```diff
diff --git a/include/msau_hip.h b/include/msau_hip.h
--- a/include/msau_hip.h
+++ b/include/msau_hip.h
@@ -37,6 +37,7 @@
     MSAU_CONV_OWNER    = 2048,
     MSAU_CONV_NCHW     = 4096,
     MSAU_CONV_WGRAD    = 8192,
+    MSAU_CONV_UNPOOL_IN = 16384,
     MSAU_CONV_ELU      = 32768,
     MSAU_CONV_EXTENT   = 65536,
     MSAU_CONV_HEAD     = 64
@@ -73,6 +74,10 @@
     float* wg_slabs;
     int32_t wg_nslabs;
     int32_t reserved1;
+    const void* up_dy;
+    const uint8_t* up_idx;
+    const void* up_z;
+    void* up_g;
     const int32_t* extent;
 } msau_conv_desc;
 int msau_conv2d_rider_slabs(int dtype, const msau_conv_desc* d);
diff --git a/msau_amd/_lib.py b/msau_amd/_lib.py
--- a/msau_amd/_lib.py
+++ b/msau_amd/_lib.py
@@ -11,6 +11,7 @@
 CONV_RELU_IN, CONV_RELU_OUT, CONV_ADD, CONV_ACCUM, CONV_MASK_A, CONV_MASK_B, CONV_HEAD, CONV_DOUT = 1, 2, 4, 8, 16, 32, 64, 128
 CONV_LRN, CONV_POOL, CONV_IDS, CONV_OWNER, CONV_NCHW, CONV_WGRAD, CONV_ELU = 256, 512, 1024, 2048, 4096, 8192, 32768
 CONV_EXTENT = 65536
+CONV_UNPOOL_IN = 16384
 
 i32, i64, vp, f32 = C.c_int32, C.c_int64, C.c_void_p, C.c_float
 
@@ -21,7 +22,8 @@
                [(n, vp) for n in ("x1", "x2", "wpack", "bias", "add", "mask_a", "mask_b", "y", "head_probs", "head_argmax")] + \
                [("head_classes", i32), ("flags2", i32), ("y2", vp), ("mask_b2", vp)] + \
                [("lrn_alpha_over_n", f32), ("lrn_beta", f32), ("lrn_k", f32), ("reserved0", i32), ("pool_y", vp), ("pool_idx", vp)] + \
-               [("wg_x1", vp), ("wg_slabs", vp), ("wg_nslabs", i32), ("reserved1", i32), ("extent", vp)]
+               [("wg_x1", vp), ("wg_slabs", vp), ("wg_nslabs", i32), ("reserved1", i32)] + \
+               [(n, vp) for n in ("up_dy", "up_idx", "up_z", "up_g")] + [("extent", vp)]
 
 
 class ConvPairDesc(C.Structure):
diff --git a/msau_amd/csrc/conv.hip b/msau_amd/csrc/conv.hip
--- a/msau_amd/csrc/conv.hip
+++ b/msau_amd/csrc/conv.hip
@@ -334,7 +334,7 @@
 
 static int conv_takes_extent(int dtype, const msau_conv_desc* d, const ConvGeom& g) {
     const int only_others = MSAU_CONV_HEAD | MSAU_CONV_DOUT | MSAU_CONV_LRN | MSAU_CONV_POOL | MSAU_CONV_IDS | MSAU_CONV_OWNER |
-                            MSAU_CONV_NCHW | MSAU_CONV_WGRAD;
+                            MSAU_CONV_NCHW | MSAU_CONV_WGRAD | MSAU_CONV_UNPOOL_IN;
     if (d->flags & only_others) return 0;
     if (g.nslices == 1 && (msau_rowconv_takes(dtype, d) || msau_conv_chunked_capable(dtype, d, g.cch, g.nchunks, g.CT) ||
                            msau_conv_lean_applicable(dtype, d, g.nchunks, g.CT)))
@@ -371,6 +371,15 @@
         p.flags |= MSAU_CONV_EXTENT;
         if (conv_takes_extent(dtype, &p, g)) info[7] |= 128;
     }
+    if (g.nslices == 1 && (d->flags & MSAU_CONV_DOUT)) {
+        msau_conv_desc p = *d;
+        p.flags |= MSAU_CONV_UNPOOL_IN;
+        if (!p.up_dy) p.up_dy = p.wpack;
+        if (!p.up_idx) p.up_idx = static_cast<const uint8_t*>(p.wpack);
+        if (!p.up_z) p.up_z = p.wpack;
+        if (!p.up_g) p.up_g = p.y;
+        if (msau_rowconv_unpool_in(dtype, &p) || (!msau_rowconv_takes(dtype, &p) && msau_conv_lean_unpool_in(dtype, &p, g.nchunks, g.CT))) info[7] |= 256;
+    }
     if (g.nslices == 1 && !(info[7] & 4)) {
         msau_conv_desc p = *d;
         p.flags |= MSAU_CONV_LRN;
@@ -398,7 +407,7 @@
 }
 
 extern "C" int msau_conv2d(void* stream, int dtype, const msau_conv_desc* d) {
-    MSAU_CHECK_ARG(d && d->x1 && d->wpack && d->y, "conv2d: null pointer");
+    MSAU_CHECK_ARG(d && (d->x1 || (d->flags & MSAU_CONV_UNPOOL_IN)) && d->wpack && d->y, "conv2d: null pointer");
     MSAU_CHECK_ARG(d->B > 0 && d->Hin > 0 && d->Win > 0 && d->Hout > 0 && d->Wout > 0, "conv2d: bad dims");
     MSAU_CHECK_ARG(d->C1 % 8 == 0 && d->C2 % 8 == 0 && (d->C2 == 0 || d->x2), "conv2d: bad sources");
     MSAU_CHECK_ARG(!(d->flags & MSAU_CONV_ADD) || d->add, "conv2d: ADD without pointer");
@@ -415,6 +424,13 @@
     }
     if (d->flags & MSAU_CONV_WGRAD)
         MSAU_CHECK_ARG(msau_conv2d_rider_slabs(dtype, d) > 0, "conv2d: MSAU_CONV_WGRAD is not implemented for this launch (msau_conv2d_rider_slabs says 0)");
+    if (d->flags & MSAU_CONV_UNPOOL_IN) {
+        ConvGeom g;
+        int rc = conv_geom(dtype, d->C1, d->C2, d->Cout, d->KH, d->KW, d->dil, d->stride, d->ups, &g);
+        if (rc) return rc;
+        MSAU_CHECK_ARG(g.nslices == 1 && (msau_rowconv_unpool_in(dtype, d) || (!msau_rowconv_takes(dtype, d) && msau_conv_lean_unpool_in(dtype, d, g.nchunks, g.CT))), "conv2d: MSAU_CONV_UNPOOL_IN is not implemented for this launch (see msau_conv2d_launch_info "
+                       "info[7] & 256); run msau_maxpool2x2_bwd before it instead");
+    }
     if (d->flags & MSAU_CONV_OWNER) {
         MSAU_CHECK_ARG(msau_ownerconv_takes(dtype, d), "conv2d: MSAU_CONV_OWNER is the 3x3 stride-1 C -> 8 conv, no other flag but RELU_OUT");
         return msau_ownerconv_fwd(static_cast<hipStream_t>(stream), dtype, d);
@@ -435,7 +451,7 @@
                                   "msau_conv2d_launch_info info[7]); run msau_softmax_argmax_nhwc on y instead");
     }
     if (d->flags & MSAU_CONV_DOUT) {
-        const int okf = MSAU_CONV_DOUT | MSAU_CONV_ADD | MSAU_CONV_ACCUM | MSAU_CONV_MASK_B | MSAU_CONV_WGRAD;
+        const int okf = MSAU_CONV_DOUT | MSAU_CONV_ADD | MSAU_CONV_ACCUM | MSAU_CONV_MASK_B | MSAU_CONV_WGRAD | MSAU_CONV_UNPOOL_IN;
         MSAU_CHECK_ARG(d->y2 && !(d->flags & ~okf) && !(d->flags2 & ~(MSAU_CONV_ACCUM | MSAU_CONV_MASK_B)) &&
                        (!(d->flags2 & MSAU_CONV_MASK_B) || d->mask_b2), "conv2d: bad DOUT arguments");
         if (!msau_conv_lean_dout_capable(dtype, d, g.nchunks, g.CT) && !(g.nslices == 1 && msau_rowconv_takes(dtype, d)))
diff --git a/msau_amd/csrc/conv_lean.hip b/msau_amd/csrc/conv_lean.hip
--- a/msau_amd/csrc/conv_lean.hip
+++ b/msau_amd/csrc/conv_lean.hip
@@ -45,8 +45,9 @@
 constexpr int kOperandBits = MSAU_CONV_RELU_IN | MSAU_CONV_RELU_OUT | MSAU_CONV_ADD | MSAU_CONV_ACCUM | MSAU_CONV_MASK_A | MSAU_CONV_MASK_B;
 enum { EPI_NONE = 0, EPI_LRN = 1, EPI_POOL = 2, EPI_HEAD = 3 };
 template <typename T, int CIN8, int CT, int KS, bool DUAL, int DIL = 1, int WGW = 1, bool DOUT = false, bool SPLIT = false,
-          int STRIDE = 1, int UPS = 1, int EPI = EPI_NONE, int EOP = -1, bool IDS = false>
+          int STRIDE = 1, int UPS = 1, int EPI = EPI_NONE, int EOP = -1, bool IDS = false, bool UP = false>
 __global__ __launch_bounds__(256 * WGW) void conv_lean_kernel(const LeanArgs a) {
+    static_assert(!UP || (DOUT && KS == 1 && !DUAL && !SPLIT && !IDS && sizeof(T) == 2), "gather-on-load: the 1x1 two-output bf16 instances");
     static_assert(!IDS || (!DUAL && STRIDE == 1 && UPS == 1 && !DOUT && !SPLIT), "id-mask input: plain single-source instances");
     static_assert(!SPLIT || (CT == 1 && !DUAL && !DOUT && WGW == 1), "SPLIT instances are single-source, one tile per workgroup");
     static_assert((STRIDE == 1 && UPS == 1) || (!DUAL && !DOUT && WGW == 1 && DIL == 1 && STRIDE * UPS == 2), "strided / upsampling instances");
@@ -105,6 +106,8 @@
     constexpr int NSRC = DUAL ? 2 : 1;
     constexpr bool PIPE = IDS || NIT * NSRC <= 6;
     V8 pre[IDS ? 1 : NSRC][IDS ? 1 : NIT];
+    V8 upz[UP ? NIT : 1], upd[UP ? NIT : 1];
+    unsigned long long upi[UP ? NIT : 1];
     constexpr int NIDS = (Cfg::NPIX + NT - 1) / NT;
     int pre_id[IDS ? NIDS : 1];
     auto decode = [&](int tile, int& b, int& oy0, int& ox0) {
@@ -147,13 +150,26 @@
                     } else {
                         ok = (unsigned)vy < (unsigned)d.Hin && (unsigned)vx < (unsigned)d.Win;
                     }
+                    if constexpr (UP) {
+                        upz[it] = upd[it] = zero8<T>();
+                        upi[it] = 0ull;
+                        if (ok) {
+                            const unsigned o = (unsigned)(vy * in_row + vx * in_px + cg * 8 * ESZ);
+                            if (d.x1) pre[sidx][it] = *reinterpret_cast<const V8*>(base + o);
+                            upz[it] = *reinterpret_cast<const V8*>(static_cast<const char*>(d.up_z) + (long long)b * d.Hin * in_row + o);
+                            const int hp = (d.Hin + 1) >> 1, wp = (d.Win + 1) >> 1;
+                            const long long po = ((long long)(b * hp + (vy >> 1)) * wp + (vx >> 1)) * C8S + cg;
+                            upd[it] = *reinterpret_cast<const V8*>(static_cast<const char*>(d.up_dy) + po * (8 * ESZ));
+                            upi[it] = *reinterpret_cast<const unsigned long long*>(d.up_idx + po * 8);
+                        }
+                    } else
                     if (ok)
                         pre[sidx][it] = *reinterpret_cast<const V8*>(base + (unsigned)(vy * in_row + vx * in_px + cg * 8 * ESZ));
                 }
             }
         }
     };
-    auto write_lds = [&]() {
+    auto write_lds = [&](const int wb, const int woy0, const int wox0) {
         if constexpr (IDS) {
 #pragma unroll
             for (int it = 0; it < NIDS; ++it) {
@@ -178,6 +194,22 @@
                 if ((it + 1) * NT <= NITEMS || idx < NITEMS) {
                     const int pix = idx / C8S, cg = idx - pix * C8S;
                     V8 v = pre[sidx][it];
+                    if constexpr (UP) {
+                        const int iy = pix / TI, ix = pix - iy * TI;
+                        const int vy = woy0 + iy, vx = wox0 + ix;
+                        const unsigned pos = 2u * (unsigned)(vy & 1) + (unsigned)(vx & 1);
+                        V8 g;
+#pragma unroll
+                        for (int j = 0; j < 8; ++j) {
+                            float f = (float)v[j] + ((unsigned)((upi[it] >> (8 * j)) & 0xffull) == pos ? (float)upd[it][j] : 0.f);
+                            if (!((float)upz[it][j] > 0.f)) f = 0.f;
+                            g[j] = (T)f;
+                        }
+                        v = g;
+                        if (vy < d.Hin && vx < d.Win)
+                            *reinterpret_cast<V8*>(static_cast<char*>(d.up_g) + (long long)wb * d.Hin * a.in_row1 +
+                                                   (unsigned)(vy * a.in_row1 + vx * a.in_px1 + cg * 8 * ESZ)) = g;
+                    }
                     if (relu_in) v = relu8<T>(v);
                     *reinterpret_cast<V8*>(smem + pix * PS + (sidx * C8S + cg) * 8 * ESZ) = v;
                 }
@@ -223,7 +255,7 @@
         decode(tile, b, oy0, ox0);
         __syncthreads();
         if (!PIPE) issue_loads(tile);
-        write_lds();
+        write_lds(b, oy0, ox0);
         __syncthreads();
         if (tile == tile0) STAMP(2);
         if (PIPE && tile + tstep < tend) issue_loads(tile + tstep);
@@ -603,7 +635,7 @@
 }
 
 template <typename T, int CIN8, int CT, int KS, bool DUAL, int DIL = 1, int WGW = 1, bool DOUT = false, bool SPLIT = false,
-          int STRIDE = 1, int UPS = 1, int EPI = EPI_NONE, int EOP = -1, bool IDS = false>
+          int STRIDE = 1, int UPS = 1, int EPI = EPI_NONE, int EOP = -1, bool IDS = false, bool UP = false>
 int launch_lean_e(hipStream_t s, const LeanArgs& a0) {
     using Cfg = LeanCfg<T, CIN8, CT, KS, DUAL, DIL, WGW, STRIDE>;
     if (Cfg::LDS + 256 > MSAU_LDS_LIMIT) return 0;
@@ -613,7 +645,7 @@
     a.mag_tx = (unsigned)((0x100000000ull + a.tiles_x - 1) / a.tiles_x);
     static bool attr_set = false;
     if (!attr_set && Cfg::LDS > 60 * 1024) {
-        hipError_t e = hipFuncSetAttribute(reinterpret_cast<const void*>(&conv_lean_kernel<T, CIN8, CT, KS, DUAL, DIL, WGW, DOUT, SPLIT, STRIDE, UPS, EPI, EOP, IDS>),
+        hipError_t e = hipFuncSetAttribute(reinterpret_cast<const void*>(&conv_lean_kernel<T, CIN8, CT, KS, DUAL, DIL, WGW, DOUT, SPLIT, STRIDE, UPS, EPI, EOP, IDS, UP>),
                                            hipFuncAttributeMaxDynamicSharedMemorySize, MSAU_LDS_LIMIT);
         if (e != hipSuccess) return msau_set_error(MSAU_ERR_HIP, "conv_lean: hipFuncSetAttribute: %s", hipGetErrorString(e));
         attr_set = true;
@@ -629,7 +661,7 @@
         grid &= ~7;
         a.per_xcd = cdiv(a.ntiles, 8);
     }
-    hipLaunchKernelGGL((conv_lean_kernel<T, CIN8, CT, KS, DUAL, DIL, WGW, DOUT, SPLIT, STRIDE, UPS, EPI, EOP, IDS>), dim3(grid, SPLIT ? a.ct_total : 1), dim3(256 * WGW), Cfg::LDS, s, a);
+    hipLaunchKernelGGL((conv_lean_kernel<T, CIN8, CT, KS, DUAL, DIL, WGW, DOUT, SPLIT, STRIDE, UPS, EPI, EOP, IDS, UP>), dim3(grid, SPLIT ? a.ct_total : 1), dim3(256 * WGW), Cfg::LDS, s, a);
     MSAU_CHECK_LAUNCH("conv_lean_kernel");
     return 1;
 }
@@ -762,6 +794,13 @@
            d->Cout == CT * 16 && d->C1 == CT * 8;
 }
 
+int msau_conv_lean_unpool_in(int dtype, const msau_conv_desc* d, int nchunks, int CT) {
+    if (dtype != MSAU_BF16 || !(d->flags & MSAU_CONV_DOUT) || !(d->flags & MSAU_CONV_UNPOOL_IN)) return 0;
+    if (!msau_conv_lean_dout_capable(dtype, d, nchunks, CT) || d->KH != 1 || CT != 2 || d->pad_t != 0 || d->pad_l != 0) return 0;
+    if (d->flags & ~(MSAU_CONV_DOUT | MSAU_CONV_UNPOOL_IN | MSAU_CONV_ADD | MSAU_CONV_ACCUM | MSAU_CONV_MASK_B)) return 0;
+    return d->up_dy && d->up_idx && d->up_z && d->up_g && d->up_g != d->x1 && d->Hin >= 2 && d->Win >= 2;
+}
+
 static bool lean_wide_tile(const msau_conv_desc* d, int tiles_y) {
     return d->Wout >= 64 && (int64_t)d->B * tiles_y * cdiv(d->Wout, 32) >= 512;
 }
@@ -816,6 +855,12 @@
 
 template <typename T>
 int lean_dout(hipStream_t s, const LeanArgs& a, int KS, int CT) {
+    if (a.d.flags & MSAU_CONV_UNPOOL_IN) {
+        if constexpr (sizeof(T) == 2) {
+            if (KS == 1 && CT == 2) return launch_lean_e<T, 2, 2, 1, false, 1, 1, true, false, 1, 1, EPI_NONE, -1, false, true>(s, a);
+        }
+        return msau_set_error(MSAU_ERR_ARG, "conv_lean: no instance with MSAU_CONV_UNPOOL_IN (msau_conv2d_launch_info)");
+    }
 #define DO_CASE(K, C) if (KS == K && CT == C) return launch_lean<T, C, C, K, false, 1, 1, true>(s, a);
     DO_CASE(1, 1) DO_CASE(1, 2) DO_CASE(1, 4) DO_CASE(3, 1) DO_CASE(3, 2) DO_CASE(3, 4)
 #undef DO_CASE
diff --git a/msau_amd/csrc/conv_rows.hip b/msau_amd/csrc/conv_rows.hip
--- a/msau_amd/csrc/conv_rows.hip
+++ b/msau_amd/csrc/conv_rows.hip
@@ -800,10 +800,11 @@
 
 constexpr int WGC_ROW = 32 * 16;
 
-template <int NS, int KH, int KW, int EPI, int EPI2 = 0, bool WG = false>
+template <int NS, int KH, int KW, int EPI, int EPI2 = 0, bool WG = false, bool UP = false>
 __global__ __launch_bounds__(256) void rowconv8_kernel(const RowConvArgs a) {
     constexpr bool DOUT = (EPI & MSAU_CONV_DOUT) != 0;
     static_assert(!WG || (DOUT && KW == 1 && NS == 1 && EPI == MSAU_CONV_DOUT && EPI2 == MSAU_CONV_MASK_B), "the rider belongs to the coupling conv's data gradient");
+    static_assert(!UP || WG, "the gather-on-load belongs to the coupling conv's data gradient");
     __shared__ __align__(16) unsigned char wsm[WG ? 4 * 3 * WGC_ROW + 64 + 2 * 8 * 16 * 4 : 16];
     constexpr bool K1D = KW == 1 && NS == 2;
     static_assert((KW == 3 && (NS == 1 || NS == 2)) || (K1D && KH == 1) || (KW == 1 && NS == 1 && KH == 1 && DOUT) || (KW == 4 && NS == 1),
@@ -867,7 +868,8 @@
     constexpr bool ACC2 = (EPI2 & MSAU_CONV_ACCUM) != 0, MB2 = (EPI2 & MSAU_CONV_MASK_B) != 0;
 
     const long long img = (long long)b * a.img_bytes;
-    const __amdgpu_buffer_rsrc_t rx1 = rsrc_of(static_cast<const char*>(d.x1) + img, a.img_bytes);
+    const bool has_x1 = !UP || d.x1 != nullptr;
+    const __amdgpu_buffer_rsrc_t rx1 = rsrc_of(has_x1 ? static_cast<const char*>(d.x1) + img : nullptr, has_x1 ? a.img_bytes : 0u);
     const __amdgpu_buffer_rsrc_t rx2 = rsrc_of(NS == 2 && !K1D ? static_cast<const char*>(d.x2) + img : nullptr, NS == 2 && !K1D ? a.img_bytes : 0u);
     const __amdgpu_buffer_rsrc_t ry = rsrc_of(static_cast<char*>(d.y) + img, a.img_bytes);
     const __amdgpu_buffer_rsrc_t ry2 = rsrc_of(LRN || DOUT ? static_cast<char*>(d.y2) + img : nullptr, LRN || DOUT ? a.img_bytes : 0u);
@@ -885,10 +887,26 @@
     u32x4 X[NSL][NXR][XL];
     const char* src1x1 = nullptr;
     if constexpr (K1D) src1x1 = static_cast<const char*>(lg < 2 ? d.x1 : d.x2) + img + (lxm < W ? lxm : W - 1) * 16;
+    u32x4 UZ[UP ? NXR : 1], UD[UP ? NXR : 1];
+    u32x2 UI[UP ? NXR : 1];
+    const int upW = (W + 1) >> 1;
+    const unsigned up_img = (unsigned)((H + 1) >> 1) * (unsigned)upW * 16u;
+    const __amdgpu_buffer_rsrc_t ruz = rsrc_of(UP ? static_cast<const char*>(d.up_z) + img : nullptr, UP ? a.img_bytes : 0u);
+    const __amdgpu_buffer_rsrc_t rug = rsrc_of(UP ? static_cast<char*>(d.up_g) + img : nullptr, UP ? a.img_bytes : 0u);
+    const __amdgpu_buffer_rsrc_t rud = rsrc_of(UP ? static_cast<const char*>(d.up_dy) + (long long)b * up_img : nullptr, UP ? up_img : 0u);
+    const __amdgpu_buffer_rsrc_t rui = rsrc_of(UP ? reinterpret_cast<const char*>(d.up_idx) + (long long)b * (up_img >> 1) : nullptr, UP ? up_img >> 1 : 0u);
+    const unsigned up_col = lcol_m != kOOB ? (unsigned)((lxm >> 1) * 16) : kOOB;
     auto load_row = [&](int r, auto slot) {
         constexpr int S = decltype(slot)::value;
         const bool ok = r >= 0 && r <= rlast;
         const unsigned ro = (unsigned)(r * a.row_bytes);
+        if constexpr (UP) {
+            const bool okp = ok && up_col != kOOB;
+            const unsigned po = (unsigned)((r >> 1) * upW * 16) + up_col;
+            UZ[S] = __builtin_amdgcn_raw_buffer_load_b128(ruz, ok ? ro + lcol_m : kOOB, 0, 0);
+            UD[S] = __builtin_amdgcn_raw_buffer_load_b128(rud, okp ? po : kOOB, 0, 0);
+            UI[S] = __builtin_amdgcn_raw_buffer_load_b64(rui, okp ? po >> 1 : kOOB, 0, 0);
+        }
         if constexpr (K1D) {
             X[0][S][0] = *reinterpret_cast<const u32x4*>(src1x1 + (long long)(ok ? r : y0) * a.row_bytes);
         } else {
@@ -949,6 +967,21 @@
         const int t = tg + I;
         load_row(t - d.pad_t + NXR - 1, IC<(I + NXR - 1) % NXR>{});
         load_prev(t - d.pad_t + NXR - 1, IC<(I + NXR - 1) % NXR>{});
+        if constexpr (UP) {
+            constexpr int S = I % NXR;
+            const bf16x8 pp = __builtin_bit_cast(bf16x8, X[0][S][0]), pz = __builtin_bit_cast(bf16x8, UZ[S]), pd = __builtin_bit_cast(bf16x8, UD[S]);
+            const unsigned pos = 2u * (unsigned)(t & 1) + (unsigned)(lxm & 1);
+            bf16x8 gq;
+#pragma unroll
+            for (int jj = 0; jj < 8; ++jj) {
+                const unsigned pw = jj < 4 ? UI[S][0] : UI[S][1];
+                float v = (float)pp[jj] + (((pw >> (8 * (jj & 3))) & 0xffu) == pos ? (float)pd[jj] : 0.f);
+                if (!((float)pz[jj] > 0.f)) v = 0.f;
+                gq[jj] = (bf16_t)v;
+            }
+            X[0][S][0] = __builtin_bit_cast(u32x4, gq);
+            __builtin_amdgcn_raw_buffer_store_b128(X[0][S][0], rug, (t >= y0 && t < y1) ? (unsigned)(t * a.row_bytes) + lcol_m : kOOB, 0, 0);
+        }
         f32x4 acc = bias;
 #pragma unroll
         for (int ky = 0; ky < KH; ++ky)
@@ -1517,6 +1550,8 @@
         if (k == 3 && d->pad_t == 1 && d->pad_l == 1 && f2 == 0) return f1 == 0 ? 9 : f1 == MSAU_CONV_ACCUM ? 10 : 0;
         if (k == 1 && d->pad_t == 0 && d->pad_l == 0 && f1 == 0 && f2 == MSAU_CONV_MASK_B && d->mask_b2) return 11;
         if (k == 1 && d->pad_t == 0 && d->pad_l == 0 && f1 == MSAU_CONV_WGRAD && f2 == MSAU_CONV_MASK_B && d->mask_b2 && d->wg_x1 && d->wg_slabs && e.cplwg) return 13;
+        if (k == 1 && d->pad_t == 0 && d->pad_l == 0 && f1 == (MSAU_CONV_WGRAD | MSAU_CONV_UNPOOL_IN) && f2 == MSAU_CONV_MASK_B && d->mask_b2 && d->wg_x1 &&
+            d->wg_slabs && e.cplwg && d->up_dy && d->up_idx && d->up_z && d->up_g && d->up_g != d->x1 && d->Hout >= 2 && d->Wout >= 2) return 14;
         return 0;
     }
     if (k == 3 && !dual && d->pad_t == 1 && d->pad_l == 1) {
@@ -1536,6 +1571,7 @@
 }
 
 int msau_rowconv_takes(int dtype, const msau_conv_desc* d) { return rowconv_case(dtype, d) != 0; }
+int msau_rowconv_unpool_in(int dtype, const msau_conv_desc* d) { return rowconv_case(dtype, d) == 14; }
 
 namespace {
 void rowconv_split(const msau_conv_desc* d, RowConvArgs& a) {
@@ -1555,7 +1591,9 @@
 }
 
 extern "C" int msau_conv2d_rider_slabs(int dtype, const msau_conv_desc* d) {
-    if (!d || !(d->flags & MSAU_CONV_WGRAD) || rowconv_case(dtype, d) != 13) return 0;
+    if (!d || !(d->flags & MSAU_CONV_WGRAD)) return 0;
+    const int which = rowconv_case(dtype, d);
+    if (which != 13 && which != 14) return 0;
     RowConvArgs a;
     rowconv_split(d, a);
     return 8 * (a.tasks_per_xcd / 4);
@@ -1606,9 +1644,11 @@
         case 10: return launch_rowconv8<1, 3, 3, MSAU_CONV_DOUT | MSAU_CONV_ACCUM>(s, a);
         case 11: return launch_rowconv8<1, 1, 1, MSAU_CONV_DOUT, MSAU_CONV_MASK_B>(s, a);
         case 13:
+        case 14:
             MSAU_CHECK_ARG(8 * (a.tasks_per_xcd / 4) == d->wg_nslabs, "conv2d: MSAU_CONV_WGRAD launch has %d workgroups, the caller allocated %d slabs "
                            "(msau_conv2d_rider_slabs under other MSAU_ROWS_* settings?)", 8 * (a.tasks_per_xcd / 4), d->wg_nslabs);
-            hipLaunchKernelGGL((rowconv8_kernel<1, 1, 1, MSAU_CONV_DOUT, MSAU_CONV_MASK_B, true>), dim3(8 * (a.tasks_per_xcd / 4)), dim3(256), 0, s, a);
+            if (which == 14) hipLaunchKernelGGL((rowconv8_kernel<1, 1, 1, MSAU_CONV_DOUT, MSAU_CONV_MASK_B, true, true>), dim3(8 * (a.tasks_per_xcd / 4)), dim3(256), 0, s, a);
+            else hipLaunchKernelGGL((rowconv8_kernel<1, 1, 1, MSAU_CONV_DOUT, MSAU_CONV_MASK_B, true>), dim3(8 * (a.tasks_per_xcd / 4)), dim3(256), 0, s, a);
             MSAU_CHECK_LAUNCH("rowconv8_kernel");
             return 0;
     }
diff --git a/msau_amd/csrc/msau_common.h b/msau_amd/csrc/msau_common.h
--- a/msau_amd/csrc/msau_common.h
+++ b/msau_amd/csrc/msau_common.h
@@ -24,6 +24,8 @@
 int msau_rowpair_workgroups(const msau_conv_pair_desc* d);
 int msau_rowpair_launch(hipStream_t s, const msau_conv_pair_desc* d);
 int msau_rowconv_takes(int dtype, const msau_conv_desc* d);
+int msau_rowconv_unpool_in(int dtype, const msau_conv_desc* d);
+int msau_conv_lean_unpool_in(int dtype, const msau_conv_desc* d, int nchunks, int CT);
 int msau_rowconv_launch(hipStream_t s, int dtype, const msau_conv_desc* d, int kchunk, int rows);
 int msau_rowwgrad_takes(int dtype, const msau_wgrad_desc* d, int cch, int nchunks, int kextc);
 int msau_rowwgrad_launch(hipStream_t s, const msau_wgrad_desc* d);
diff --git a/msau_amd/plan.py b/msau_amd/plan.py
--- a/msau_amd/plan.py
+++ b/msau_amd/plan.py
@@ -43,6 +43,7 @@
         self.needs_grad = needs_grad and plan.training
         self.data = None if plan.reuse else torch.zeros((plan.B, H, W, self.Cs), dtype=plan.tdtype, device=plan.device)
         self.grad: Optional[torch.Tensor] = None
+        self.gpart: Optional[torch.Tensor] = None
         self.n_contrib = 0
         plan.acts.append(self)
 
@@ -57,6 +58,9 @@
 
     def slot_flags(self, k: int) -> Tuple[bool, bool]:
         return k != self.n_contrib - 1, (k == 0 and self.relu_out)
+
+    def gw(self) -> Optional[torch.Tensor]:
+        return self.gpart if self.gpart is not None else self.grad
 
     def alloc_grad(self):
         if self.needs_grad and self.n_contrib > 0 and self.grad is None:
@@ -280,7 +284,7 @@
                 dd.add = _ptr(self.bwd_add.grad)
             dd.flags, dd.flags2 = fl[0] | L.CONV_DOUT, fl[1]
             dd.x1, dd.wpack, dd.bias = _ptr(out.grad), P.pack_ptr(self.dd_off), None
-            dd.y, dd.y2 = _ptr(x1.grad), _ptr(x2.grad)
+            dd.y, dd.y2 = _ptr(x1.gw()), _ptr(x2.gw())
             self.ddesc[0] = dd
         for si, x in enumerate((x1, x2)):
             if x is None or self.slots[si] is None or self.dd_off is not None:
@@ -312,7 +316,7 @@
                 dd.mask_b = _ptr(x.data)
             dd.flags = fl | P.extent_flag
             dd.extent = P.extent_ptr(x)
-            dd.x1, dd.wpack, dd.bias, dd.y = _ptr(out.grad), P.pack_ptr(self.d_off[si]), None, _ptr(x.grad)
+            dd.x1, dd.wpack, dd.bias, dd.y = _ptr(out.grad), P.pack_ptr(self.d_off[si]), None, _ptr(x.gw())
             self.ddesc[si] = dd
         self.dgrad2 = None
         d1, d2 = self.ddesc
@@ -323,7 +327,7 @@
             if all((gq.nchunks, gq.rows, gq.kchunk) == (1, 64, 64) for gq in geo):
                 a = L.Dgrad2Args()
                 a.g, a.w1_pack, a.w2_pack = _ptr(out.grad), P.pack_ptr(self.d_off[0]), P.pack_ptr(self.d_off[1])
-                a.dx1, a.dx2 = _ptr(x1.grad), _ptr(x2.grad)
+                a.dx1, a.dx2 = _ptr(x1.gw()), _ptr(x2.gw())
                 a.mask1 = d1.mask_b if d1.flags & L.CONV_MASK_B else None
                 a.mask2 = d2.mask_b if d2.flags & L.CONV_MASK_B else None
                 a.npix, a.C = out.npix, 64
@@ -389,6 +393,37 @@
             else:
                 dd.flags &= ~L.CONV_WGRAD
                 dd.wg_x1 = dd.wg_slabs = None
+        self._bind_unpool()
+
+    def _bind_unpool(self):
+        P, z, dd = self.plan, self.out, self.ddesc[0]
+        self.unpool: Optional["PoolOp"] = None
+        if os.environ.get("MSAU_FUSE_UNPOOL", "1") == "0" or dd is None or self.dd_off is None or P.dtype != L.BF16 or P.generic_only \
+                or P.ragged or P.act_flag or not z.relu_out or z.name in P.ext_slot:
+            return
+        level = P.levels.index((z.H, z.W)) if (z.H, z.W) in P.levels else -1
+        if str(level) not in os.environ.get("MSAU_FUSE_UNPOOL_LEVELS", "0,1,2").split(","):
+            return
+        readers = [op for op in P.ops if op is not self and any(t is z for t in op.reads())]
+        pools = [op for op in readers if isinstance(op, PoolOp)]
+        if len(pools) != 1 or pools[0].slot != 0 or pools[0].y.grad is None or pools[0].idx is None:
+            return
+        pool = pools[0]
+        if not all(isinstance(op, ConvOp) and (op.x1 is z or op.x2 is z) and op.fwd_add is not z for op in readers if op is not pool):
+            return
+        if z.n_contrib != len(readers):
+            return
+        info = (L.i32 * 8)()
+        L.call("msau_conv2d_launch_info", P.dtype, C.byref(dd), info)
+        if not info[7] & 256:
+            return
+        if z.n_contrib > 1:
+            z.gpart = torch.zeros_like(z.grad)
+        dd.flags |= L.CONV_UNPOOL_IN
+        dd.x1 = _ptr(z.gpart)
+        dd.up_dy, dd.up_idx, dd.up_z, dd.up_g = _ptr(pool.y.grad), _ptr(pool.idx), _ptr(z.data), _ptr(z.grad)
+        self.unpool = pool
+        pool.bwd_fused_into = self
 
     def late_bind(self):
         P = self.plan
@@ -414,7 +449,12 @@
                 ex1 = sum(1 for f in (L.CONV_ADD, L.CONV_ACCUM, L.CONV_MASK_B) if d.flags & f)
                 ex2 = sum(1 for f in (L.CONV_ACCUM, L.CONV_MASK_B) if d.flags2 & f)
                 rider = (half * esz + d.wg_nslabs * 256 * 4) if d.flags & L.CONV_WGRAD else 0
-                return f"conv_lean_kernel<{T},CIN{d.C1},CT{info[0]},K{d.KH},dout{',wgrad' if rider else ''}>", (nin + half * (2 + ex1 + ex2)) * esz + rider
+                unpool = 0
+                if d.flags & L.CONV_UNPOOL_IN:
+                    npool = d.B * ((d.Hin + 1) // 2) * ((d.Win + 1) // 2) * d.C1
+                    unpool = (2 * nin - (0 if d.x1 else nin)) * esz + npool * (esz + 1)
+                return f"conv_lean_kernel<{T},CIN{d.C1},CT{info[0]},K{d.KH},dout{',wgrad' if rider else ''}{',unpool' if unpool else ''}>", \
+                    (nin + half * (2 + ex1 + ex2)) * esz + rider + unpool
             if info[6] == 3:
                 name = f"rowconv_kernel<{T},CIN{d.C1 + d.C2},CO{d.Cout},K{d.KH}{',lrn' if d.flags & L.CONV_LRN else ''}{',ups2' if d.ups == 2 else ''}>"
             elif info[6] == 2:
@@ -484,6 +524,8 @@
             return recs + (self.proj.recs() if self is self.proj.f else [])
         if self.dgrad2 is not None:
             return recs + [Launch(L.OP_DGRAD2_1X1, self.dgrad2, *self.d2meta)]
+        if getattr(self, "unpool", None) is not None:
+            return [Launch(L.OP_CONV2D, dd, *self.dmeta[si]) for si, dd in enumerate(self.ddesc) if dd is not None] + recs
         return recs + [Launch(L.OP_CONV2D, dd, *self.dmeta[si]) for si, dd in enumerate(self.ddesc) if dd is not None]
 
 
@@ -626,7 +668,7 @@
                 plain = d1 is not None and d2 is not None and d1.flags == 0 and d2.flags == L.CONV_MASK_B and d2.mask_b == _ptr(out.data)
         if plain and os.environ.get("MSAU_PAIR_DCOUPLE", "1") != "0" and P.cfg.get("fuse_couple", True):
             b.flags1 |= L.PAIR_DCOUPLE
-            b.dcp_dz, b.dcp_w, b.dcp_mask, b.dcp_dprev = _ptr(cp.out.grad), P.pack_ptr(cp.dcp_off), _ptr(out.data), _ptr(cp.x1.grad)
+            b.dcp_dz, b.dcp_w, b.dcp_mask, b.dcp_dprev = _ptr(cp.out.grad), P.pack_ptr(cp.dcp_off), _ptr(out.data), _ptr(cp.x1.gw())
             if L.load().msau_conv_pair_applicable(P.dtype, C.byref(b)) and L.load().msau_conv_pair_instance(P.dtype, C.byref(b)) == 1:
                 self.dcp = cp
                 cp.dgrad_in_pair = self
@@ -779,6 +821,7 @@
         self.slot = x.register() if x.needs_grad else None
         self.stage = plan._cur_stage
         self.fused_into = None
+        self.bwd_fused_into = None
         prod = plan.ops[-1] if plan.ops else None
         if isinstance(prod, ConvOp) and prod.out is x and os.environ.get("MSAU_FUSE_POOL", "1") != "0":
             prod.pool = self
@@ -809,7 +852,7 @@
 
     def bwd_recs(self):
         x, y = self.x, self.y
-        if y.grad is None or x.grad is None:
+        if y.grad is None or x.grad is None or self.bwd_fused_into is not None:
             return []
         accum, maskb = x.slot_flags(self.slot)
         self._ba = L.PoolArgs(_ptr(y.grad), _ptr(x.grad), _ptr(self.idx), _ptr(x.data) if maskb else None,
@@ -1706,6 +1749,7 @@
         n = 0
         for a in self.acts:
             n += a.data.numel() * a.data.element_size()
-            if a.grad is not None:
-                n += a.grad.numel() * a.grad.element_size()
+            for g in (a.grad, a.gpart):
+                if g is not None:
+                    n += g.numel() * g.element_size()
         return n
```

New measurement: 5797 tiles/s (median of 4 runs). No clear change (+0.5%).
